# zzhang1987/Factor-Graph-Neural-Network

Hardware: AMD Instinct MI355X
Metric: VF+FV messages/sec on 96.3.963 LDPC graph (higher is better)
Workload: dtype bf16

## Files before the change

factor-graph-neural-network_amd/csrc/bnact.hip:

```cpp
#include "fgnn_common.h"
#include "fgnn_device.h"
#include "fgnn_gridfold.h"
#include <stdlib.h>

#define BN_THREADS 256
#define BN_GRID 512
#define BN_MAXPART 1024
#define BN_APPLY_GRID 4096

struct BnParams {
    const void* x;
    const void* gy;
    void* out;
    float* ws;
    const float* a;
    const float* b;
    const float* gamma;
    const float* beta;
    const float* ref;
    const void* addend;
    const void* addend2;
    const void* addend3;
    int aperiod[3];
    int64_t R;
// ... 27 lines not shown
        const uint4 t = *reinterpret_cast<const uint4*>(p);
        v[0] = __uint_as_float(t.x << 16); v[1] = __uint_as_float(t.x & 0xffff0000u);
        v[2] = __uint_as_float(t.y << 16); v[3] = __uint_as_float(t.y & 0xffff0000u);
        v[4] = __uint_as_float(t.z << 16); v[5] = __uint_as_float(t.z & 0xffff0000u);
        v[6] = __uint_as_float(t.w << 16); v[7] = __uint_as_float(t.w & 0xffff0000u);
    }
    __device__ static void store(bf16_t* p, const float (&v)[8]) {
        *reinterpret_cast<uint4*>(p) = make_uint4(fgnn_pack2(v[0], v[1]), fgnn_pack2(v[2], v[3]), fgnn_pack2(v[4], v[5]), fgnn_pack2(v[6], v[7]));
    }
};

template <typename T, int MODE>
__global__ __launch_bounds__(BN_THREADS) void bn_reduce_kernel(const BnParams p) {
    constexpr int EPC = Chunk<T>::EPC;
    __shared__ __attribute__((aligned(16))) float red[BN_THREADS * 2 * EPC];
    const int tid = threadIdx.x;
    const int cpr = 1 << p.cshift;
    const int cg = tid & (cpr - 1), rg = tid >> p.cshift;
    const int rstep = BN_THREADS >> p.cshift;
    const int c0 = cg * EPC;
    const T* xg = static_cast<const T*>(p.x);
    const T* gg = static_cast<const T*>(p.gy);
    float s0[EPC], s1[EPC], ka[EPC], kb[EPC], kc[EPC], kd[EPC];
#pragma unroll
    for (int e = 0; e < EPC; ++e) {
        s0[e] = 0.f; s1[e] = 0.f;
        if (MODE == 0) { ka[e] = p.ref ? p.ref[c0 + e] : 0.f; kb[e] = 0.f; kc[e] = 0.f; kd[e] = 0.f; }
        else {
            ka[e] = p.a[c0 + e];
            kb[e] = p.b[c0 + e];
            kc[e] = p.gamma[c0 + e] * kb[e];
            kd[e] = p.beta[c0 + e] - ka[e] * kc[e];
        }
    }
    const int64_t r_begin = (int64_t)blockIdx.x * p.rows_per_wg;
    const int64_t r_end = r_begin + p.rows_per_wg < p.R ? r_begin + p.rows_per_wg : p.R;
#pragma unroll 4
    for (int64_t r = r_begin + rg; r < r_end; r += rstep) {
        float v[EPC];
        Chunk<T>::load(xg + r * p.C + c0, v);
        if (MODE == 0) {
#pragma unroll
            for (int e = 0; e < EPC; ++e) { const float dlt = v[e] - ka[e]; s0[e] += dlt; s1[e] = fmaf(dlt, dlt, s1[e]); }
        } else {
            float g[EPC];
            Chunk<T>::load(gg + r * p.C + c0, g);
#pragma unroll
            for (int e = 0; e < EPC; ++e) {
                const float pre = fmaf(v[e], kc[e], kd[e]);
                const float ge = pre > 0.f ? g[e] : g[e] * p.slope;
                s0[e] += ge;
                s1[e] = fmaf(ge, (v[e] - ka[e]) * kb[e], s1[e]);
            }
        }
    }
#pragma unroll
    for (int e = 0; e < EPC; ++e) { red[(tid * 2) * EPC + e] = s0[e]; red[(tid * 2 + 1) * EPC + e] = s1[e]; }
    __syncthreads();
    if (rg == 0) {
        for (int q = 1; q < rstep; ++q) {
            const int t2 = q * cpr + cg;
#pragma unroll
            for (int e = 0; e < EPC; ++e) { s0[e] += red[(t2 * 2) * EPC + e]; s1[e] += red[(t2 * 2 + 1) * EPC + e]; }
        }
        float* w = p.ws + (int64_t)blockIdx.x * 2 * p.C;
#pragma unroll
        for (int e = 0; e < EPC; ++e) { fgnn_fold_store(w + c0 + e, s0[e]); fgnn_fold_store(w + p.C + c0 + e, s1[e]); }
    }
    if (p.fold.tickets) {
        double* sums = reinterpret_cast<double*>(red);
        if (fgnn_grid_fold(p.fold, sums, blockIdx.x)) {
            if (MODE == 0) fgnn_bn_final_apply(p.fin, p.C, sums);
            else fgnn_bn_bwd_final_apply(p.C, sums, nullptr, nullptr, p.dsum, p.gweight, p.gbias);
        }
    }
}

#define BN_FC 4
__device__ __forceinline__ void bn_fold(const float* ws, int nwg, int C, int c, int pg, bool ok, double& s0, double& s1) {
    __shared__ double red0[256], red1[256];
    double a = 0.0, b = 0.0;
    if (ok) {
#pragma unroll 16
        for (int w = pg; w < nwg; w += 256 / BN_FC) { a += (double)ws[(int64_t)w * 2 * C + c]; b += (double)ws[(int64_t)w * 2 * C + C + c]; }
    }
    red0[threadIdx.x] = a;
    red1[threadIdx.x] = b;
    __syncthreads();
    const int cc = threadIdx.x & (BN_FC - 1);
    a = 0.0; b = 0.0;
    if (pg < 8)
        for (int q = pg * 8; q < pg * 8 + 8; ++q) { a += red0[q * BN_FC + cc]; b += red1[q * BN_FC + cc]; }
    __syncthreads();
    if (pg < 8) { red0[threadIdx.x] = a; red1[threadIdx.x] = b; }
    __syncthreads();
    s0 = 0.0; s1 = 0.0;
    if (pg == 0)
        for (int q = 0; q < 8; ++q) { s0 += red0[q * BN_FC + cc]; s1 += red1[q * BN_FC + cc]; }
}

__global__ __launch_bounds__(256) void bn_stats_final_kernel(const float* ws, int nwg, int C, const fgnn_bn_final fin) {
    if (fin.num_batches_tracked && blockIdx.x == 0 && threadIdx.x == 0) *fin.num_batches_tracked += 1;
    const int c = blockIdx.x * BN_FC + (threadIdx.x & (BN_FC - 1)), pg = threadIdx.x / BN_FC;
    double s0, s1;
    bn_fold(ws, nwg, C, c, pg, c < C, s0, s1);
    if (pg != 0 || c >= C) return;
    const double n = (double)fin.count;
    const double m0 = s0 / n;
    double var = s1 / n - m0 * m0;
    if (var < 0.0) var = 0.0;
    const float mu = (float)(m0 + (fin.shift_k ? (double)fin.shift_k[c] : 0.0));
    const float is = (float)(1.0 / sqrt(var + (double)fin.eps));
    fin.mean[c] = mu;
    fin.invstd[c] = is;
    const float g = fin.gamma ? fin.gamma[c] : 1.f, b = fin.beta ? fin.beta[c] : 0.f;
    fin.scale[c] = g * is;
    fin.shift[c] = b - mu * g * is;
    if (fin.running_mean) {
        const double np = (double)(fin.population > 0 ? fin.population : fin.count);
        const double unbiased = np > 1.0 ? var * np / (np - 1.0) : var;
        fin.running_mean[c] = (1.f - fin.momentum) * fin.running_mean[c] + fin.momentum * mu;
        fin.running_var[c] = (1.f - fin.momentum) * fin.running_var[c] + fin.momentum * (float)unbiased;
    }
}

__global__ __launch_bounds__(256) void bn_bwd_final_kernel(const float* ws, int nwg, int C, float* dsum,
                                                           float* gweight, float* gbias) {
    const int c = blockIdx.x * BN_FC + (threadIdx.x & (BN_FC - 1)), pg = threadIdx.x / BN_FC;
    double s0, s1;
    bn_fold(ws, nwg, C, c, pg, c < C, s0, s1);
    if (pg != 0 || c >= C) return;
    dsum[c] = (float)s0;
    dsum[C + c] = (float)s1;
    if (gbias) gbias[c] += (float)s0;
    if (gweight) gweight[c] += (float)s1;
}

template <typename T, int MODE>
__global__ __launch_bounds__(BN_THREADS) void bn_apply_kernel(const BnParams p) {
    constexpr int EPC = Chunk<T>::EPC;
    const int tid = threadIdx.x;
    const int cpr = 1 << p.cshift;
    const int cg = tid & (cpr - 1), rg = tid >> p.cshift;
    const int rstep = BN_THREADS >> p.cshift;
    const int c0 = cg * EPC;
    const T* xg = static_cast<const T*>(p.x);
    const T* gg = static_cast<const T*>(p.gy);
    T* og = static_cast<T*>(p.out);
    float ka[EPC], kb[EPC], kc[EPC], kd[EPC], ke[EPC], kf[EPC];
#pragma unroll
    for (int e = 0; e < EPC; ++e) {
        if (MODE == 0) { ka[e] = p.a[c0 + e]; kb[e] = p.b[c0 + e]; kc[e] = kd[e] = ke[e] = kf[e] = 0.f; }
        else {
            ka[e] = p.a[c0 + e];
            kb[e] = p.b[c0 + e];
            kc[e] = p.gamma[c0 + e] * kb[e];
            kd[e] = p.beta[c0 + e] - ka[e] * kc[e];
            ke[e] = p.dbeta[c0 + e] * p.dsum_scale;
            kf[e] = p.dgamma[c0 + e] * p.dsum_scale;
        }
    }
    const int64_t r_begin = (int64_t)blockIdx.x * p.rows_per_wg;
    const int64_t r_end = r_begin + p.rows_per_wg < p.R ? r_begin + p.rows_per_wg : p.R;
#pragma unroll 4
    for (int64_t r = r_begin + rg; r < r_end; r += rstep) {
        float v[EPC], o[EPC];
        Chunk<T>::load(xg + r * p.C + c0, v);
        if (MODE == 0) {
#pragma unroll
            for (int e = 0; e < EPC; ++e) { const float pre = fmaf(v[e], ka[e], kb[e]); o[e] = pre > 0.f ? pre : pre * p.slope; }
            const void* const ads[3] = {p.addend, p.addend2, p.addend3};
#pragma unroll
            for (int a = 0; a < 3; ++a) {
                if (ads[a]) {
                    float ad[EPC];
                    const int64_t ar = p.aperiod[a] > 1 ? r / p.aperiod[a] : r;
                    Chunk<T>::load(static_cast<const T*>(ads[a]) + ar * p.C + c0, ad);
#pragma unroll
                    for (int e = 0; e < EPC; ++e) o[e] += ad[e];
                }
            }
        } else {
            float g[EPC];
            Chunk<T>::load(gg + r * p.C + c0, g);
#pragma unroll
            for (int e = 0; e < EPC; ++e) {
                const float pre = fmaf(v[e], kc[e], kd[e]);
                const float ge = pre > 0.f ? g[e] : g[e] * p.slope;
                const float xh = (v[e] - ka[e]) * kb[e];
                o[e] = kc[e] * (ge - ke[e] - xh * kf[e]);
            }
        }
        Chunk<T>::store(og + r * p.C + c0, o);
    }
}

static int bn_apply_grid() {
    return BN_APPLY_GRID;
}

static int bn_reduce_grid() {
    return BN_GRID > BN_MAXPART ? BN_MAXPART : BN_GRID;
}

static int bn_plan(int64_t R, int C, int dtype, BnParams* p, int* grid, int target = 0) {
    const int epc = dtype == FGNN_F32 ? 4 : 8;
    if (C % epc != 0) return -1;
    const int cpr = C / epc;
    if (cpr > BN_THREADS || (cpr & (cpr - 1)) != 0) return -1;
    int sh = 0;
    while ((1 << sh) < cpr) ++sh;
    p->cshift = sh;
    p->C = C;
    p->R = R;
    int g = target > 0 ? target : bn_reduce_grid();
    int64_t rows = (R + g - 1) / g;
    const int rstep = BN_THREADS / cpr;
    if (rows < rstep) rows = rstep;
    p->rows_per_wg = (int)rows;
    *grid = (int)((R + rows - 1) / rows);
    return 0;
}

extern "C" int fgnn_bn_supported(int64_t R, int C, int dtype) {
    BnParams p;
    int grid;
    return (R > 0 && C > 0 && (dtype == FGNN_F32 || dtype == FGNN_BF16) && bn_plan(R, C, dtype, &p, &grid) == 0) ? 1 : 0;
}

extern "C" int64_t fgnn_bn_workspace_bytes(int64_t R, int C) { return (int64_t)BN_MAXPART * 2 * C * 4 + 2 * C * 4; }

static int g_inkernel_finalisers = -1;
int fgnn_separate_finalisers(void) {
    if (g_inkernel_finalisers < 0) g_inkernel_finalisers = 0;
    return !g_inkernel_finalisers;
}
extern "C" int fgnn_set_inkernel_finalisers(int on) {
    const int was = !fgnn_separate_finalisers();
    g_inkernel_finalisers = on ? 1 : 0;
    return was;
}

static int bn_check_final(const char* who, const fgnn_bn_final* fin) {
    if (!fin || !fin->mean || !fin->invstd || !fin->scale || !fin->shift) FGNN_FAIL(FGNN_EINVAL, "%s: null pointer in fgnn_bn_final", who);
    if (fin->count < 1 || (fin->population != 0 && fin->population < fin->count)) FGNN_FAIL(FGNN_EINVAL, "%s: bad row counts in fgnn_bn_final", who);
    if ((fin->running_mean == nullptr) != (fin->running_var == nullptr)) FGNN_FAIL(FGNN_EINVAL, "%s: running_mean and running_var go together", who);
    return FGNN_OK;
}

int fgnn_bn_finalize_launch(const float* partials, int npartials, int C, const fgnn_bn_final* fin, hipStream_t st) {
    hipLaunchKernelGGL(bn_stats_final_kernel, dim3((C + BN_FC - 1) / BN_FC), dim3(256), 0, st, partials, npartials, C, *fin);
    return hipGetLastError() == hipSuccess ? 0 : -1;
}

extern "C" int fgnn_bn_stats(const void* x, int64_t R, int C, int dtype, const fgnn_bn_final* fin, void* workspace,
                             int64_t workspace_bytes, void* fold_scratch, fgnn_stream_t stream) {
    BnParams p = {};
    int grid, rc;
    if (!x || !workspace) FGNN_FAIL(FGNN_EINVAL, "bn_stats: null pointer");
    if ((rc = bn_check_final("bn_stats", fin))) return rc;
    if (fin->count != R) FGNN_FAIL(FGNN_EINVAL, "bn_stats: fin->count must be R");
    if (bn_plan(R, C, dtype, &p, &grid)) FGNN_FAIL(FGNN_EUNSUPPORTED, "bn: C=%d not a supported channel count", C);
    if (workspace_bytes < fgnn_bn_workspace_bytes(R, C)) FGNN_FAIL(FGNN_EINVAL, "bn: workspace too small");
    float* ws = (float*)workspace;
    hipStream_t st = (hipStream_t)stream;
    const float* ref = dtype == FGNN_F32 ? (const float*)x : nullptr;
    p.x = x; p.ws = ws; p.ref = ref;
    p.fin = *fin;
    if (ref) {
        if (fin->shift_k) FGNN_FAIL(FGNN_EINVAL, "bn_stats: shift_k is for partials produced elsewhere");
        p.fin.shift_k = ref;
    }
    const bool inkernel = fold_scratch && 2 * C <= FGNN_FOLD_MAXJ && !fgnn_separate_finalisers();
    p.fold = fgnn_fold_make(ws, inkernel ? fold_scratch : nullptr, grid, C);
    if (dtype == FGNN_F32) hipLaunchKernelGGL((bn_reduce_kernel<float, 0>), dim3(grid), dim3(BN_THREADS), 0, st, p);
    else hipLaunchKernelGGL((bn_reduce_kernel<bf16_t, 0>), dim3(grid), dim3(BN_THREADS), 0, st, p);
    if (!inkernel) hipLaunchKernelGGL(bn_stats_final_kernel, dim3((C + BN_FC - 1) / BN_FC), dim3(256), 0, st, ws, grid, C, p.fin);
    hipError_t e = hipGetLastError();
    if (e != hipSuccess) FGNN_FAIL(FGNN_ELAUNCH, "bn_stats launch: %s", hipGetErrorString(e));
    return FGNN_OK;
}

extern "C" int fgnn_bn_finalize(const float* partials, int npartials, int C, const fgnn_bn_final* fin, fgnn_stream_t stream) {
    int rc;
    if (!partials) FGNN_FAIL(FGNN_EINVAL, "bn_finalize: null pointer");
    if ((rc = bn_check_final("bn_finalize", fin))) return rc;
    if (npartials < 1 || npartials > BN_MAXPART || C < 1) FGNN_FAIL(FGNN_EINVAL, "bn_finalize: bad sizes");
    if (fgnn_bn_finalize_launch(partials, npartials, C, fin, (hipStream_t)stream))
        FGNN_FAIL(FGNN_ELAUNCH, "bn_finalize launch: %s", hipGetErrorString(hipGetLastError()));
    return FGNN_OK;
}

extern "C" int fgnn_bn_apply(const void* x, void* y, int64_t R, int C, int dtype, const float* scale,
                             const float* shift, float slope, const void* addend, const void* addend2,
                             const void* addend3, const int32_t* addend_period, fgnn_stream_t stream) {
    BnParams p = {};
    int grid;
    if (!x || !y || !scale || !shift) FGNN_FAIL(FGNN_EINVAL, "bn_apply: null pointer");
    if (bn_plan(R, C, dtype, &p, &grid, bn_apply_grid())) FGNN_FAIL(FGNN_EUNSUPPORTED, "bn: C=%d not a supported channel count", C);
    p.x = x; p.out = y; p.a = scale; p.b = shift; p.slope = slope; p.addend = addend; p.addend2 = addend2; p.addend3 = addend3;
    for (int a = 0; a < 3; ++a) {
        p.aperiod[a] = addend_period ? addend_period[a] : 1;
        if (p.aperiod[a] < 1) FGNN_FAIL(FGNN_EINVAL, "bn_apply: addend period < 1");
    }
    hipStream_t st = (hipStream_t)stream;
    if (dtype == FGNN_F32) hipLaunchKernelGGL((bn_apply_kernel<float, 0>), dim3(grid), dim3(BN_THREADS), 0, st, p);
    else hipLaunchKernelGGL((bn_apply_kernel<bf16_t, 0>), dim3(grid), dim3(BN_THREADS), 0, st, p);
    hipError_t e = hipGetLastError();
    if (e != hipSuccess) FGNN_FAIL(FGNN_ELAUNCH, "bn_apply launch: %s", hipGetErrorString(e));
    return FGNN_OK;
}

int fgnn_bn_backward_sums(const void* x, const void* gy, int64_t R, int C, int dtype, const float* mean, const float* invstd,
                          const float* gamma, const float* beta, float slope, float* gweight, float* gbias,
                          void* workspace, void* fold_scratch, hipStream_t st, BnParams* out, const float** dsum_out) {
    BnParams p = {};
    int grid;
    if (bn_plan(R, C, dtype, &p, &grid)) return -1;
    float* ws = (float*)workspace;
    float* dsum = ws + (int64_t)BN_MAXPART * 2 * C;
    p.x = x; p.gy = gy; p.out = nullptr; p.ws = ws; p.a = mean; p.b = invstd; p.gamma = gamma; p.beta = beta;
    p.slope = slope; p.dsum_scale = 1.0f / (float)R; p.dbeta = dsum; p.dgamma = dsum + C;
    p.dsum = dsum; p.gweight = gweight; p.gbias = gbias;
    const bool inkernel = fold_scratch && 2 * C <= FGNN_FOLD_MAXJ && !fgnn_separate_finalisers();
    p.fold = fgnn_fold_make(ws, inkernel ? fold_scratch : nullptr, grid, C);
    if (dtype == FGNN_F32) hipLaunchKernelGGL((bn_reduce_kernel<float, 1>), dim3(grid), dim3(BN_THREADS), 0, st, p);
    else hipLaunchKernelGGL((bn_reduce_kernel<bf16_t, 1>), dim3(grid), dim3(BN_THREADS), 0, st, p);
    if (!inkernel) hipLaunchKernelGGL(bn_bwd_final_kernel, dim3((C + BN_FC - 1) / BN_FC), dim3(256), 0, st, ws, grid, C, dsum, gweight, gbias);
    if (out) *out = p;
    if (dsum_out) *dsum_out = dsum;
    return 0;
}

int fgnn_bn_backward_sums_bf16(const void* x, const void* gy, int64_t R, int C, const float* mean, const float* invstd,
                               const float* gamma, const float* beta, float slope, float* gweight, float* gbias,
                               void* workspace, void* fold_scratch, hipStream_t st, const float** dsum_out) {
    return fgnn_bn_backward_sums(x, gy, R, C, FGNN_BF16, mean, invstd, gamma, beta, slope, gweight, gbias, workspace, fold_scratch, st,
                                 nullptr, dsum_out);
}

extern "C" int fgnn_bn_backward(const void* x, const void* gy, void* gx, int64_t R, int C, int dtype,
                                const float* mean, const float* invstd, const float* gamma, const float* beta,
                                float slope, float* gweight, float* gbias, void* workspace,
                                int64_t workspace_bytes, void* fold_scratch, fgnn_stream_t stream) {
// ... 57 lines not shown
```

factor-graph-neural-network_amd/csrc/fgnn_device.h:

```cpp
#pragma once
#include "fgnn_common.h"

typedef __bf16 bf16x2 __attribute__((ext_vector_type(2)));
typedef __bf16 bf16x8 __attribute__((ext_vector_type(8)));
typedef short s16x4 __attribute__((ext_vector_type(4)));

__device__ __forceinline__ unsigned fgnn_pack2(float a, float b) {
    const bf16x2 h = {(__bf16)a, (__bf16)b};
    return __builtin_bit_cast(unsigned, h);
}
__device__ __forceinline__ float fgnn_lo(unsigned u) { return __uint_as_float(u << 16); }
__device__ __forceinline__ float fgnn_hi(unsigned u) { return __uint_as_float(u & 0xffff0000u); }
__device__ __forceinline__ bf16x8 fgnn_frag8(const float* p8) {
    const f32x4 a = *reinterpret_cast<const f32x4*>(p8), b = *reinterpret_cast<const f32x4*>(p8 + 4);
    return __builtin_bit_cast(bf16x8, make_uint4(fgnn_pack2(a[0], a[1]), fgnn_pack2(a[2], a[3]),
                                                 fgnn_pack2(b[0], b[1]), fgnn_pack2(b[2], b[3])));
}

template <typename T> __device__ __forceinline__ const T* fgnn_at(const void* base, unsigned byte_off) {
    return reinterpret_cast<const T*>(static_cast<const char*>(base) + byte_off);
}
template <typename T> __device__ __forceinline__ T* fgnn_at(void* base, unsigned byte_off) {
    return reinterpret_cast<T*>(static_cast<char*>(base) + byte_off);
}

__device__ __forceinline__ void fgnn_dma16(const void* gsrc, unsigned lds_dst) {
    unsigned keep;
    asm volatile("s_mov_b32 %0, m0\n\ts_mov_b32 m0, %2\n\ts_nop 0\n\tglobal_load_lds_dwordx4 %1, off\n\ts_mov_b32 m0, %0"
                 : "=&s"(keep) : "v"(gsrc), "s"(lds_dst) : "memory");
}
__device__ __forceinline__ void fgnn_dma16s(const void* sbase, unsigned voff, unsigned lds_dst) {
    unsigned keep;
    asm volatile("s_mov_b32 %0, m0\n\ts_mov_b32 m0, %3\n\ts_nop 0\n\tglobal_load_lds_dwordx4 %1, %2\n\ts_mov_b32 m0, %0"
                 : "=&s"(keep) : "v"(voff), "s"(sbase), "s"(lds_dst) : "memory");
}
template <int N> __device__ __forceinline__ void fgnn_wait_vm() { asm volatile("s_waitcnt vmcnt(%0)" ::"n"(N) : "memory"); }

__device__ __forceinline__ uint2 fgnn_tr16(unsigned lds_addr) {
    typedef __attribute__((address_space(3))) s16x4 lds_s16x4;
    const s16x4 v = __builtin_amdgcn_ds_read_tr16_b64_v4i16(reinterpret_cast<lds_s16x4*>(static_cast<uintptr_t>(lds_addr)));
    return __builtin_bit_cast(uint2, v);
}

template <int P>
__device__ __forceinline__ uint4 fgnn_perm_col(const uint2 (&r)[8]) {
    constexpr unsigned sel = (P & 1) ? 0x07060302u : 0x05040100u;
    unsigned w[4];
#pragma unroll
    for (int q = 0; q < 4; ++q) {
        const unsigned a = P < 2 ? r[2 * q].x : r[2 * q].y, b = P < 2 ? r[2 * q + 1].x : r[2 * q + 1].y;
        w[q] = __builtin_amdgcn_perm(b, a, sel);
    }
    return make_uint4(w[0], w[1], w[2], w[3]);
}
__device__ __forceinline__ uint4 fgnn_perm_col_dyn(const uint2 (&r)[8], int P) {
    switch (P) {
        case 0: return fgnn_perm_col<0>(r);
        case 1: return fgnn_perm_col<1>(r);
        case 2: return fgnn_perm_col<2>(r);
        default: return fgnn_perm_col<3>(r);
    }
}

__device__ __forceinline__ float fgnn_row_sum(float v) {
    v += __int_as_float(__builtin_amdgcn_update_dpp(0, __float_as_int(v), 0xB1, 0xF, 0xF, false));
    v += __int_as_float(__builtin_amdgcn_update_dpp(0, __float_as_int(v), 0x4E, 0xF, 0xF, false));
    v += __int_as_float(__builtin_amdgcn_update_dpp(0, __float_as_int(v), 0x141, 0xF, 0xF, false));
    v += __int_as_float(__builtin_amdgcn_update_dpp(0, __float_as_int(v), 0x140, 0xF, 0xF, false));
    return v;
}
__device__ __forceinline__ float fgnn_row_max(float v) {
    v = fmaxf(v, __int_as_float(__builtin_amdgcn_update_dpp(__float_as_int(v), __float_as_int(v), 0xB1, 0xF, 0xF, false)));
    v = fmaxf(v, __int_as_float(__builtin_amdgcn_update_dpp(__float_as_int(v), __float_as_int(v), 0x4E, 0xF, 0xF, false)));
    v = fmaxf(v, __int_as_float(__builtin_amdgcn_update_dpp(__float_as_int(v), __float_as_int(v), 0x141, 0xF, 0xF, false)));
    v = fmaxf(v, __int_as_float(__builtin_amdgcn_update_dpp(__float_as_int(v), __float_as_int(v), 0x140, 0xF, 0xF, false)));
    return v;
}
__device__ __forceinline__ float fgnn_bcast(float v, int lane) {
    return __int_as_float(__builtin_amdgcn_readlane(__float_as_int(v), lane));
}
__device__ __forceinline__ float fgnn_dot2(unsigned p, unsigned e, float acc) {
    return __builtin_amdgcn_fdot2_f32_bf16(__builtin_bit_cast(bf16x2, p), __builtin_bit_cast(bf16x2, e), acc, false);
}

template <int DK> __device__ __forceinline__ void fgnn_pgm_logits(const void* dec, int64_t o, int64_t cs, float& v0, float& v1) {
    if (DK == FGNN_PGM_DEC_F32) {
        const float* d = static_cast<const float*>(dec);
        v0 = d[o]; v1 = d[o + cs];
    } else {
        const bf16_t* d = static_cast<const bf16_t*>(dec);
        v0 = fgnn_ld(d + o); v1 = fgnn_ld(d + o + cs);
    }
}
__device__ __forceinline__ int64_t fgnn_pgm_label(const int64_t* label, int64_t b, int64_t sb, int i) { return label[b * sb + i]; }
__device__ __forceinline__ int fgnn_pgm_decide(float v0, float v1) {
    return v1 > v0 || (__builtin_isnan(v1) && !__builtin_isnan(v0));
}
```

factor-graph-neural-network_amd/csrc/mpconv_bwd.hip:

```cpp
#include "fgnn_common.h"
#include "mpconv_dispatch.h"
#include <stdlib.h>

#define BWD_MAXT 8

struct BwdParams {
    fgnn_mpconv_desc d;
    const void* x;
    const int64_t* idx;
    const void* et;
    const float* W;
    const void* gz;
    const void* z;
    const uint8_t* argmax;
    void* gx;
    void* get;
    float* slab;
    int has_gbias;
    const float* bias;
    int chunk;
    int OT, CT, nproj, Npad, Kpad, XS, WS, PS;
    int off_xs, off_ws, off_ps, off_dps, off_idx, off_et, off_det, off_gz, off_aux, off_gb, off_cs, off_cl;
};

// ... 306 lines not shown
                    }
                }
            }
        }

        for (int step = 0; step < (d.ext == FGNN_EXT_DIFF ? 2 : 1); ++step) {
#pragma unroll
            for (int t = 0; t < BWD_MAXT; ++t) {
                const int u = wave + FGNN_WAVES * t;
                if (u < tpt) {
                    const int ctile = u % nct, colt = u / nct;
                    const int tc = colt * 16 + li;
                    const int proj = tc / CT, q = tc - proj * CT;
                    if (q < vcols) {
                        const int g = o0 * net + q;
#pragma unroll
                        for (int r = 0; r < 4; ++r) {
                            const int c = ctile * 16 + 4 * lk + r;
                            if (c >= nin) continue;
                            const float v = gw[t][r];
                            if (d.ext == FGNN_EXT_NONE) {
                                slab[(int64_t)c * ncols + g] = v;
                            } else if (d.ext == FGNN_EXT_NEIGHBOR) {
                                slab[(int64_t)(proj == 0 ? nin + c : c) * ncols + g] = v;
                            } else if (step == 0) {
                                if (proj == 1) { slab[(int64_t)c * ncols + g] = v; slab[(int64_t)(nin + c) * ncols + g] = v; }
                            } else if (proj == 0) {
                                slab[(int64_t)(nin + c) * ncols + g] -= v;
                            }
                        }
                    }
                }
            }
            __syncthreads();
        }
        if (tid < otc) slab[R_rows * ncols + o0 + tid] = gb_s[tid];
    }
}

static int plan_backward(const fgnn_mpconv_desc* d, BwdParams* p) {
    const int nproj = d->ext == FGNN_EXT_NONE ? 1 : 2;
    p->nproj = nproj;
    p->Npad = fgnn_round_up(d->N, 16);
    p->Kpad = fgnn_round_up(d->nin, 16);
    p->XS = (p->Kpad + 29) / 32 * 32 + 2;
    const int mk = d->M * d->k;
    const int nct = p->Kpad / 16;
    int best = 0;
    for (int pass = 0; pass < 2 && !best; ++pass) {
        const int64_t budget = pass == 0 ? 78 * 1024 : 160 * 1024;
        for (int ot = d->nou < 64 ? d->nou : 64; ot >= 1; ot = (ot == 1) ? 0 : (ot + 1) / 2) {
            const int CT = fgnn_round_up(ot * d->net, 16);
            const int CTT = CT * nproj;
            if (nct * (CTT / 16) > FGNN_WAVES * BWD_MAXT) continue;
            const int WS = (CTT + 13) / 32 * 32 + 18;
            const int PS = CTT + 4;
            int64_t fl = (int64_t)p->Npad * p->XS + (int64_t)p->Kpad * WS + 2 * (int64_t)p->Npad * PS +
                         fgnn_round_up(mk, 4) + 2 * (int64_t)fgnn_round_up(mk * d->net, 4) +
                         2 * (int64_t)fgnn_round_up(ot * d->M, 4) + fgnn_round_up(ot, 4) +
                         fgnn_round_up(d->N + 1, 4) + fgnn_round_up(mk, 4);
            if (fl * 4 <= budget) { best = ot; break; }
        }
    }
    if (!best) FGNN_FAIL(FGNN_EUNSUPPORTED, "mpconv backward: shape does not fit LDS/register tiling");
    p->OT = best;
    p->CT = fgnn_round_up(best * d->net, 16);
    const int CTT = p->CT * nproj;
    p->WS = (CTT + 13) / 32 * 32 + 18;
    p->PS = CTT + 4;
    int off = 0;
    p->off_xs = off;  off += p->Npad * p->XS;  off = fgnn_round_up(off, 4);
    p->off_ws = off;  off += p->Kpad * p->WS;  off = fgnn_round_up(off, 4);
    p->off_ps = off;  off += p->Npad * p->PS;  off = fgnn_round_up(off, 4);
    p->off_dps = off; off += p->Npad * p->PS;  off = fgnn_round_up(off, 4);
    p->off_idx = off; off += fgnn_round_up(mk, 4);
    p->off_et = off;  off += fgnn_round_up(mk * d->net, 4);
    p->off_det = off; off += fgnn_round_up(mk * d->net, 4);
    p->off_gz = off;  off += fgnn_round_up(best * d->M, 4);
    p->off_aux = off; off += fgnn_round_up(best * d->M, 4);
    p->off_gb = off;  off += fgnn_round_up(best, 4);
    p->off_cs = off;  off += fgnn_round_up(d->N + 1, 4);
    p->off_cl = off;  off += fgnn_round_up(mk, 4);
    return off * 4;
}

template <typename T, int NET>
static void* pick_agg_b(int agg) {
    switch (agg) {
        case FGNN_AGG_MAX: return (void*)mpconv_bwd_kernel<T, NET, FGNN_AGG_MAX>;
        case FGNN_AGG_LSE: return (void*)mpconv_bwd_kernel<T, NET, FGNN_AGG_LSE>;
        default: return (void*)mpconv_bwd_kernel<T, NET, FGNN_AGG_MEAN>;
    }
}
template <typename T>
static void* pick_net_b(int net, int agg) {
    switch (net) {
        case 1: return pick_agg_b<T, 1>(agg);
        case 4: return pick_agg_b<T, 4>(agg);
        case 16: return pick_agg_b<T, 16>(agg);
        default: return pick_agg_b<T, 0>(agg);
    }
}

extern "C" int fgnn_mpconv_backward_reduces_getype(const fgnn_mpconv_desc* d) {
    if (!d || fgnn_check_desc(d)) return 0;
    return fgnn_bwd_ext_accepts(d, fgnn_switches());
}

static int generic_plan(const FgnnBwdCall& c, const FgnnSwitches&, FgnnPlan* pl) {
    const fgnn_mpconv_desc* d = c.d;
    if (d->reserved & FGNN_DESC_GETYPE_REDUCED)
        FGNN_FAIL(FGNN_EUNSUPPORTED, "batch-reduced edge-type gradient asked of a shape without that kernel");
    BwdParams p;
    pl->lds = plan_backward(d, &p);
    if (pl->lds < 0) return pl->lds;
    const int64_t R_rows = d->ext == FGNN_EXT_NONE ? d->nin : 2 * d->nin;
    const int64_t slab_len = R_rows * d->nou * d->net + d->nou;
    if (!c.workspace || c.workspace_bytes < 256 * slab_len * 4)
        FGNN_FAIL(FGNN_EINVAL, "mpconv backward: workspace of fgnn_mpconv_backward_workspace_bytes(d) bytes needed");
    const int chunk = (d->B + 255) / 256 < 1 ? 1 : (d->B + 255) / 256;
    pl->aux = chunk;
    pl->grid = (d->B + chunk - 1) / chunk;
    pl->block = FGNN_THREADS;
    pl->fn = d->dtype == FGNN_F32 ? pick_net_b<float>(d->net, d->agg) : pick_net_b<bf16_t>(d->net, d->agg);
    return 1;
}

static int generic_launch(const FgnnBwdCall& c, const FgnnPlan& pl) {
    const fgnn_mpconv_desc* d = c.d;
    BwdParams p;
    p.d = *d;
    p.x = c.x; p.idx = c.idx; p.et = c.et; p.W = c.W; p.gz = c.gz; p.z = c.z; p.argmax = c.argmax;
    p.gx = c.gx; p.get = c.getype; p.bias = nullptr; p.has_gbias = c.gbias != nullptr;
    plan_backward(d, &p);
    const int64_t R_rows = d->ext == FGNN_EXT_NONE ? d->nin : 2 * d->nin;
    const int64_t nw = R_rows * d->nou * d->net, slab_len = nw + d->nou;
    p.slab = (float*)c.workspace;
    p.chunk = pl.aux;
    if (pl.lds > 48 * 1024) {
        hipError_t e = hipFuncSetAttribute(pl.fn, hipFuncAttributeMaxDynamicSharedMemorySize, pl.lds);
        if (e != hipSuccess) FGNN_FAIL(FGNN_ELAUNCH, "hipFuncSetAttribute(%d B LDS): %s", pl.lds, hipGetErrorString(e));
    }
    fgnn_note_kernel("mpconv_bwd_kernel<%s, %d, %d>", d->dtype ? "bf16_t" : "float",
                     (d->net == 1 || d->net == 4 || d->net == 16) ? d->net : 0, d->agg);
    void* args[] = {(void*)&p};
    hipError_t e = hipLaunchKernel(pl.fn, dim3(pl.grid), dim3(pl.block), args, pl.lds, c.stream);
    if (e != hipSuccess) FGNN_FAIL(FGNN_ELAUNCH, "mpconv backward launch: %s", hipGetErrorString(e));
    fgnn_launch_slab_reduce(p.slab, pl.grid, slab_len, nw, c.gW, c.gbias, c.stream);
    e = hipGetLastError();
    if (e != hipSuccess) FGNN_FAIL(FGNN_ELAUNCH, "mpconv backward fold launch: %s", hipGetErrorString(e));
    return FGNN_OK;
}

static const struct { FgnnBwdPlanFn plan; FgnnBwdLaunchFn launch; } kBwdFamilies[] = {
    {fgnn_bwd_ext_plan, fgnn_bwd_ext_launch},
    {fgnn_bwd_hyper_plan, fgnn_bwd_hyper_launch},
    {fgnn_bwd_ws_plan, fgnn_bwd_ws_launch},
    {fgnn_bwd_sg_plan, fgnn_bwd_sg_launch},
    {fgnn_bwd_b16_plan, fgnn_bwd_b16_launch},
    {fgnn_bwd_res_plan, fgnn_bwd_res_launch},
    {generic_plan, generic_launch},
};
static const int kBwdGeneric = sizeof(kBwdFamilies) / sizeof(kBwdFamilies[0]) - 1;

static int bwd_run(const FgnnBwdCall& c) {
    const FgnnSwitches& sw = fgnn_switches();
    for (int f = sw.force_generic ? kBwdGeneric : 0; f <= kBwdGeneric; ++f) {
        FgnnPlan pl = {};
        pl.family = f;
        const int rc = kBwdFamilies[f].plan(c, sw, &pl);
        if (rc < 0) return rc;
        if (rc > 0) return kBwdFamilies[f].launch(c, pl);
    }
    return FGNN_EUNSUPPORTED;
}

extern "C" int fgnn_mpconv_backward_with_tables(const fgnn_mpconv_desc* d, const void* x, const int64_t* nn_idx,
                                                const void* etype, const float* filters, const void* gz,
                                                const void* z, const uint8_t* argmax, void* gx, void* getype,
                                                float* gfilters, float* gbias, void* workspace,
                                                int64_t workspace_bytes, const void* tables, fgnn_stream_t stream) {
    int rc = fgnn_check_desc(d);
    if (rc) return rc;
    if (!x || !nn_idx || !etype || !filters || !gz || !gx || !gfilters)
        FGNN_FAIL(FGNN_EINVAL, "null tensor pointer");
    if (d->agg == FGNN_AGG_MAX && !argmax) FGNN_FAIL(FGNN_EINVAL, "max aggregator needs the forward's argmax");
    if (d->B == 0) return FGNN_OK;
    const FgnnBwdCall c = {d, x, nn_idx, etype, filters, gz, z, argmax, gx, getype, gfilters, gbias, workspace, workspace_bytes,
                           tables, (hipStream_t)stream};
    return bwd_run(c);
}

extern "C" int fgnn_mpconv_backward(const fgnn_mpconv_desc* d, const void* x, const int64_t* nn_idx,
                                    const void* etype, const float* filters, const void* gz,
                                    const void* z, const uint8_t* argmax, void* gx, void* getype,
                                    float* gfilters, float* gbias, void* workspace,
                                    int64_t workspace_bytes, fgnn_stream_t stream) {
    return fgnn_mpconv_backward_with_tables(d, x, nn_idx, etype, filters, gz, z, argmax, gx, getype, gfilters, gbias, workspace,
                                            workspace_bytes, nullptr, stream);
}
```

factor-graph-neural-network_amd/csrc/mpconv_bwd_hyper.hip:

```cpp
#include "fgnn_common.h"
#include "fgnn_device.h"
#include "mpconv_dispatch.h"
#include <stdlib.h>

#define BH_THREADS 512
#define BH_WAVES 8

struct BhParams {
    fgnn_mpconv_desc d;
    const void* x;
    const int64_t* idx;
    const void* et;
    const float* W;
    const void* gz;
    const uint8_t* argmax;
    void* gx;
    float* ws;
    int has_bias;
};

extern __shared__ __attribute__((aligned(16))) float fgnn_lds_bh[];


template <int NIN, int NOU>
__device__ __forceinline__ void bh_stage_w(const float* __restrict__ W, float* Wl, int tid) {
    for (int f = tid; f < NIN * NOU; f += BH_THREADS) {
        const int c = f / NOU, o = f - c * NOU;
        Wl[o * NIN + c] = W[f];
    }
}

template <int NI, int NO>
__device__ __forceinline__ void bh_flush(const BhParams& p, float* Wl, float* bl, float (&dW)[NI][64 * NO],
                                         const float (&gbv)[4 * NO], const int (&gbc)[4 * NO], int ngb, int tid,
                                         int lane, int wave) {
    constexpr int NIN = 64 * NI, NOU = 64 * NO;
    __syncthreads();
    for (int w = 0; w < BH_WAVES; ++w) {
        if (wave == w) {
#pragma unroll
            for (int i = 0; i < NI; ++i)
#pragma unroll
                for (int o = 0; o < NOU; ++o) {
                    float* q = Wl + o * NIN + lane + 64 * i;
                    *q = (w == 0) ? dW[i][o] : *q + dW[i][o];
                }
#pragma unroll
            for (int t = 0; t < 4 * NO; ++t)
                if (t < ngb && gbc[t] >= 0) bl[gbc[t]] = (w == 0) ? gbv[t] : bl[gbc[t]] + gbv[t];
        }
        __syncthreads();
    }
    float* slab = p.ws + (int64_t)blockIdx.x * (NIN * NOU + NOU);
    for (int f = tid; f < NIN * NOU; f += BH_THREADS) {
        const int c = f / NOU, o = f - c * NOU;
        slab[f] = Wl[o * NIN + c];
    }
    for (int f = tid; f < NOU; f += BH_THREADS) slab[NIN * NOU + f] = bl[f];
}

template <typename T, int NI, int NO>
__global__ __launch_bounds__(BH_THREADS) void mpconv_bwd_fanin_kernel(const BhParams p) {
    constexpr int NIN = 64 * NI, NOU = 64 * NO;
    const fgnn_mpconv_desc& d = p.d;
    const int tid = threadIdx.x, lane = tid & 63;
    const int wave = __builtin_amdgcn_readfirstlane(tid >> 6);
    float* Wl = fgnn_lds_bh;
    float* bl = Wl + NIN * NOU;
    bh_stage_w<NIN, NOU>(p.W, Wl, tid);
    __syncthreads();

    const T* X = reinterpret_cast<const T*>(p.x);
    const T* ET = reinterpret_cast<const T*>(p.et);
    const T* GZ = reinterpret_cast<const T*>(p.gz);
    T* GX = reinterpret_cast<T*>(p.gx);
    const int N = d.N, k = d.k;

    float dW[NI][NOU];
#pragma unroll
    for (int i = 0; i < NI; ++i)
#pragma unroll
        for (int o = 0; o < NOU; ++o) dW[i][o] = 0.f;
    float gbv[4 * NO];
    int gbc[4 * NO];
#pragma unroll
    for (int t = 0; t < 4 * NO; ++t) { gbv[t] = 0.f; gbc[t] = -1; }
#pragma unroll
    for (int q = 0; q < NO; ++q) gbc[q] = lane + 64 * q;

    const int nwaves = gridDim.x * BH_WAVES;
    for (int b = blockIdx.x * BH_WAVES + wave; b < d.B; b += nwaves) {
        int ns[NO];
        float cf[NO];
#pragma unroll
        for (int q = 0; q < NO; ++q) {
            const int64_t yo = (int64_t)b * d.y_sb + (int64_t)(lane + 64 * q) * d.y_sc;
            const float g = fgnn_ld(GZ + yo);
            int js = p.argmax[yo];
            js = js < k ? js : k - 1;
            int n = (int)p.idx[(int64_t)b * d.idx_sb + (int64_t)js * d.idx_sk];
            n = n < 0 ? 0 : (n >= N ? N - 1 : n);
            ns[q] = n;
            cf[q] = g * fgnn_ld(ET + (int64_t)b * d.et_sb + (int64_t)js * d.et_sk);
            gbv[q] += g;
        }
        const T* xb = X + (int64_t)b * d.x_sb;
#pragma unroll
        for (int q = 0; q < NO; ++q)
#pragma unroll
            for (int ol = 0; ol < 64; ++ol) {
                const int n = __builtin_amdgcn_readlane(ns[q], ol);
                const float s = fgnn_bcast(cf[q], ol);
#pragma unroll
                for (int i = 0; i < NI; ++i)
                    dW[i][ol + 64 * q] =
                        fmaf(s, fgnn_ld(xb + (int64_t)n * d.x_sn + (int64_t)(lane + 64 * i) * d.x_sc), dW[i][ol + 64 * q]);
            }
        T* gxb = GX + (int64_t)b * d.x_sb;
        for (int n = 0; n < N; ++n) {
            float acc[NI];
#pragma unroll
            for (int i = 0; i < NI; ++i) acc[i] = 0.f;
#pragma unroll
            for (int q = 0; q < NO; ++q) {
                unsigned long long mask = __ballot(ns[q] == n);
                while (mask) {
                    const int ol = __builtin_ctzll(mask);
                    mask &= mask - 1;
                    const float s = fgnn_bcast(cf[q], ol);
                    const float* wr = Wl + (ol + 64 * q) * NIN + lane;
#pragma unroll
                    for (int i = 0; i < NI; ++i) acc[i] = fmaf(s, wr[64 * i], acc[i]);
                }
            }
#pragma unroll
            for (int i = 0; i < NI; ++i)
                fgnn_st(gxb + (int64_t)n * d.x_sn + (int64_t)(lane + 64 * i) * d.x_sc, acc[i]);
        }
    }
    bh_flush<NI, NO>(p, Wl, bl, dW, gbv, gbc, NO, tid, lane, wave);
}

template <typename T, int NI, int NO>
__global__ __launch_bounds__(BH_THREADS) void mpconv_bwd_fanout_kernel(const BhParams p) {
    constexpr int NIN = 64 * NI, NOU = 64 * NO, CH = 4 * NO;
    const fgnn_mpconv_desc& d = p.d;
    const int tid = threadIdx.x, lane = tid & 63;
    const int wave = __builtin_amdgcn_readfirstlane(tid >> 6);
    float* Wl = fgnn_lds_bh;
    float* bl = Wl + NIN * NOU;
    bh_stage_w<NIN, NOU>(p.W, Wl, tid);
    __syncthreads();

    const T* X = reinterpret_cast<const T*>(p.x);
    const T* ET = reinterpret_cast<const T*>(p.et);
    const T* GZ = reinterpret_cast<const T*>(p.gz);
    T* GX = reinterpret_cast<T*>(p.gx);
    const int M = d.M;
    const int ch0 = (lane & 15) * CH, rc = lane >> 4;

    float dW[NI][NOU];
#pragma unroll
    for (int i = 0; i < NI; ++i)
#pragma unroll
        for (int o = 0; o < NOU; ++o) dW[i][o] = 0.f;
    float gbv[CH];
    int gbc[CH];
#pragma unroll
    for (int t = 0; t < CH; ++t) { gbv[t] = 0.f; gbc[t] = rc == 0 ? ch0 + t : -1; }

    const int nwaves = gridDim.x * BH_WAVES;
    for (int b = blockIdx.x * BH_WAVES + wave; b < d.B; b += nwaves) {
        float xv[NI];
#pragma unroll
        for (int i = 0; i < NI; ++i) xv[i] = fgnn_ld(X + (int64_t)b * d.x_sb + (int64_t)(lane + 64 * i) * d.x_sc);
        float dp[CH], bs[CH];
#pragma unroll
        for (int t = 0; t < CH; ++t) { dp[t] = 0.f; bs[t] = 0.f; }
        const T* gzb = GZ + (int64_t)b * d.y_sb + ch0;
        const T* etb = ET + (int64_t)b * d.et_sb;
        for (int r = rc; r < M; r += 4) {
            const float e = fgnn_ld(etb + (int64_t)r * d.et_sm);
#pragma unroll
            for (int h = 0; h < NO; ++h) {
                const f32x4 v = fgnn_ld4(gzb + (int64_t)r * d.y_sm + 4 * h);
#pragma unroll
                for (int u = 0; u < 4; ++u) {
                    dp[4 * h + u] = fmaf(e, v[u], dp[4 * h + u]);
                    bs[4 * h + u] += v[u];
                }
            }
        }
#pragma unroll
        for (int t = 0; t < CH; ++t) {
            dp[t] += __shfl_xor(dp[t], 16);
            dp[t] += __shfl_xor(dp[t], 32);
            bs[t] += __shfl_xor(bs[t], 16);
            bs[t] += __shfl_xor(bs[t], 32);
            gbv[t] += bs[t];
        }
        float acc[NI];
#pragma unroll
        for (int i = 0; i < NI; ++i) acc[i] = 0.f;
#pragma unroll
        for (int o = 0; o < NOU; ++o) {
            const float s = fgnn_bcast(dp[o % CH], o / CH);
#pragma unroll
            for (int i = 0; i < NI; ++i) {
                acc[i] = fmaf(s, Wl[o * NIN + lane + 64 * i], acc[i]);
                dW[i][o] = fmaf(s, xv[i], dW[i][o]);
            }
        }
#pragma unroll
        for (int i = 0; i < NI; ++i) fgnn_st(GX + (int64_t)b * d.x_sb + (int64_t)(lane + 64 * i) * d.x_sc, acc[i]);
    }
    bh_flush<NI, NO>(p, Wl, bl, dW, gbv, gbc, CH, tid, lane, wave);
}

template <typename T>
static void* bh_pick(bool fanin, int NI, int NO) {
#define BH_CASE(ni, no) if (NI == ni && NO == no) return fanin ? (void*)mpconv_bwd_fanin_kernel<T, ni, no> : (void*)mpconv_bwd_fanout_kernel<T, ni, no>;
    BH_CASE(1, 1) BH_CASE(1, 2) BH_CASE(2, 1)
#undef BH_CASE
    return nullptr;
}

int fgnn_bwd_hyper_plan(const FgnnBwdCall& c, const FgnnSwitches&, FgnnPlan* pl) {
    const fgnn_mpconv_desc* d = c.d;
    if (c.getype) FGNN_REJECT("hyper-edge backward", 1);
    if (d->ext != FGNN_EXT_NONE || d->agg != FGNN_AGG_MAX || d->net != 1) FGNN_REJECT("hyper-edge backward", 2);
    if (d->nin % 64 || d->nou % 64 || d->nin > 128 || d->nou > 128 || d->nin * d->nou > 64 * 128) FGNN_REJECT("hyper-edge backward", 3);
    const bool fanin = d->M == 1 && d->k >= 1 && d->k <= 256 && d->N >= 1;
    const bool fanout = !fanin && d->N == 1 && d->k == 1;
    if (!fanin && !fanout) FGNN_REJECT("hyper-edge backward", 4);
    if (fanout && !(d->y_sc == 1 && d->y_sm % 4 == 0 && d->y_sb % 4 == 0 && d->y_sm >= d->nou)) FGNN_REJECT("hyper-edge backward", 5);
    const int64_t slab_len = (int64_t)d->nin * d->nou + d->nou;
    if (!c.workspace || c.workspace_bytes < 256 * slab_len * 4) FGNN_REJECT("hyper-edge backward", 6);
    const int NI = d->nin / 64, NO = d->nou / 64;
    pl->fn = d->dtype == FGNN_F32 ? bh_pick<float>(fanin, NI, NO) : bh_pick<bf16_t>(fanin, NI, NO);
    if (!pl->fn) FGNN_REJECT("hyper-edge backward", 7);
    pl->mode = fanin;
    pl->lds = (int)(slab_len * 4);
    pl->grid = (d->B + BH_WAVES - 1) / BH_WAVES < 256 ? (d->B + BH_WAVES - 1) / BH_WAVES : 256;
    pl->block = BH_THREADS;
    return 1;
}

int fgnn_bwd_hyper_launch(const FgnnBwdCall& c, const FgnnPlan& pl) {
    const fgnn_mpconv_desc* d = c.d;
    const int64_t nw = (int64_t)d->nin * d->nou, slab_len = nw + d->nou;
    if (pl.lds > 48 * 1024) {
        hipError_t e = hipFuncSetAttribute(pl.fn, hipFuncAttributeMaxDynamicSharedMemorySize, pl.lds);
        if (e != hipSuccess) FGNN_FAIL(FGNN_ELAUNCH, "hipFuncSetAttribute(%d B LDS): %s", pl.lds, hipGetErrorString(e));
    }
    BhParams p;
    p.d = *d;
    p.x = c.x; p.idx = c.idx; p.et = c.et; p.W = c.W; p.gz = c.gz; p.argmax = c.argmax; p.gx = c.gx;
    p.ws = (float*)c.workspace; p.has_bias = c.gbias != nullptr;
    fgnn_note_kernel("mpconv_bwd_%s_kernel<%s, %d, %d>", pl.mode ? "fanin" : "fanout", d->dtype ? "bf16_t" : "float", d->nin / 64, d->nou / 64);
    void* args[] = {(void*)&p};
    hipError_t e = hipLaunchKernel(pl.fn, dim3(pl.grid), dim3(pl.block), args, pl.lds, c.stream);
    if (e != hipSuccess) FGNN_FAIL(FGNN_ELAUNCH, "mpconv hyper-edge backward launch: %s", hipGetErrorString(e));
    fgnn_launch_slab_reduce(p.ws, pl.grid, slab_len, nw, c.gW, c.gbias, c.stream);
    e = hipGetLastError();
    if (e != hipSuccess) FGNN_FAIL(FGNN_ELAUNCH, "mpconv backward helper launch: %s", hipGetErrorString(e));
    return FGNN_OK;
}
```

factor-graph-neural-network_amd/csrc/mpconv_bwd_ws.hip:

```cpp
#include "fgnn_common.h"
#include "fgnn_device.h"
#include "mpconv_dispatch.h"
#include <stdlib.h>

#define BW_THREADS 512
#define BW_WAVES 8
#define BW_MAXN 96
#define BW_XROW 128
#define BW_GROW 128
#define BW_PROW 512
#define BW_DROW 528

typedef float bw_f32x16 __attribute__((ext_vector_type(16)));

struct BwParams {
    const uint16_t* x;
    const int64_t* idx;
    const uint16_t* et;
    const float* W;
    const uint16_t* gz;
    const uint8_t* argmax;
    uint16_t* gx;
    uint16_t* get;
    float* ws;
    int B, N, M;
    int y_ld, w_ld, x_ld;
    int accum;
    long long x_sb, et_sb, y_sb;
    const int* tables;
    long long* prof;
};

#ifdef FGNN_ENABLE_PROF
#define BW_STAMP(slot) do { if (p.prof && blockIdx.x == 0 && lane == 0 && b == b_begin + 3) p.prof[wave * 16 + (slot)] = __builtin_readcyclecounter(); } while (0)
#define BW_STAMP_G(slot) do { if (p.prof && blockIdx.x == 0 && tid == 0 && (slot) < 128) p.prof[128 + (slot)] = __builtin_readcyclecounter(); } while (0)
#else
#define BW_STAMP(slot) do { } while (0)
#define BW_STAMP_G(slot) do { } while (0)
#endif

extern __shared__ __attribute__((aligned(16))) unsigned char bw_lds[];

__device__ __forceinline__ unsigned bw_add2(unsigned a, unsigned b) {
    return fgnn_pack2(__uint_as_float(a << 16) + __uint_as_float(b << 16), __uint_as_float(a & 0xffff0000u) + __uint_as_float(b & 0xffff0000u));
}
__device__ __forceinline__ void bw_barrier() { asm volatile("s_waitcnt lgkmcnt(0)\n\ts_barrier" ::: "memory"); }
__device__ __forceinline__ int bw_swz_r(int r) { return (((r >> 1) & 1) << 2) | ((((r >> 2) ^ (r >> 3)) & 1) << 1) | ((r >> 3) & 1); }
__device__ __forceinline__ int bw_swz_p(int n, int e) { return ((2 * (n & 3) + (e >> 1)) ^ ((n >> 2) & 1)) & 7; }

template <int KC> struct BwLayout {
    static constexpr int DEG = KC == 6 ? 3 : 6, QS = DEG <= 4 ? 4 : 8;
    static constexpr int NMAX = KC == 6 ? 96 : 64, MMAX = KC == 6 ? 48 : 96;
    static constexpr int OFF_X = 0;
    static constexpr int OFF_G = OFF_X + 3 * BW_MAXN * BW_XROW;
    static constexpr int OFF_PD = OFF_G + NMAX * QS * BW_GROW;
    static constexpr int OFF_ET = OFF_PD + NMAX * BW_DROW;
    static constexpr int OFF_GST = OFF_ET + NMAX * 4 * QS * 2;
    static constexpr int OFF_TAB = OFF_GST + 8 * MMAX * KC + 16;
    static constexpr int OFF_SLOT = OFF_TAB + NMAX * QS * 4 + 16;
    static constexpr int OFF_GT = OFF_SLOT + MMAX * KC * 4;
    static constexpr int OFF_DUMP = OFF_GT + 8 * MMAX * KC * 4;
    static constexpr int BYTES = OFF_DUMP + 16;
};

template <int KC, int DEG>
__device__ __forceinline__ void bw_build_tables(long long idx_v, int N, int M, int tid, int* tab, int* slot_of, unsigned* gtab, int* cnt) {
    typedef BwLayout<KC> LY;
    constexpr int QS = LY::QS, NMAX = LY::NMAX;
    const int mk = M * KC;
    int* tmp = cnt + NMAX;
    for (int f = tid; f < NMAX * QS + 4; f += BW_THREADS) tab[f] = -1;
    if (tid < mk) {
        const int r = tid;
        const long long v = idx_v;
        const int n = (int)(v < 0 ? 0 : (v >= N ? N - 1 : v));
        slot_of[r] = -1;
        const int pos = atomicAdd(&cnt[n], 1);
        if (pos < 8) tmp[n * 8 + pos] = r;
    }
    bw_barrier();
    if (tid < N) {
        const int n = tid, c = min(cnt[n], 8);
        int e[8];
#pragma unroll
        for (int q = 0; q < 8; ++q) e[q] = q < c ? tmp[n * 8 + q] : 0x7fffffff;
#pragma unroll
        for (int a = 0; a < 8; ++a)
#pragma unroll
            for (int q = a & 1; q + 1 < 8; q += 2) {
                const int lo = min(e[q], e[q + 1]), hi = max(e[q], e[q + 1]);
                e[q] = lo; e[q + 1] = hi;
            }
#pragma unroll
        for (int q = 0; q < DEG; ++q)
            if (q < c) { tab[n * QS + q] = e[q]; slot_of[e[q]] = n * QS + q; }
    }
    bw_barrier();
    for (int f = tid; f < 8 * mk; f += BW_THREADS) {
        const int item = f / KC, j = f - item * KC, m = item >> 3, c8 = item & 7;
        const int R = slot_of[m * KC + j];
        gtab[f] = R >= 0 ? (unsigned)(LY::OFF_G + R * BW_GROW + ((c8 ^ bw_swz_r(R)) << 4)) : (unsigned)LY::OFF_DUMP;
    }
    bw_barrier();
}

template <int KC, int DEG>
__global__ __launch_bounds__(BW_THREADS) void mpconv_bwd_ws_tables_kernel(const int64_t* idx, int N, int M, int* out) {
    typedef BwLayout<KC> LY;
    constexpr int QS = LY::QS, NMAX = LY::NMAX, MMAX = LY::MMAX;
    __shared__ int tab[NMAX * QS + 4], slot_of[MMAX * KC], cnt[NMAX * 9];
    __shared__ unsigned gtab[8 * MMAX * KC];
    const int tid = threadIdx.x, mk = M * KC;
    for (int f = tid; f < NMAX * 9; f += BW_THREADS) cnt[f] = 0;
    const long long idx_v = tid < mk ? idx[tid] : 0;
    bw_barrier();
    bw_build_tables<KC, DEG>(idx_v, N, M, tid, tab, slot_of, gtab, cnt);
    for (int f = tid; f < NMAX * QS + 4; f += BW_THREADS) out[f] = tab[f];
    for (int f = tid; f < 8 * mk; f += BW_THREADS) out[NMAX * QS + 4 + f] = (int)gtab[f];
}

template <int KC, int DEG, int XLD = 64, int NL = BwLayout<KC>::NMAX>
__global__ __launch_bounds__(BW_THREADS) void mpconv_bwd_ws_kernel(const BwParams p) {
    typedef BwLayout<KC> LY;
    constexpr int QS = LY::QS;
    constexpr int NMAX = LY::NMAX;
    constexpr int OFF_X = LY::OFF_X, OFF_G = LY::OFF_G, OFF_PD = LY::OFF_PD, OFF_ET = LY::OFF_ET, OFF_GST = LY::OFF_GST,
                  OFF_TAB = LY::OFF_TAB, OFF_SLOT = LY::OFF_SLOT, OFF_GT = LY::OFF_GT;
    constexpr int NPG = 16 / QS;
    static_assert(NL % 16 == 0 && NL <= LY::NMAX && (NL / 8) % NPG == 0, "NL");
    constexpr int NG = NL / NPG / 8;
    constexpr int NSLOT = KC == 3 ? 2 : 1;
    constexpr int ESLOT = 1;
    constexpr int MAXNPW = NL / 8;
    const int tid = threadIdx.x;
    BW_STAMP_G(0);
    const int wave = __builtin_amdgcn_readfirstlane(tid >> 6), lane = tid & 63;
    const int l31 = lane & 31, lh = lane >> 5, i16 = lane & 15, g4 = lane >> 4;
    const int N = p.N, M = p.M, mk = M * KC;
    constexpr int Npad = NMAX;
    const unsigned lds0 = (unsigned)(uintptr_t)bw_lds;
    int* tab = reinterpret_cast<int*>(bw_lds + OFF_TAB);
    int* slot_of = reinterpret_cast<int*>(bw_lds + OFF_SLOT);
    unsigned* gtab = reinterpret_cast<unsigned*>(bw_lds + OFF_GT);

    BW_STAMP_G(1);
    const bool dx_wave = wave < 2;
    const bool dw_wave = wave == 2 || wave == 3 || wave == 6 || wave == 7;
    const bool build_wave = wave >= 2;
    const bool dma_wave = dw_wave;
    const int bl = (wave - 2) * 64 + lane;
    const int dwq = wave < 4 ? wave - 2 : wave - 4;

    unsigned dsrc[3];
#pragma unroll
    for (int u = 0; u < 3; ++u) {
        const int slot = 64 * (dwq + 4 * u) + lane, row = slot >> 3, pos = slot & 7;
        dsrc[u] = (unsigned)(min(row, N - 1) * (XLD * 2) + ((pos ^ bw_swz_r(row)) << 4));
    }
    constexpr int npieces = 12;

    const int chunk_b = (p.B + gridDim.x - 1) / gridDim.x;
    const int b_begin = blockIdx.x * chunk_b, b_end = min(p.B, b_begin + chunk_b);
    const unsigned char* xg = reinterpret_cast<const unsigned char*>(p.x);

    auto dma_x = [&](int b, int buf) {
        const unsigned char* xb = xg + (int64_t)b * p.x_sb * 2;
#pragma unroll
        for (int u = 0; u < 3; ++u) {
            const int piece = dwq + 4 * u;
            if (piece < npieces) fgnn_dma16s(xb, dsrc[u], lds0 + (unsigned)(OFF_X + buf * (BW_MAXN * BW_XROW) + piece * 1024));
        }
    };
    if (b_begin < b_end && dma_wave) { dma_x(b_begin, 0); if (b_begin + 1 < b_end) dma_x(b_begin + 1, 1); }

    constexpr int WROW = 528;
    {
        unsigned char* wst = bw_lds + OFF_G;
        static_assert(64 * WROW <= LY::OFF_ET - LY::OFF_G, "W staging fits the G + P region");
#pragma unroll
        for (int it = 0; it < 4; ++it) {
            const int i = tid + BW_THREADS * it, row = i >> 5, c8 = i & 31;
            const bf16x8 f = fgnn_frag8(p.W + (int64_t)row * p.w_ld + 8 * c8);
            *reinterpret_cast<bf16x8*>(wst + row * WROW + c8 * 16) = f;
        }
    }
    long long idx_v = tid < mk ? p.idx[tid] : 0;
    bw_barrier();
    BW_STAMP_G(40);
    bf16x8 aP[4];
    unsigned xoff[4], pwo[2];
    {
        const int ob = (wave & 7) >> 1, ep = wave & 1;
        const int g = l31 >> 3, h = (l31 >> 2) & 1, r = l31 & 3;
        const int col = 4 * (16 * ob + 8 * h + 4 * (g & 1) + r) + 2 * ep + (g >> 1);
#pragma unroll
        for (int kk = 0; kk < 4; ++kk) {
            unsigned w8[8];
#pragma unroll
            for (int u = 0; u < 8; ++u) w8[u] = *reinterpret_cast<const uint16_t*>(bw_lds + OFF_G + (16 * kk + 8 * lh + u) * WROW + col * 2);
            aP[kk] = __builtin_bit_cast(bf16x8, make_uint4(w8[0] | (w8[1] << 16), w8[2] | (w8[3] << 16), w8[4] | (w8[5] << 16), w8[6] | (w8[7] << 16)));
            xoff[kk] = (unsigned)(l31 * BW_XROW + (((2 * kk + lh) ^ bw_swz_r(l31)) << 4));
        }
#pragma unroll
        for (int el = 0; el < 2; ++el)
            pwo[el] = (unsigned)(OFF_PD + l31 * BW_PROW + (2 * ep + el) * 128 + (((2 * ob + lh) ^ bw_swz_p(l31, 2 * ep + el)) << 4));
    }
    bw_f32x16 RA[4];
    const int dwi = wave < 4 ? wave - 2 : wave - 4;
    if (dx_wave) {
#pragma unroll
        for (int t = 0; t < 4; ++t)
#pragma unroll
            for (int sub = 0; sub < 4; ++sub) {
                const f32x4 f = *reinterpret_cast<const f32x4*>(bw_lds + OFF_G + (32 * wave + l31) * WROW + 32 * (4 * t + sub) + 16 * lh);
#pragma unroll
                for (int u = 0; u < 4; ++u) RA[t][4 * sub + u] = f[u];
            }
    } else {
#pragma unroll
        for (int t = 0; t < 4; ++t)
#pragma unroll
            for (int u = 0; u < 16; ++u) RA[t][u] = 0.f;
    }
    auto prefetch_g = [&](int b, uint4 (&pg)[NSLOT], uint2 (&pa)[NSLOT]) {
        const unsigned char* gzb = reinterpret_cast<const unsigned char*>(p.gz + (int64_t)b * p.y_sb);
        const unsigned char* amb = p.argmax + (int64_t)b * p.y_sb;
        int blo = bl;
        asm volatile("" : "+v"(blo));
#pragma unroll
        for (int sl = 0; sl < NSLOT; ++sl) {
            const int item = blo + 384 * sl;
            pg[sl] = make_uint4(0, 0, 0, 0);
            pa[sl] = make_uint2(0, 0);
            if (build_wave && item < 8 * M) {
                const unsigned el = (unsigned)((item >> 3) * p.y_ld + 8 * (item & 7));
                pg[sl] = *fgnn_at<uint4>(gzb, el * 2u);
                pa[sl] = *fgnn_at<uint2>(amb, el);
            }
        }
    };
    BW_STAMP_G(41);
    uint4 pg0[NSLOT];
    uint2 pa0[NSLOT];
    if (b_begin < b_end) prefetch_g(b_begin, pg0, pa0);

    bw_barrier();
    BW_STAMP_G(42);
    for (int f = OFF_G / 16 + tid; f < LY::BYTES / 16; f += BW_THREADS) reinterpret_cast<uint4*>(bw_lds)[f] = make_uint4(0, 0, 0, 0);
    BW_STAMP_G(43);
    bw_barrier();
    BW_STAMP_G(44);
    if (p.tables) {
        for (int f = tid; f < Npad * QS + 4; f += BW_THREADS) tab[f] = p.tables[f];
        for (int f = tid; f < 8 * mk; f += BW_THREADS) gtab[f] = (unsigned)p.tables[Npad * QS + 4 + f];
        bw_barrier();
        BW_STAMP_G(2);
        BW_STAMP_G(6);
    } else {
        int* cnt = reinterpret_cast<int*>(bw_lds + OFF_PD);
        bw_build_tables<KC, DEG>(idx_v, N, M, tid, tab, slot_of, gtab, cnt);
        BW_STAMP_G(6);
        for (int f = tid; f < (NMAX * 9 + 3) / 4; f += BW_THREADS) reinterpret_cast<uint4*>(cnt)[f] = make_uint4(0, 0, 0, 0);
        bw_barrier();
    }

    BW_STAMP_G(7);
    int et_src[ESLOT];
    unsigned et_dst[ESLOT];
#pragma unroll
    for (int sl = 0; sl < ESLOT; ++sl) {
        et_src[sl] = -1;
        et_dst[sl] = 0;
        const int is = bl + 384 * sl;
        if (build_wave && is < N * QS) {
            const int n = is / QS, q = is - n * QS;
            if (q < DEG) et_src[sl] = tab[n * QS + q];
            et_dst[sl] = (unsigned)(OFF_ET + ((n * 4) * QS + q) * 2);
        }
    }
    unsigned da[NG], db_[NG], dt[NG];
#pragma unroll
    for (int sl = 0; sl < NG; ++sl) {
        const int gi = wave + 8 * sl;
        const int R = gi * 16 + i16;
        da[sl] = (unsigned)(OFF_G + R * BW_GROW + ((g4 ^ bw_swz_r(R)) << 4));
        const int jn = QS == 4 ? (i16 >> 2) : ((i16 & 7) >> 2), e = i16 & 3;
        const int nb = gi * NPG + jn;
        db_[sl] = (unsigned)(OFF_PD + nb * BW_PROW + e * 128 + ((g4 ^ bw_swz_p(nb, e)) << 4));
        bool ok;
        int n, q0;
        if (QS == 4) { ok = g4 == (i16 >> 2); n = gi * 4 + g4; q0 = 0; }
        else { ok = i16 < 8 && (g4 >> 1) == (i16 >> 2); n = gi * 2 + (g4 >> 1); q0 = 4 * (g4 & 1); }
        dt[sl] = (ok && n < N) ? (unsigned)(OFF_TAB + (n * QS + q0) * 4) : (unsigned)(OFF_TAB + NMAX * QS * 4);
    }
    constexpr int npw = MAXNPW;
    unsigned gpat[4][QS / 4];
#pragma unroll
    for (int v = 0; v < 4; ++v)
#pragma unroll
        for (int h4 = 0; h4 < QS / 4; ++h4) {
            const int R = v * QS + 4 * h4 + (i16 >> 2);
            const int chunk = 2 * g4 + ((i16 & 3) >> 1);
            gpat[v][h4] = lds0 + (unsigned)(OFF_G + (4 * h4 + (i16 >> 2)) * BW_GROW + ((chunk ^ bw_swz_r(R)) << 4) + 8 * (i16 & 1));
        }
    unsigned xa[2][2], db[2];
#pragma unroll
    for (int r = 0; r < 2; ++r) {
        const int nd = 8 * (g4 >> 1) + (i16 >> 2) + 4 * r;
        const int fx = bw_swz_r(nd);
#pragma unroll
        for (int c2 = 0; c2 < 2; ++c2) {
            const int chunk = 4 * c2 + 2 * (g4 & 1) + ((i16 & 3) >> 1);
            xa[c2][r] = (unsigned)(nd * BW_XROW + ((chunk ^ fx) << 4) + 8 * (i16 & 1));
        }
        db[r] = lds0 + (unsigned)(OFF_PD + nd * BW_DROW + (64 * dwi + 16 * (g4 & 1) + 4 * (i16 & 3)) * 2);
    }
    s16x4 ones_row0;
    {
        const short o = (lane & 3) == 0 ? (short)0x3f80 : (short)0;
        ones_row0 = (s16x4){o, o, o, o};
    }
    f32x4 dbacc = {0.f, 0.f, 0.f, 0.f};

    auto prefetch_e = [&](int b, uint2 (&pe)[ESLOT]) {
#pragma unroll
        for (int sl = 0; sl < ESLOT; ++sl) {
            pe[sl] = make_uint2(0, 0);
            if (et_src[sl] >= 0) pe[sl] = *fgnn_at<uint2>(p.et + (int64_t)b * p.et_sb, (unsigned)et_src[sl] * 8u);
        }
    };
    auto build = [&](const uint4 (&pg)[NSLOT], const uint2 (&pa)[NSLOT], const uint2 (&pe)[ESLOT]) {
#pragma unroll
        for (int sl = 0; sl < ESLOT; ++sl) {
            if (et_src[sl] >= 0) {
                uint16_t* ew = reinterpret_cast<uint16_t*>(bw_lds + et_dst[sl]);
                ew[0] = (uint16_t)pe[sl].x; ew[QS] = (uint16_t)(pe[sl].x >> 16);
                ew[2 * QS] = (uint16_t)pe[sl].y; ew[3 * QS] = (uint16_t)(pe[sl].y >> 16);
            }
        }
#pragma unroll
        for (int sl = 0; sl < NSLOT; ++sl) {
            const int item = bl + 384 * sl;
            if (item < 8 * M) {
                typedef unsigned short u16x2 __attribute__((ext_vector_type(2)));
                typedef short s16x2 __attribute__((ext_vector_type(2)));
                const unsigned gq[4] = {pg[sl].x, pg[sl].y, pg[sl].z, pg[sl].w};
                unsigned gofs[KC];
#pragma unroll
                for (int j = 0; j < KC; ++j) gofs[j] = gtab[item * KC + j];
                u16x2 oh[4];
#pragma unroll
                for (int d = 0; d < 4; ++d) {
                    const unsigned src = d < 2 ? pa[sl].x : pa[sl].y;
                    const unsigned a2 = __builtin_amdgcn_perm(0u, src, (d & 1) ? 0x0c030c02u : 0x0c010c00u) & 0x00070007u;
                    oh[d] = (u16x2){1, 1} << __builtin_bit_cast(u16x2, a2);
                }
#pragma unroll
                for (int j = 0; j < KC; ++j) {
                    unsigned w[4];
#pragma unroll
                    for (int d = 0; d < 4; ++d) {
                        const s16x2 msk = __builtin_bit_cast(s16x2, (u16x2)(oh[d] << (u16x2){(unsigned short)(15 - j), (unsigned short)(15 - j)})) >> (s16x2){15, 15};
                        w[d] = gq[d] & __builtin_bit_cast(unsigned, msk);
                    }
                    *reinterpret_cast<uint4*>(bw_lds + gofs[j]) = make_uint4(w[0], w[1], w[2], w[3]);
                }
            }
        }
    };

    BW_STAMP_G(3);
    if (b_begin < b_end) {
        if (build_wave) {
            uint2 pe[ESLOT];
            prefetch_e(b_begin, pe); build(pg0, pa0, pe);
        }
        if (dma_wave) fgnn_wait_vm<0>();
    }
    bw_barrier();
    constexpr int ntile = NMAX / 32;
    int cur = 0;

    for (int b = b_begin; b < b_end; ++b) {
        const unsigned char* xs = bw_lds + OFF_X + cur * (BW_MAXN * BW_XROW);
        const bool has_next = b + 1 < b_end;
        BW_STAMP(0);
        BW_STAMP_G(8 + (b - b_begin));
        {
            uint4 xb[3][4];
#pragma unroll
            for (int t = 0; t < 3; ++t)
#pragma unroll
                for (int kk = 0; kk < 4; ++kk)
                    xb[t][kk] = t < ntile ? *reinterpret_cast<const uint4*>(xs + t * 32 * BW_XROW + xoff[kk]) : make_uint4(0, 0, 0, 0);
            __builtin_amdgcn_sched_barrier(0);
            bw_f32x16 acc[3];
#pragma unroll
            for (int t = 0; t < 3; ++t)
#pragma unroll
                for (int u = 0; u < 16; ++u) acc[t][u] = 0.f;
#pragma unroll
            for (int kk = 0; kk < 4; ++kk)
#pragma unroll
                for (int t = 0; t < 3; ++t)
                    if (t < ntile) acc[t] = __builtin_amdgcn_mfma_f32_32x32x16_bf16(aP[kk], __builtin_bit_cast(bf16x8, xb[t][kk]), acc[t], 0, 0, 0);
#pragma unroll
            for (int t = 0; t < 3; ++t) {
                if (t < ntile) {
                    unsigned char* pp0 = bw_lds + t * 32 * BW_PROW + pwo[0];
                    unsigned char* pp1 = bw_lds + t * 32 * BW_PROW + pwo[1];
                    *reinterpret_cast<uint4*>(pp0) = make_uint4(fgnn_pack2(acc[t][0], acc[t][1]), fgnn_pack2(acc[t][2], acc[t][3]),
                                                                fgnn_pack2(acc[t][4], acc[t][5]), fgnn_pack2(acc[t][6], acc[t][7]));
                    *reinterpret_cast<uint4*>(pp1) = make_uint4(fgnn_pack2(acc[t][8], acc[t][9]), fgnn_pack2(acc[t][10], acc[t][11]),
                                                                fgnn_pack2(acc[t][12], acc[t][13]), fgnn_pack2(acc[t][14], acc[t][15]));
                }
            }
        }
        BW_STAMP(1);
        bw_barrier();
        BW_STAMP(2);
        auto phase2a = [&]() {
            {
                uint16_t* gst = reinterpret_cast<uint16_t*>(bw_lds + OFF_GST);
                uint4 fa[NG][2], fb[NG][2];
                int4 te[NG];
    #pragma unroll
                for (int sl = 0; sl < NG; ++sl) {
                    fa[sl][0] = *reinterpret_cast<const uint4*>(bw_lds + da[sl]);
                    fb[sl][0] = *reinterpret_cast<const uint4*>(bw_lds + db_[sl]);
                    fa[sl][1] = *reinterpret_cast<const uint4*>(bw_lds + (da[sl] ^ 64u));
                    fb[sl][1] = *reinterpret_cast<const uint4*>(bw_lds + (db_[sl] ^ 64u));
                    te[sl] = *reinterpret_cast<const int4*>(bw_lds + dt[sl]);
                }
                __builtin_amdgcn_sched_barrier(0);
                f32x4 acc[NG];
    #pragma unroll
                for (int sl = 0; sl < NG; ++sl)
                    acc[sl] = __builtin_amdgcn_mfma_f32_16x16x32_bf16(__builtin_bit_cast(bf16x8, fa[sl][0]), __builtin_bit_cast(bf16x8, fb[sl][0]),
                                                                      (f32x4){0.f, 0.f, 0.f, 0.f}, 0, 0, 0);
    #pragma unroll
                for (int sl = 0; sl < NG; ++sl)
                    acc[sl] = __builtin_amdgcn_mfma_f32_16x16x32_bf16(__builtin_bit_cast(bf16x8, fa[sl][1]), __builtin_bit_cast(bf16x8, fb[sl][1]),
                                                                      acc[sl], 0, 0, 0);
                const int e = i16 & 3;
    #pragma unroll
                for (int sl = 0; sl < NG; ++sl) {
                    const int ed[4] = {te[sl].x, te[sl].y, te[sl].z, te[sl].w};
    #pragma unroll
                    for (int r = 0; r < 4; ++r)
                        if (ed[r] >= 0) gst[e * mk + ed[r]] = (uint16_t)(fgnn_pack2(acc[sl][r], 0.f) & 0xffffu);
                }
            }
        };
        auto phase2b = [&]() {
            {
                uint2 bv[MAXNPW][QS / 4], av[MAXNPW][QS / 4];
    #pragma unroll
                for (int i = 0; i < MAXNPW; ++i) {
                    const int n = wave * npw + i;
    #pragma unroll
                    for (int h4 = 0; h4 < QS / 4; ++h4) {
                        bv[i][h4] = fgnn_tr16(gpat[i & 3][h4] + (unsigned)(n * QS * BW_GROW));
                        av[i][h4] = *reinterpret_cast<const uint2*>(bw_lds + OFF_ET + ((n * 4 + (lane & 3)) * QS + 4 * h4) * 2);
                    }
                }
                __builtin_amdgcn_sched_barrier(0);
                BW_STAMP(9);
    #pragma unroll
                for (int i = 0; i < MAXNPW; ++i) {
                    {
                        const int n = wave * npw + i;
                        f32x4 acc = {0.f, 0.f, 0.f, 0.f};
    #pragma unroll
                        for (int h4 = 0; h4 < QS / 4; ++h4) {
                            const s16x4 b4 = __builtin_bit_cast(s16x4, bv[i][h4]);
                            acc = __builtin_amdgcn_mfma_f32_4x4x4bf16_1k(__builtin_bit_cast(s16x4, av[i][h4]), b4, acc, 0, 0, 0);
                            dbacc = __builtin_amdgcn_mfma_f32_4x4x4bf16_1k(ones_row0, b4, dbacc, 0, 0, 0);
                        }
                        *reinterpret_cast<uint2*>(bw_lds + OFF_PD + n * BW_DROW + lane * 8) = make_uint2(fgnn_pack2(acc[0], acc[1]), fgnn_pack2(acc[2], acc[3]));
                    }
                }
                BW_STAMP(10);
                const int nvec = (8 * mk) >> 4;
                if (tid < nvec) {
                    uint4 v = *reinterpret_cast<const uint4*>(bw_lds + OFF_GST + tid * 16);
                    if (p.accum & 2) {
                        const uint4 o = *fgnn_at<uint4>(p.get + (int64_t)b * 4 * mk, (unsigned)tid * 16u);
                        v = make_uint4(bw_add2(v.x, o.x), bw_add2(v.y, o.y), bw_add2(v.z, o.z), bw_add2(v.w, o.w));
                    }
                    *fgnn_at<uint4>(p.get + (int64_t)b * 4 * mk, (unsigned)tid * 16u) = v;
                }
            }
        };
        auto phase3_dw = [&](const uint4 (&pg)[NSLOT], const uint2 (&pa)[NSLOT], const uint2 (&pe)[ESLOT]) {
                const unsigned xbase = lds0 + (unsigned)(OFF_X + cur * (BW_MAXN * BW_XROW));
                constexpr int nks = NL / 16;
                uint2 f0[8], f1[8];
                auto load = [&](uint2 (&f)[8], int ks) {
    #pragma unroll
                    for (int c2 = 0; c2 < 2; ++c2) {
                        f[2 * c2] = fgnn_tr16(xbase + xa[c2][0] + ks * (16 * BW_XROW));
                        f[2 * c2 + 1] = fgnn_tr16(xbase + xa[c2][1] + ks * (16 * BW_XROW));
                    }
    #pragma unroll
                    for (int cj = 0; cj < 2; ++cj) {
                        f[4 + 2 * cj] = fgnn_tr16(db[0] + ks * (16 * BW_DROW) + cj * 64);
                        f[5 + 2 * cj] = fgnn_tr16(db[1] + ks * (16 * BW_DROW) + cj * 64);
                    }
                };
                auto mma = [&](const uint2 (&f)[8]) {
    #pragma unroll
                    for (int c2 = 0; c2 < 2; ++c2)
    #pragma unroll
                        for (int cj = 0; cj < 2; ++cj)
                            RA[2 * c2 + cj] = __builtin_amdgcn_mfma_f32_32x32x16_bf16(
                                __builtin_bit_cast(bf16x8, make_uint4(f[2 * c2].x, f[2 * c2].y, f[2 * c2 + 1].x, f[2 * c2 + 1].y)),
                                __builtin_bit_cast(bf16x8, make_uint4(f[4 + 2 * cj].x, f[4 + 2 * cj].y, f[5 + 2 * cj].x, f[5 + 2 * cj].y)),
                                RA[2 * c2 + cj], 0, 0, 0);
                };
                load(f0, 0);
                if (has_next) build(pg, pa, pe);
    #pragma unroll 1
                for (int ks = 0; ks + 1 < nks; ks += 2) {
                    load(f1, ks + 1);
                    mma(f0);
                    if (ks + 2 < nks) load(f0, ks + 2);
                    mma(f1);
                }
                if (nks & 1) mma(f0);
        };
        if (build_wave) {
            uint4 pg[NSLOT];
            uint2 pa[NSLOT], pe[ESLOT];
            prefetch_g(has_next ? b + 1 : b, pg, pa);
            prefetch_e(has_next ? b + 1 : b, pe);
            phase2a();
            BW_STAMP(3);
            bw_barrier();
            BW_STAMP(4);
            phase2b();
            BW_STAMP(5);
            bw_barrier();
            BW_STAMP(6);
            if (dw_wave) phase3_dw(pg, pa, pe);
            else if (has_next) build(pg, pa, pe);
        } else {
            phase2a();
            BW_STAMP(3);
            bw_barrier();
            BW_STAMP(4);
            phase2b();
            BW_STAMP(5);
            bw_barrier();
            BW_STAMP(6);
            {
                uint16_t* gxb = p.gx + (int64_t)b * p.x_sb;
                uint4 bf[16];
                const unsigned char* bp0 = bw_lds + OFF_PD + l31 * BW_DROW + lh * 16;
#pragma unroll
                for (int ks = 0; ks < 8; ++ks) bf[ks] = *reinterpret_cast<const uint4*>(bp0 + 32 * ks);
#pragma unroll
                for (int nt = 0; nt < ntile; ++nt) {
                    const unsigned char* bp = bp0 + nt * 32 * BW_DROW;
#pragma unroll
                    for (int ks = 8; ks < 16; ++ks) bf[ks] = *reinterpret_cast<const uint4*>(bp + 32 * ks);
                    __builtin_amdgcn_sched_barrier(0);
                    bw_f32x16 ae, ao;
#pragma unroll
                    for (int u = 0; u < 16; ++u) { ae[u] = 0.f; ao[u] = 0.f; }
#pragma unroll
                    for (int ks = 0; ks < 16; ks += 2) {
                        if (ks == 8) {
                            __builtin_amdgcn_sched_barrier(0);
                            if (nt + 1 < ntile) {
#pragma unroll
                                for (int k2 = 0; k2 < 8; ++k2) bf[k2] = *reinterpret_cast<const uint4*>(bp + 32 * BW_DROW + 32 * k2);
                            }
                            __builtin_amdgcn_sched_barrier(0);
                        }
                        f32x4 f0, f1;
#pragma unroll
                        for (int u = 0; u < 4; ++u) { f0[u] = RA[ks >> 2][4 * (ks & 3) + u]; f1[u] = RA[(ks + 1) >> 2][4 * ((ks + 1) & 3) + u]; }
                        ae = __builtin_amdgcn_mfma_f32_32x32x16_bf16(__builtin_bit_cast(bf16x8, f0), __builtin_bit_cast(bf16x8, bf[ks]), ae, 0, 0, 0);
                        ao = __builtin_amdgcn_mfma_f32_32x32x16_bf16(__builtin_bit_cast(bf16x8, f1), __builtin_bit_cast(bf16x8, bf[ks + 1]), ao, 0, 0, 0);
                    }
                    const int n = nt * 32 + l31;
                    if (n < N) {
#pragma unroll
                        for (int g = 0; g < 4; ++g) {
                            float v0 = ae[4 * g] + ao[4 * g], v1 = ae[4 * g + 1] + ao[4 * g + 1], v2 = ae[4 * g + 2] + ao[4 * g + 2],
                                  v3 = ae[4 * g + 3] + ao[4 * g + 3];
                            uint2* dst = fgnn_at<uint2>(gxb, (unsigned)(n * XLD + 32 * wave + 8 * g + 4 * lh) * 2u);
                            if (p.accum & 1) {
                                const uint2 o = *dst;
                                v0 += __uint_as_float(o.x << 16); v1 += __uint_as_float(o.x & 0xffff0000u);
                                v2 += __uint_as_float(o.y << 16); v3 += __uint_as_float(o.y & 0xffff0000u);
                            }
                            *dst = make_uint2(fgnn_pack2(v0, v1), fgnn_pack2(v2, v3));
                        }
                    }
                }
            }
        }
        if (dma_wave) {
            fgnn_wait_vm<0>();
            if (b + 2 < b_end) dma_x(b + 2, cur >= 1 ? cur - 1 : 2);
        }
        BW_STAMP(7);
        bw_barrier();
        BW_STAMP(8);
        cur = cur == 2 ? 0 : cur + 1;
    }

    BW_STAMP_G(4);
    if (b_begin < b_end) {
        float* slab = p.ws + (int64_t)blockIdx.x * (64 * 256 + 64);
        if (dw_wave) {
#pragma unroll
            for (int c2 = 0; c2 < 2; ++c2)
#pragma unroll
                for (int cj = 0; cj < 2; ++cj) {
                    const int col = 32 * (2 * dwi + cj) + l31;
#pragma unroll
                    for (int u = 0; u < 16; ++u) {
                        const int c = 32 * c2 + (u & 3) + 8 * (u >> 2) + 4 * lh;
                        slab[c * 256 + col] = RA[2 * c2 + cj][u];
                    }
                }
        }
        __syncthreads();
        float* red = reinterpret_cast<float*>(bw_lds + OFF_X);
        red[wave * 64 + lane] = dbacc[0];
        __syncthreads();
        if (tid < 64) {
            float s = 0.f;
            for (int w = 0; w < BW_WAVES; ++w) s += red[w * 64 + tid];
            slab[64 * 256 + tid] = s;
        }
    }
    BW_STAMP_G(5);
}

static int bw_tables_count(const fgnn_mpconv_desc* d) {
    if (fgnn_switches().no_ws || d->dtype != FGNN_BF16 || d->ext != FGNN_EXT_NONE || d->net != 4 || d->agg != FGNN_AGG_MAX) return 0;
    if (d->nin != 64 || (d->nou != 64 && d->nou != 128) || (d->k != 3 && d->k != 6)) return 0;
    if (d->idx_sb != 0 && d->B > 1) return 0;
    if (!(d->idx_sk == 1 && d->idx_sm == d->k)) return 0;
    const int KC = d->k;
    if (KC == 6 ? (d->N > 96 || d->M > 48) : (d->N > 64 || d->M > 96)) return 0;
    if ((d->M * KC) & 1) return 0;
    return (KC == 6 ? BwLayout<6>::NMAX * BwLayout<6>::QS : BwLayout<3>::NMAX * BwLayout<3>::QS) + 4 + 8 * d->M * KC;
}

extern "C" int64_t fgnn_mpconv_backward_tables_bytes(const fgnn_mpconv_desc* d) {
    if (fgnn_check_desc(d)) return 0;
    return (int64_t)bw_tables_count(d) * 4;
}

extern "C" int fgnn_mpconv_backward_tables(const fgnn_mpconv_desc* d, const int64_t* nn_idx, void* tables, fgnn_stream_t stream) {
    int rc = fgnn_check_desc(d);
    if (rc) return rc;
    if (!nn_idx || !tables) FGNN_FAIL(FGNN_EINVAL, "mpconv_backward_tables: null pointer");
    const int KC = d->k, DEG = KC == 6 ? 3 : 6, indeg = d->reserved & 0xffff;
    if (bw_tables_count(d) == 0 || indeg < 1 || indeg > DEG)
        FGNN_FAIL(FGNN_EUNSUPPORTED, "mpconv_backward_tables: not a shape / in-degree of the table-driven backward");
    if (KC == 6) hipLaunchKernelGGL((mpconv_bwd_ws_tables_kernel<6, 3>), dim3(1), dim3(BW_THREADS), 0, (hipStream_t)stream, nn_idx, d->N, d->M, (int*)tables);
    else hipLaunchKernelGGL((mpconv_bwd_ws_tables_kernel<3, 6>), dim3(1), dim3(BW_THREADS), 0, (hipStream_t)stream, nn_idx, d->N, d->M, (int*)tables);
    hipError_t e = hipGetLastError();
    if (e != hipSuccess) FGNN_FAIL(FGNN_ELAUNCH, "mpconv_backward_tables launch: %s", hipGetErrorString(e));
    return FGNN_OK;
}

int fgnn_bwd_ws_plan(const FgnnBwdCall& c, const FgnnSwitches& sw, FgnnPlan* pl) {
    const fgnn_mpconv_desc* d = c.d;
    const bool ksplit = d->nin == 128 && d->nou == 64;
    const int r = fgnn_bwd_sg_rules(c, sw, ksplit, pl);
    if (r <= 0) return r;
    if (sw.no_ws) FGNN_REJECT("ws backward", 0);
    const bool split = !ksplit && pl->split;
    const int KC = d->k, DEG = KC == 6 ? 3 : 6;
    const int indeg = d->reserved & 0xffff;
    if (indeg < 1 || indeg > DEG) FGNN_REJECT("ws backward", 2);
    if (KC == 6 ? (d->N > 96 || d->M > 48) : (d->N > 64 || d->M > 96)) FGNN_REJECT("ws backward", 3);
    if ((d->M * KC) & 1) FGNN_REJECT("ws backward", 4);
    if (((uintptr_t)c.getype & 15) || ((uintptr_t)c.x & 15) || ((uintptr_t)c.gz & 15) || ((uintptr_t)c.argmax & 7) || ((uintptr_t)c.gx & 7) ||
        ((uintptr_t)c.et & 7)) FGNN_REJECT("ws backward", 5);
    if ((d->x_sb % 8) != 0 || (d->y_sb % 8) != 0 || (d->et_sb % 4) != 0) FGNN_REJECT("ws backward", 6);
    const int64_t slab_len = 64 * 256 + 64;
    if (!c.workspace || c.workspace_bytes < ((split || ksplit) ? 2 : 1) * 256 * slab_len * 4) FGNN_REJECT("ws backward", 7);
    const bool nl48 = KC == 3 && d->N <= 48;
    pl->fn = ksplit ? (KC == 6 ? (void*)mpconv_bwd_ws_kernel<6, 3, 128> : nl48 ? (void*)mpconv_bwd_ws_kernel<3, 6, 128, 48> : (void*)mpconv_bwd_ws_kernel<3, 6, 128>)
                    : (KC == 6 ? (void*)mpconv_bwd_ws_kernel<6, 3> : nl48 ? (void*)mpconv_bwd_ws_kernel<3, 6, 64, 48> : (void*)mpconv_bwd_ws_kernel<3, 6>);
    static_assert(BwLayout<6>::BYTES <= 160 * 1024 && BwLayout<3>::BYTES <= 160 * 1024, "LDS");
    pl->lds = KC == 6 ? BwLayout<6>::BYTES : BwLayout<3>::BYTES;
    int grid = d->B < 256 ? d->B : 256;
    const int chunk = (d->B + grid - 1) / grid;
    pl->grid = (d->B + chunk - 1) / chunk;
    pl->block = BW_THREADS;
    pl->split = split ? 1 : 0;
    pl->mode = ksplit ? 1 : 0;
    pl->aux = c.tables && bw_tables_count(d) > 0;
    return 1;
}

int fgnn_bwd_ws_launch(const FgnnBwdCall& c, const FgnnPlan& pl) {
    const fgnn_mpconv_desc* d = c.d;
    const bool split = pl.split, ksplit = pl.mode;
    const int KC = d->k, DEG = KC == 6 ? 3 : 6;
    const int64_t nw = 64 * 256, slab_len = nw + 64;
    BwParams p;
    p.x = (const uint16_t*)c.x; p.idx = c.idx; p.et = (const uint16_t*)c.et; p.W = c.W;
    p.gz = (const uint16_t*)c.gz; p.argmax = c.argmax; p.gx = (uint16_t*)c.gx; p.get = (uint16_t*)c.getype;
    p.ws = (float*)c.workspace;
    p.B = d->B; p.N = d->N; p.M = d->M;
    p.y_ld = d->nou; p.w_ld = d->nou * 4; p.x_ld = d->nin; p.accum = 0;
    p.x_sb = d->x_sb; p.et_sb = d->et_sb; p.y_sb = d->y_sb;
    p.tables = pl.aux ? (const int*)c.tables : nullptr;
    hipError_t e = hipFuncSetAttribute(pl.fn, hipFuncAttributeMaxDynamicSharedMemorySize, pl.lds);
    if (e != hipSuccess) FGNN_FAIL(FGNN_ELAUNCH, "hipFuncSetAttribute(%d B LDS): %s", pl.lds, hipGetErrorString(e));
    const int grid = pl.grid;
    hipStream_t st = c.stream;
    fgnn_note_kernel(split ? "mpconv_bwd_ws_kernel<%d, %d> x2" : (ksplit ? "mpconv_bwd_ws_kernel<%d, %d> k2" : "mpconv_bwd_ws_kernel<%d, %d>"), KC, DEG);
    p.prof = fgnn_prof_begin();
    void* args[] = {(void*)&p};
    e = hipLaunchKernel(pl.fn, dim3(grid), dim3(pl.block), args, pl.lds, st);
    if (e != hipSuccess) FGNN_FAIL(FGNN_ELAUNCH, "mpconv ws backward launch: %s", hipGetErrorString(e));
    fgnn_prof_print(p.prof, "ws bwd", 0, 8, 11, 16);
    fgnn_prof_print(p.prof, "ws bwd kernel", 128, 1, 45, 0);
    if (ksplit) {
        fgnn_launch_slab_reduce(p.ws, grid, slab_len, nw, c.gW, c.gbias, st);
        p.ws += (int64_t)grid * slab_len;
        p.x += 64; p.W += 64 * (int64_t)p.w_ld; p.gx += 64; p.accum = 2;
        e = hipLaunchKernel(pl.fn, dim3(grid), dim3(pl.block), args, pl.lds, st);
        if (e != hipSuccess) FGNN_FAIL(FGNN_ELAUNCH, "mpconv ws backward launch (upper input channels): %s", hipGetErrorString(e));
        fgnn_launch_slab_reduce(p.ws, grid, slab_len, nw, c.gW + nw, nullptr, st);
    } else if (!split) fgnn_launch_slab_reduce(p.ws, grid, slab_len, nw, c.gW, c.gbias, st);
    else {
        fgnn_launch_slab_reduce_ld(p.ws, grid, slab_len, nw, 256, 512, c.gW, c.gbias, st);
        p.ws += (int64_t)grid * slab_len;
        p.W += 256; p.gz += 64; p.argmax += 64; p.accum = 3;
        e = hipLaunchKernel(pl.fn, dim3(grid), dim3(pl.block), args, pl.lds, st);
        if (e != hipSuccess) FGNN_FAIL(FGNN_ELAUNCH, "mpconv ws backward launch (upper half): %s", hipGetErrorString(e));
        fgnn_launch_slab_reduce_ld(p.ws, grid, slab_len, nw, 256, 512, c.gW + 256, c.gbias + 64, st);
    }
    e = hipGetLastError();
    if (e != hipSuccess) FGNN_FAIL(FGNN_ELAUNCH, "mpconv backward helper launch: %s", hipGetErrorString(e));
    return FGNN_OK;
}
```

factor-graph-neural-network_amd/csrc/mpconv_dispatch.h:

```cpp
#pragma once
#include "fgnn_common.h"

struct FgnnFold;

struct FgnnSwitches {
    bool force_generic;
    bool no_ws;
    bool no_sg;
    bool sg_nosplit;
    bool no_bwd_b16;
    bool no_fwd_hyper;
    bool no_fanin_id;
    bool no_ext;
    bool ext_bf16_split;
};
const FgnnSwitches& fgnn_switches();

struct FgnnFwdCall {
    const fgnn_mpconv_desc* d;
    const void* x; const int64_t* idx; const void* et; const float* W; const float* bias;
    const float* pscale; const float* pshift; void* y; uint8_t* argmax;
    bool stats_epilogue; float* stats; const fgnn_bn_final* fin; void* fold_scratch;
    const void* add[3];
    hipStream_t stream;
};

struct FgnnBwdCall {
    const fgnn_mpconv_desc* d;
    const void* x; const int64_t* idx; const void* et; const float* W; const void* gz; const void* z; const uint8_t* argmax;
    void* gx; void* getype; float* gW; float* gbias; void* workspace; int64_t workspace_bytes;
    const void* tables;
    hipStream_t stream;
};

struct FgnnPlan {
    int family;
    void* fn;
    int grid, block, lds;
    int mode, split, et_mode, aux;
};

typedef int (*FgnnFwdPlanFn)(const FgnnFwdCall&, const FgnnSwitches&, FgnnPlan*);
typedef int (*FgnnFwdLaunchFn)(const FgnnFwdCall&, const FgnnPlan&);
typedef int (*FgnnBwdPlanFn)(const FgnnBwdCall&, const FgnnSwitches&, FgnnPlan*);
typedef int (*FgnnBwdLaunchFn)(const FgnnBwdCall&, const FgnnPlan&);

int fgnn_fwd_hyper_plan(const FgnnFwdCall& c, const FgnnSwitches& sw, FgnnPlan* pl);
int fgnn_fwd_hyper_launch(const FgnnFwdCall& c, const FgnnPlan& pl);
int fgnn_fwd_ws_plan(const FgnnFwdCall& c, const FgnnSwitches& sw, FgnnPlan* pl);
int fgnn_fwd_ws_launch(const FgnnFwdCall& c, const FgnnPlan& pl);
int fgnn_fwd_sg_plan(const FgnnFwdCall& c, const FgnnSwitches& sw, FgnnPlan* pl);
int fgnn_fwd_sg_launch(const FgnnFwdCall& c, const FgnnPlan& pl);
int fgnn_fwd_b16_plan(const FgnnFwdCall& c, const FgnnSwitches& sw, FgnnPlan* pl);
int fgnn_fwd_b16_launch(const FgnnFwdCall& c, const FgnnPlan& pl);
int fgnn_fwd_ext_plan(const FgnnFwdCall& c, const FgnnSwitches& sw, FgnnPlan* pl);
int fgnn_fwd_ext_launch(const FgnnFwdCall& c, const FgnnPlan& pl);
int fgnn_fwd_res_plan(const FgnnFwdCall& c, const FgnnSwitches& sw, FgnnPlan* pl);
int fgnn_fwd_res_launch(const FgnnFwdCall& c, const FgnnPlan& pl);
int fgnn_fwd_sg_layout(const FgnnFwdCall& c, const FgnnSwitches& sw, FgnnPlan* pl);

int fgnn_bwd_ext_plan(const FgnnBwdCall& c, const FgnnSwitches& sw, FgnnPlan* pl);
int fgnn_bwd_ext_launch(const FgnnBwdCall& c, const FgnnPlan& pl);
int fgnn_bwd_ext_accepts(const fgnn_mpconv_desc* d, const FgnnSwitches& sw);
int fgnn_bwd_hyper_plan(const FgnnBwdCall& c, const FgnnSwitches& sw, FgnnPlan* pl);
int fgnn_bwd_hyper_launch(const FgnnBwdCall& c, const FgnnPlan& pl);
int fgnn_bwd_ws_plan(const FgnnBwdCall& c, const FgnnSwitches& sw, FgnnPlan* pl);
int fgnn_bwd_ws_launch(const FgnnBwdCall& c, const FgnnPlan& pl);
int fgnn_bwd_sg_plan(const FgnnBwdCall& c, const FgnnSwitches& sw, FgnnPlan* pl);
int fgnn_bwd_sg_launch(const FgnnBwdCall& c, const FgnnPlan& pl);
int fgnn_bwd_b16_plan(const FgnnBwdCall& c, const FgnnSwitches& sw, FgnnPlan* pl);
int fgnn_bwd_b16_launch(const FgnnBwdCall& c, const FgnnPlan& pl);
int fgnn_bwd_res_plan(const FgnnBwdCall& c, const FgnnSwitches& sw, FgnnPlan* pl);
int fgnn_bwd_res_launch(const FgnnBwdCall& c, const FgnnPlan& pl);
int fgnn_bwd_sg_rules(const FgnnBwdCall& c, const FgnnSwitches& sw, bool layout_only, FgnnPlan* pl);

int fgnn_check_desc(const fgnn_mpconv_desc* d);
void fgnn_stats_upper_half(FgnnFold* fold, fgnn_bn_final* fin);
void fgnn_launch_slab_store(const float* ws, int nslab, int64_t slab_len, float* out, hipStream_t st);
int64_t fgnn_mpconv_backward_ext_extra_bytes(const fgnn_mpconv_desc* d);
```

factor-graph-neural-network_amd/fgnn_amd/_hip.py:

```python
import ctypes
import os
import re

import torch

_HERE = os.path.dirname(os.path.abspath(__file__))
LIB_PATH = os.environ.get('FGNN_HIP_LIB') or os.path.join(_HERE, 'libfgnn_hip.so')
HEADER_PATH = os.path.normpath(os.path.join(_HERE, '..', '..', 'include', 'fgnn_hip.h'))


class FgnnHipError(RuntimeError):
    pass


class MPConvDesc(ctypes.Structure):
    _fields_ = [(n, ctypes.c_int32) for n in
                ('B', 'nin', 'nou', 'net', 'N', 'M', 'k', 'ext', 'agg', 'dtype', 'relu', 'reserved')] + \
               [(n, ctypes.c_int64) for n in
                ('x_sb', 'x_sc', 'x_sn', 'idx_sb', 'idx_sm', 'idx_sk',
                 'et_sb', 'et_se', 'et_sm', 'et_sk', 'y_sb', 'y_sc', 'y_sm')]


class BnFinal(ctypes.Structure):
    _fields_ = [(n, ctypes.c_void_p) for n in ('gamma', 'beta', 'running_mean', 'running_var', 'num_batches_tracked',
                                               'mean', 'invstd', 'scale', 'shift', 'shift_k')] + \
               [('count', ctypes.c_int64), ('population', ctypes.c_int64), ('momentum', ctypes.c_float), ('eps', ctypes.c_float)]


class DevicePointer:

    @classmethod
    def from_param(cls, obj):
        if isinstance(obj, torch.Tensor):
            if not obj.is_cuda:
                raise FgnnHipError('a %s tensor of shape %s was passed where libfgnn_hip expects device memory'
                                   % (obj.device, tuple(obj.shape)))
            return ctypes.c_void_p(obj.data_ptr())
        if obj is None or isinstance(obj, (ctypes.c_void_p, ctypes.Array, ctypes._Pointer)):
            return obj
        if isinstance(obj, int):
            return ctypes.c_void_p(obj)
        raise TypeError('expected a tensor, None, an address or a ctypes array / pointer, got %s' % type(obj).__name__)


_SCALARS = {'int': ctypes.c_int32, 'int32_t': ctypes.c_int32, 'int64_t': ctypes.c_int64, 'uint64_t': ctypes.c_uint64,
            'float': ctypes.c_float, 'double': ctypes.c_double, 'fgnn_stream_t': DevicePointer}
_STRUCTS = {'fgnn_mpconv_desc': MPConvDesc, 'fgnn_bn_final': BnFinal}


def _uncommented(header_text):
    return re.sub(r'//[^\n]*', '', re.sub(r'/\*.*?\*/', '', header_text, flags=re.S))


def _ctype(decl, proto, returned=False):
    words = [w for w in decl.replace('*', ' * ').split() if w != 'const']
    if words and re.fullmatch(r'\w+', words[0]) and all(w == '*' for w in words[1:]):
        base, depth = words[0], len(words) - 1
        if depth == 0 and base in _SCALARS:
            return _SCALARS[base]
        if returned:
            if words == ['void']:
                return None
            if words == ['char', '*']:
                return ctypes.c_char_p
        elif depth == 1 and base in _STRUCTS:
            return ctypes.POINTER(_STRUCTS[base])
        elif depth >= 1:
            return DevicePointer
    raise FgnnHipError('include/fgnn_hip.h: no ctypes type for `%s` in `%s`' % (decl.strip(), proto))


def signatures(header_text):
    text = re.sub(r'^[ \t]*#.*$', '', _uncommented(header_text), flags=re.M).replace('extern "C" {', '')
    text = re.sub(r'\{[^{}]*\}', '', text)
    out = {}
    for stmt in text.split(';'):
        stmt = ' '.join(stmt.split())
        if not stmt or stmt == '}' or stmt.startswith(('typedef ', 'enum')):
            continue
        m = re.fullmatch(r'(.*?)\b(fgnn_\w+) ?\((.*)\)', stmt)
        if not m:
            raise FgnnHipError('include/fgnn_hip.h: cannot parse the declaration `%s`' % stmt)
        ret, name, plist = m.groups()
        params = []
        for p in [] if plist.strip() == 'void' else plist.split(','):
            pm = re.fullmatch(r'(.*\W)(\w+)', p.strip())
            if not pm:
                raise FgnnHipError('include/fgnn_hip.h: cannot parse the parameter `%s` of `%s`' % (p.strip(), stmt))
            params.append((pm.group(2), _ctype(pm.group(1), stmt)))
        out[name] = (_ctype(ret, stmt, returned=True), params)
    return out


def constants(header_text):
    text = _uncommented(header_text)
    pairs = re.findall(r'^[ \t]*#define[ \t]+FGNN_(\w+)[ \t]+(\S.*)$', text, flags=re.M)
    for body in re.findall(r'\benum\s*\{([^}]*)\}', text):
        pairs += re.findall(r'FGNN_(\w+)\s*=\s*([^,]+)', body)
    out = {}
    for name, value in pairs:
        if not re.fullmatch(r'[\s\dxXa-fA-F()+*-]+', value):
            raise FgnnHipError('include/fgnn_hip.h: FGNN_%s = `%s` is not an integer expression' % (name, value.strip()))
        out[name] = int(eval(value, {'__builtins__': {}}))
    return out


def _header():
    if not os.path.exists(HEADER_PATH):
        raise FgnnHipError('the C-ABI header was not found at %s — the binding is derived from it and has no built-in '
                           'copy of the interface' % HEADER_PATH)
    with open(HEADER_PATH) as f:
        return f.read()


SIGNATURES, _K = (parse(_header()) for parse in (signatures, constants))
EXPORTS = tuple(SIGNATURES)
EXT_NONE, EXT_NEIGHBOR, EXT_DIFF = _K['EXT_NONE'], _K['EXT_NEIGHBOR'], _K['EXT_DIFF']
DESC_GETYPE_REDUCED = _K['DESC_GETYPE_REDUCED']
DESC_IDENTITY_LIST = _K['DESC_IDENTITY_LIST']
AGG_MAX, AGG_LSE, AGG_MEAN = _K['AGG_MAX'], _K['AGG_LSE'], _K['AGG_MEAN']
F32, BF16 = _K['F32'], _K['BF16']
DEC_F32, DEC_BF16, DEC_U8 = _K['DEC_F32'], _K['DEC_BF16'], _K['DEC_U8']
LABEL_I64, LABEL_U8 = _K['LABEL_I64'], _K['LABEL_U8']
PGM_DEC_F32, PGM_DEC_BF16, PGM_DEC_I64 = _K['PGM_DEC_F32'], _K['PGM_DEC_BF16'], _K['PGM_DEC_I64']
ABI_VERSION = _K['ABI_VERSION']
EUNSUPPORTED = _K['EUNSUPPORTED']
FOLD_SCRATCH_BYTES = _K['FOLD_SCRATCH_BYTES']

AGG_CODES = {'max': AGG_MAX, 'softmax': AGG_LSE, 'mean': AGG_MEAN}


def bn_final(stats, gamma, beta, running_mean, running_var, num_batches_tracked, momentum, eps, count, population=0):
    f = BnFinal()
    dp = lambda t: None if t is None else t.data_ptr()
    f.gamma, f.beta = dp(gamma), dp(beta)
    f.running_mean, f.running_var, f.num_batches_tracked = dp(running_mean), dp(running_var), dp(num_batches_tracked)
    f.mean, f.invstd, f.scale, f.shift = (stats[i].data_ptr() for i in range(4))
    f.shift_k = None
    f.count, f.population = int(count), int(population)
    f.momentum, f.eps = float(momentum), float(eps)
    return f


_lib = None
COMPANIONS = {}
_MISSING = {}


def _bind_companions(L, sigs, header):
    for name, (restype, params) in sigs.items():
        try:
            fn = getattr(L, name)
        except AttributeError:
            _MISSING[name] = header
            continue
        fn.restype, fn.argtypes = restype, [t for _, t in params]
        _MISSING.pop(name, None)


def bind_header(path):
    if not os.path.isabs(path):
        path = os.path.join(os.path.dirname(HEADER_PATH), path)
    if not os.path.exists(path):
        raise FgnnHipError('the companion header %s was not found' % path)
    with open(path) as f:
        sigs = signatures(f.read())
    clash = sorted(set(sigs) & set(SIGNATURES))
    if clash:
        raise FgnnHipError('%s declares %s again (include/fgnn_hip.h has it)' % (os.path.basename(path), ', '.join(clash)))
    for name in sigs:
        COMPANIONS[name] = sigs[name] + (os.path.basename(path),)
    if _lib is not None:
        _bind_companions(_lib, sigs, os.path.basename(path))
    return tuple(sigs)


def _prototype(name):
    if name in SIGNATURES:
        return SIGNATURES[name]
    return COMPANIONS[name][:2]


def _entry(name):
    L = lib()
    if name in _MISSING:
        raise FgnnHipError('%s does not export %s (include/%s): it was built before that header — rebuild it with '
                           '`python __graft_entry__.py`' % (LIB_PATH, name, _MISSING[name]))
    return getattr(L, name)


def lib():
    global _lib
    if _lib is not None:
        return _lib
    if not os.path.exists(LIB_PATH):
        raise FgnnHipError(
            'libfgnn_hip.so not found at %s — the FGNN message operator has no CPU/eager '
            'fallback; build it with `python __graft_entry__.py` (hipcc --offload-arch=gfx950).'
            % LIB_PATH)
    L = ctypes.CDLL(LIB_PATH)
    try:
        L.fgnn_abi_version.restype = ctypes.c_int
        have = int(L.fgnn_abi_version())
    except AttributeError:
        have = None
    if have != ABI_VERSION:
        raise FgnnHipError('%s speaks C-ABI version %s, this package binds version %d (include/fgnn_hip.h): rebuild it '
                           'with `python __graft_entry__.py`' % (LIB_PATH, have, ABI_VERSION))
    for name, (restype, params) in SIGNATURES.items():
        fn = getattr(L, name)
        fn.restype, fn.argtypes = restype, [t for _, t in params]
    for header in sorted({c[2] for c in COMPANIONS.values()}):
        _bind_companions(L, {n: c[:2] for n, c in COMPANIONS.items() if c[2] == header}, header)
    _lib = L
    return L


def invoke(name, *args):
    params = _prototype(name)[1]
    if len(args) == len(params) - 1 and params[-1][0] == 'stream':
        args += (stream_ptr(),)
    if len(args) != len(params):
        raise TypeError('%s takes %d arguments (%s), got %d' % (name, len(params), ', '.join(n for n, _ in params), len(args)))
    try:
        return _entry(name)(*args)
    except ctypes.ArgumentError as e:
        raise FgnnHipError('%s: %s' % (name, e)) from None


def call(name, *args):
    check(invoke(name, *args))


def check(rc):
    if rc != 0:
        raise FgnnHipError('libfgnn_hip: %s (code %d)' % (lib().fgnn_last_error().decode(), rc))


def _ptr(t):
    return None if t is None else ctypes.c_void_p(t.data_ptr())


def stream_ptr():
    return ctypes.c_void_p(torch.cuda.current_stream().cuda_stream)


def dtype_code(t):
    if t.dtype == torch.float32:
        return F32
    if t.dtype == torch.bfloat16:
        return BF16
    raise FgnnHipError('fgnn_amd supports float32 and bfloat16 tensors, got %s' % t.dtype)


def make_desc(x, nn_idx, etype, nou, net, ext, agg, relu, y=None):
    B, nin, N = x.shape[0], x.shape[1], x.shape[2]
    M, k = nn_idx.shape[1], nn_idx.shape[2]
    d = MPConvDesc()
    d.B, d.nin, d.nou, d.net, d.N, d.M, d.k = B, nin, nou, net, N, M, k
    d.ext, d.agg, d.dtype, d.relu = ext, agg, dtype_code(x), int(bool(relu))
    d.x_sb, d.x_sc, d.x_sn = x.stride(0), x.stride(1), x.stride(2)
    d.idx_sb, d.idx_sm, d.idx_sk = nn_idx.stride(0), nn_idx.stride(1), nn_idx.stride(2)
    d.et_sb, d.et_se, d.et_sm, d.et_sk = (etype.stride(0), etype.stride(1),
                                          etype.stride(2), etype.stride(3))
    if y is not None:
        d.y_sb, d.y_sc, d.y_sm = y.stride(0), y.stride(1), y.stride(2)
    return d


LDPC_TRAIN = bind_header('fgnn_hip_ldpc_train.h')
PGM_BP = bind_header('fgnn_hip_pgm_bp.h')
LDPC_CODE = bind_header('fgnn_hip_ldpc_code.h')
```

factor-graph-neural-network_amd/fgnn_amd/mpnn/blocks.py:

```python
import ctypes

import torch

from .. import _hip, ops
from . import pointwise
from .message_op import _EXT_CODE, base_mp_nn, mp_conv_type, mp_conv_v2
from .pointwise import (BatchNormAct2d, BnHandoff, NodeInstanceNorm, PointwiseConv2d, _InstNormAct, _RowLinear, as_addends, node_sum,
                        refresh_in_place)
from .pointwise import state_epoch as pointwise_state_epoch


def _conv_norm_act(cin, cout, norm, act, bias=True):
    layers = [PointwiseConv2d(cin, cout, 1, bias=bias)]
    if norm is not None:
        layers.append(norm)
    layers.append(act)
    return torch.nn.Sequential(*layers)


FUSE_EVAL_BLOCKS = True


class iid_mapping(torch.nn.Module):
    def __init__(self, nin, nout, bias=True):
        super().__init__()
        self.main = _conv_norm_act(nin, nout, None, torch.nn.LeakyReLU(), bias)

    def forward(self, x):
        return self.main(x)


class iid_mapping_bn(torch.nn.Module):
    def __init__(self, nin, nout, bias=True, bn=True):
        super().__init__()
        self.main = _conv_norm_act(nin, nout, BatchNormAct2d(nout, slope=0.0), torch.nn.Identity(), bias)

    def forward(self, x):
        handoff = BnHandoff.of(self.main[1])
        return self.main[1](self.main[0](x, bn=handoff), handoff=handoff)


class iid_mapping_in(torch.nn.Module):
    def __init__(self, nin, nout, bias=True):
        super().__init__()
        self.main = _conv_norm_act(nin, nout, NodeInstanceNorm(relu=True), torch.nn.Identity(), bias)

    def forward(self, x):
        if x.dim() == 4 and x.shape[2] * x.shape[3] == 1:
            return x.new_zeros((x.shape[0], self.main[0].out_channels, 1, 1))
        y = self._fused(x)
        return self.main(x) if y is None else y

    def _fused(self, x):
        if not FUSE_IID_IN or not x.is_cuda or x.dim() != 4 or x.shape[3] != 1 or x.shape[2] not in (48, 96):
            return None
        conv, norm = self.main[0], self.main[1]
        B, C, N, _ = x.shape
        cout = conv.out_channels
        dt = torch.get_autocast_dtype('cuda') if torch.is_autocast_enabled() else x.dtype
        if dt != torch.bfloat16 or C % 64 or cout % 64 or C > 256 or cout > 256 or conv.weight.dtype != torch.float32:
            return None
        grad = torch.is_grad_enabled() and (conv.weight.requires_grad or x.requires_grad)
        if C > (_IID_FUSE_MAX_CIN if grad else 256):
            return None
        rows = x.permute(0, 2, 3, 1)
        if not rows.is_contiguous():
            rows = rows.contiguous()
        rows = rows.view(B * N, C)
        if rows.dtype != torch.bfloat16:
            rows = rows.to(torch.bfloat16)
        weight = conv.weight.view(cout, C)
        w = weight.detach()
        b = None if conv.bias is None else conv.bias.detach().float().contiguous()
        z = torch.empty((B * N, cout), device=x.device, dtype=torch.bfloat16) if grad else None
        y = torch.empty((B, N, 1, cout), device=x.device, dtype=torch.bfloat16)
        rc = []
        ops.timed('linear_instnorm_fwd_kernel', 2 * B * N * (C + cout * (2 if grad else 1)),
                  lambda: rc.append(_hip.invoke('fgnn_linear_instnorm_forward', rows, w, b, z, y, B, N, C, cout, int(norm.relu),
                                                float(norm.eps))),
                  nflops=2 * B * N * C * cout)
        if rc[0] == _hip.EUNSUPPORTED:
            return None
        _hip.check(rc[0])
        if not grad:
            return y.permute(0, 3, 1, 2)
        zz = _RowLinear.apply(rows, weight, conv.bias, False, z, ops.fan_box(x))
        return _InstNormAct.apply(zz.view(B, N, 1, cout).permute(0, 3, 1, 2), norm.relu, y)


_IID_FUSE_MAX_CIN = 128
FUSE_IID_IN = True


class max_pool_layer(torch.nn.Module):
    def __init__(self, dim=2):
        super().__init__()
        self.dim = dim

    def forward(self, input):
        return input.max(dim=self.dim, keepdim=True)[0]


class flatten(torch.nn.Module):
    def forward(self, input):
        return input.view(input.size(0), -1)


TAIL_WGRAD_MOMENTS = True
FUSE_TRAIN_TAIL = True


FUSE_TRAIN_HEAD = True


_HEAD_WIDTHS = (64, 128)


class _BlockHead(torch.autograd.Function):

    @staticmethod
    def forward(ctx, rows, weight, bias, bn_w, bn_b, handoff, slope, box=None):
        ctx.box = box
        z1 = pointwise.hip_linear(rows, weight, bias, bn=handoff)
        if z1 is None:
            raise _hip.FgnnHipError('fused block head: the 1x1 map is outside csrc/linear_fwd_b16.hip (checked by the caller)')
        R = rows.shape[0]
        stats = handoff.batch_stats(z1)
        a1 = torch.empty_like(z1)
        ops.timed('bn_apply (forward)', 2 * z1.numel() * 2, lambda: _hip.call(
            'fgnn_bn_apply', z1, a1, R, 64, _hip.BF16, stats[2], stats[3], slope, None, None, None, None))
        ctx.save_for_backward(rows, z1, stats, weight, bn_w, bn_b)
        ctx.slope = slope
        ctx.params = (weight, bias, bn_w, bn_b)
        return a1

    @staticmethod
    def backward(ctx, ga1):
        ops.backward_node_begins()
        L = _hip.lib()
        rows, z1, stats, weight, bn_w, bn_b = ctx.saved_tensors
        pW, pbias, pw, pb = ctx.params
        R, cin = rows.shape
        dev = rows.device
        ga1 = ga1.contiguous()
        if ga1.dtype != z1.dtype:
            ga1 = ga1.to(z1.dtype)
        grads = ops.param_grads(dev)
        gw1, gb1 = grads.acc('gamma', pw, (64,)), grads.acc('beta', pb, (64,))
        gW, gbias = grads.acc('W', pW, (64, cin)), grads.acc('bias', pbias, (64,))
        sinks = grads.all_sunk('W', 'bias')
        gz1 = torch.empty_like(z1)
        lazy = ctx.needs_input_grad[0] and ctx.box is not None and weight.is_contiguous() and weight.dtype == torch.float32
        gx = None if lazy else torch.empty((R, cin), device=dev, dtype=z1.dtype)
        ws = ops._workspace(dev, int(L.fgnn_bn_workspace_bytes(R, 64)))
        ops.timed('block_head_backward (reduce + finalise + grad)', 2 * R * (5 * 64 + cin), lambda: _hip.call(
            'fgnn_block_head_backward', z1, ga1, stats[0], stats[1], bn_w.detach(), bn_b.detach(), ctx.slope, weight.detach(), gz1, gx, gw1,
            gb1, R, cin, ws, ws.numel() * 4, ops._fold_scratch(dev)), nflops=2 * R * 64 * cin)

        taken = 0
        if lazy:
            taken = ctx.box.deposit(gz1, weight.detach(), wgrad=(rows, gW, gbias) if sinks else None)
        if taken != 2:
            def launch(record, rows=rows, gz1=gz1, gW=gW, gbias=gbias):
                ops.linear_wgrad(rows, [(gz1, gW.view(64, cin), gbias)], record)
            grads.run_wgrad(launch, (rows, gz1), 'W', 'bias')
        if lazy:
            if taken:
                gx = ctx.box.placeholder(rows.shape)
            else:
                gx = pointwise.hip_linear(gz1, weight.detach(), None, transposed=True)
                if gx is None:
                    gx = gz1 @ pointwise.cast_cached(pW._base if pW._base is not None else pW, gz1.dtype).view(weight.shape)
        return (gx if ctx.needs_input_grad[0] else None, grads.result('W', pW.dtype), grads.result('bias'),
                grads.result('gamma'), grads.result('beta'), None, None, None)


LATE_JOIN = True
ROUTE_ADDEND_GRADS = True


class _AddendRoute(torch.autograd.Function):

    @staticmethod
    def forward(ctx, out, periods, streams, *adds):
        ctx.periods = tuple(periods)[:len(adds)]
        ctx.streams = tuple(streams)[:len(adds)]
        return out.view_as(out)

    @staticmethod
    def backward(ctx, g):
        outs = []
        for i, q in enumerate(ctx.periods):
            if not ctx.needs_input_grad[3 + i]:
                outs.append(None)
            elif q == 1:
                outs.append(g)
            else:
                ops.backward_node_begins()
                home = ctx.streams[i] if NODE_SUM_HOME and g.is_cuda else None
                cur = torch.cuda.current_stream(g.device) if g.is_cuda else None
                if home is not None and home != cur:
                    ready = torch.cuda.Event()
                    ready.record(cur)
                    with torch.cuda.stream(home):
                        home.wait_event(ready)
                        outs.append(node_sum(g.contiguous(), q))
                    g.record_stream(home)
                else:
                    outs.append(node_sum(g.contiguous(), q))
        return (g, None, None) + tuple(outs)


NODE_SUM_HOME = True


class _BlockTail(torch.autograd.Function):

    @staticmethod
    def forward(ctx, e, w2, b2, slope2, slope3, bn2, bn3, W2, bias2, w3, b3, population, add0=None, add1=None, add2=None,
                periods=(1, 1, 1)):
        L = _hip.lib()
        R, Cout = e.shape[0], W2.shape[0]
        dev = e.device
        st2 = bn2.batch_stats(e, population)
        ws = ops._workspace(dev, int(L.fgnn_bn_workspace_bytes(R, Cout)))
        fold = ops._fold_scratch(dev)
        a2 = None if TAIL_WGRAD_MOMENTS else torch.empty_like(e)
        W2c = W2.detach()
        bias2c = None if bias2 is None else bias2.detach()
        flops = 2 * R * 64 * Cout
        st3, fin3 = bn3.final(Cout, dev, R, population)
        ops.timed('block_tail_stats_kernel', 2 * R * 64, lambda: _hip.call(
            'fgnn_block_tail_stats', e, st2[2], st2[3], slope2, W2c, bias2c, R, Cout, ws, fin3, fold), nflops=flops)
        out = torch.empty((R, Cout), device=dev, dtype=e.dtype)
        if callable(add0):
            (add0, add1, add2), periods = add0()
        adds = (add0, add1, add2)
        nadd = sum(a is not None for a in adds)
        ops.timed('block_tail_apply_kernel', 2 * R * (2 * 64 + (1 + nadd) * Cout), lambda: _hip.call(
            'fgnn_block_tail_apply', e, st2[2], st2[3], slope2, W2c, bias2c, st3[2], st3[3], slope3, add0, add1, add2,
            pointwise.period_array(periods), out, a2, R, Cout), nflops=flops)
        pointwise.note_state_change()
        ctx.save_for_backward(e, a2, st2, st3, w2, b2, W2, w3)
        ctx.slopes = (slope2, slope3)
        ctx.has_add = tuple(a is not None and a.requires_grad for a in adds)
        ctx.periods = tuple(periods)
        ctx.params = (w2, b2, W2, bias2, w3, b3)
        return out

    @staticmethod
    def backward(ctx, gout):
        ops.backward_node_begins()
        L = _hip.lib()
        e, a2, st2, st3, w2, b2, W2, w3 = ctx.saved_tensors
        slope2, slope3 = ctx.slopes
        pw2, pb2, pW2, pbias2, pw3, pb3 = ctx.params
        R, Cout = e.shape[0], W2.shape[0]
        dev = e.device
        gout = gout.contiguous()
        if gout.dtype != e.dtype:
            gout = gout.to(e.dtype)
        grads = ops.param_grads(dev)
        gw3, gb3 = grads.acc('gamma3', pw3, (Cout,)), grads.acc('beta3', pb3, (Cout,))
        gw2, gb2 = grads.acc('gamma2', pw2, (64,)), grads.acc('beta2', pb2, (64,))
        gW2, gbias2 = grads.acc('W2', pW2, (Cout, 64)), grads.acc('bias2', pbias2, (Cout,))
        moments = a2 is None
        gz3 = None if moments else torch.empty((R, Cout), device=dev, dtype=e.dtype)
        ga2 = torch.empty_like(e)
        nws = (2048 * Cout + 2 * Cout + 1024 * 128) * 4
        ws = ops._workspace(dev, max(nws, int(L.fgnn_linear_wgrad_workspace_bytes(R, 64, Cout))))
        dsum2 = torch.empty((2, 64), device=dev, dtype=torch.float32)
        bias2c = None if pbias2 is None else pbias2.detach()
        if moments:
            mom = torch.empty(int(L.fgnn_block_tail_moments_bytes(R, Cout)) // 4, device=dev, dtype=torch.float32)
            ops.timed('block_tail_backward (reduce + moments + grad)', 2 * R * (2 * 64 + 2 * Cout + 64),
                      lambda: _hip.call('fgnn_block_tail_backward_moments', e, st2[2], st2[3], slope2, W2.detach(), bias2c, st3[0], st3[1],
                                        w3.detach(), st3[2], st3[3], slope3, gout, None, ga2, gw3, gb3, st2[0], st2[1], gw2, gb2, dsum2, R,
                                        Cout, ws, ws.numel() * 4, ops._fold_scratch(dev), mom, mom.numel() * 4),
                      nflops=8 * R * 64 * Cout)
        else:
            ops.timed('block_tail_backward (reduce + grad)', 2 * R * (2 * 64 + 2 * Cout + 64 + Cout),
                      lambda: _hip.call('fgnn_block_tail_backward', e, st2[2], st2[3], slope2, W2.detach(), bias2c, st3[0], st3[1],
                                        w3.detach(), st3[2], st3[3], slope3, gout, gz3, ga2, gw3, gb3, st2[0], st2[1], gw2, gb2, dsum2, R,
                                        Cout, ws, ws.numel() * 4, ops._fold_scratch(dev)),
                      nflops=6 * R * 64 * Cout)
        ge = torch.empty_like(e)
        ops.timed('bn_backward (apply)', 3 * e.numel() * 2, lambda: _hip.call(
            'fgnn_bn_backward_apply', e, ga2, ge, R, 64, _hip.BF16, st2[0], st2[1], w2.detach(), b2.detach(), slope2, dsum2))
        if moments:
            scale3 = st3[2]

            def launch(record, mom=mom, gW2=gW2, scale3=scale3, W2d=W2.detach(), bias2c=bias2c):
                ops.timed('block_tail_wgrad_finish (fold + combine)', 4 * mom.numel(), lambda: _hip.call(
                    'fgnn_block_tail_wgrad_finish', mom, mom.numel() * 4, R, Cout, W2d, bias2c, scale3, gW2.view(Cout, 64)))
            operands = (mom, scale3)
        else:
            def launch(record, a2=a2, gz3=gz3, gW2=gW2, gbias2=gbias2):
                ops.linear_wgrad(a2, [(gz3, gW2.view(Cout, 64), gbias2)], record)
            operands = (a2, gz3)
        grads.run_wgrad(launch, operands, 'W2', 'bias2')
        ha = ctx.has_add
        gadd = [None, None, None]
        for i in range(3):
            if ha[i]:
                gadd[i] = gout if ctx.periods[i] == 1 else pointwise.node_sum(gout, ctx.periods[i])
        return (ge, grads.result('gamma2'), grads.result('beta2'), None, None, None, None, grads.result('W2', pW2.dtype),
                grads.result('bias2'), grads.result('gamma3'), grads.result('beta3'), None, *gadd, None)


class mp_conv_residual(base_mp_nn):

    def __init__(self, nin, nmed, netype, extension=mp_conv_type.ORIG_WITH_DIFF,
                 with_residual=True, with_hop=False, aggregator='max', nout=None):
        super().__init__()
        nout = nin if nout is None else nout
        self.conv1 = _conv_norm_act(nin, nmed, BatchNormAct2d(nmed, slope=0.01), torch.nn.Identity())
        self.mp_conv = mp_conv_v2(nmed, nmed, netype, extension=extension, aggregtor=aggregator)
        self.conv2 = _conv_norm_act(nmed, nout, BatchNormAct2d(nout, slope=0.01), torch.nn.Identity())
        self.with_residual = with_residual
        self.with_hop = with_hop

    def folded_for_inference(self, device):
        mp = self.mp_conv
        bn1, bn2, bn3 = self.conv1[1], mp.bn, self.conv2[1]
        nin, nout = self.conv1[0].in_channels, self.conv2[0].out_channels
        key = tuple(t._version for t in (self.conv1[0].weight, self.conv1[0].bias, bn1.weight, bn1.bias, bn1.running_mean,
                                         bn1.running_var, mp.filters, mp.bias, bn2.weight, bn2.bias, bn2.running_mean,
                                         bn2.running_var, self.conv2[0].weight, self.conv2[0].bias, bn3.weight, bn3.bias,
                                         bn3.running_mean, bn3.running_var)) + (device, pointwise_state_epoch())
        if getattr(self, '_fuse_key', None) != key:
            def fold(bn, bias):
                s = bn.weight.float() * torch.rsqrt(bn.running_var.float() + bn.eps)
                t = bn.bias.float() - bn.running_mean.float() * s
                return s.contiguous(), (t + (bias.float() * s if bias is not None else 0)).contiguous()
            s1, t1 = fold(bn1, self.conv1[0].bias)
            s2, t2 = fold(bn2, mp.bias)
            s3, t3 = fold(bn3, self.conv2[0].bias)
            self._fuse = refresh_in_place(getattr(self, '_fuse', None), (
                self.conv1[0].weight.detach().float().reshape(64, nin), s1, t1,
                mp.filters.detach().float(), s2, t2,
                self.conv2[0].weight.detach().float().reshape(nout, 64), s3, t3))
            self._fuse_key = key
        return self._fuse

    def fusable_for_inference(self):
        mp = self.mp_conv
        bn1, bn2, bn3 = self.conv1[1], mp.bn, self.conv2[1]
        return (not self.with_residual and mp.nin == 64 and mp.nou == 64 and mp.nedge_types in (1, 4) and mp.aggregtor == 'max'
                and mp.extension == mp_conv_type.NO_EXTENSION and bn2 is not None and mp.bias is not None
                and isinstance(mp.activation_fn, torch.nn.ReLU) and isinstance(bn1, BatchNormAct2d)
                and isinstance(bn3, BatchNormAct2d) and bn1.slope == bn3.slope)

    def _fused_eval(self, x, nn_idx, etype, addend):
        mp = self.mp_conv
        bn1, bn2, bn3 = self.conv1[1], mp.bn, self.conv2[1]
        if (not FUSE_EVAL_BLOCKS or self.with_residual or self.training or torch.is_grad_enabled() or not x.is_cuda
                or x.dtype != torch.bfloat16 or x.shape[1] not in (64, 128, 256) or mp.nin != 64 or mp.nou != 64
                or mp.nedge_types not in (1, 4) or mp.aggregtor != 'max' or mp.extension != mp_conv_type.NO_EXTENSION
                or bn2 is None or mp.bias is None or not isinstance(mp.activation_fn, torch.nn.ReLU)
                or self.conv2[0].out_channels not in (64, 128, 256)
                or not isinstance(bn1, BatchNormAct2d) or not isinstance(bn3, BatchNormAct2d)
                or bn1.slope != bn3.slope or etype.dtype != torch.bfloat16):
            return None
        B, nin, N, _ = x.shape
        nout = self.conv2[0].out_channels
        M, k = nn_idx.shape[1:]
        fanout = mp.nedge_types == 1 and N == 1 and k == 1
        fanin = mp.nedge_types == 1 and M == 1 and k == N and N > 1 and ops.is_identity_list(nn_idx)
        if not (fanout or fanin) and not (mp.nedge_types == 4 and k in (3, 6)):
            return None
        xr = x.permute(0, 2, 3, 1)
        et = etype.permute(0, 2, 3, 1)
        if not xr.is_contiguous() or not (et.is_contiguous() or (etype.stride(0) == 0 and et[0].is_contiguous())):
            return None
        adds = as_addends(addend)
        if len(adds) > 3:
            return None
        row_mask = 0
        for i, a in enumerate(adds):
            src = getattr(a, '_fgnn_bcast_src', None)
            if src is not None and a.shape[2] > 1 and not (fanout or fanin) and src.dtype == x.dtype:
                adds[i] = src
                row_mask |= 1 << i
        for a in adds:
            if a.dtype != x.dtype or not a.permute(0, 2, 3, 1).is_contiguous():
                return None
        a0, a1, a2 = (adds + [None, None, None])[:3]
        W1, s1, t1, F, s2, t2, W2, s3, t3 = self.folded_for_inference(x.device)
        y = torch.empty((B, M, 1, nout), device=x.device, dtype=x.dtype).permute(0, 3, 1, 2)
        d = _hip.make_desc(x, nn_idx, etype, 64, mp.nedge_types, _hip.EXT_NONE, _hip.AGG_MAX, True, y)
        d.nin = 64
        if fanin:
            rc = _hip.invoke('fgnn_mpconv_block_forward_fanin', ctypes.byref(d), x, etype, W1, s1, t1, F, s2, t2, W2, s3, t3,
                             float(bn1.slope), nin, nout, a0, a1, a2, y)
            if rc == _hip.EUNSUPPORTED:
                return None
            _hip.check(rc)
            return y
        if fanout and not adds and B > 1 and ops.single_source_fanout(x, nn_idx, etype):
            y1 = torch.empty((B, 1, 1, nout), device=x.device, dtype=x.dtype).permute(0, 3, 1, 2)
            et1 = etype[:, :, :1, :]
            d1 = _hip.make_desc(x, nn_idx[:, :1, :], et1, 64, 1, _hip.EXT_NONE, _hip.AGG_MAX, True, y1)
            d1.nin = 64
            rc = _hip.invoke('fgnn_mpconv_block_forward_fanout', ctypes.byref(d1), x, et1, W1, s1, t1, F, s2, t2, W2, s3, t3,
                             float(bn1.slope), nin, nout, None, None, None, y1)
            if rc != _hip.EUNSUPPORTED:
                _hip.check(rc)
                return ops.broadcast_nodes(y1, M)
        if fanout:
            rc = _hip.invoke('fgnn_mpconv_block_forward_fanout', ctypes.byref(d), x, etype, W1, s1, t1, F, s2, t2, W2, s3, t3,
                             float(bn1.slope), nin, nout, a0, a1, a2, y)
            if rc == _hip.EUNSUPPORTED:
                return None
            _hip.check(rc)
            return y
        rc = _hip.invoke('fgnn_mpconv_block_forward_rows', ctypes.byref(d), x, nn_idx, etype, W1, s1, t1, F, s2, t2, W2, s3, t3,
                         float(bn1.slope), nin, nout, a0, a1, a2, row_mask, y)
        if rc == _hip.EUNSUPPORTED:
            return None
        _hip.check(rc)
        return y

    def forward(self, node_feature, nn_idx, etype, addend=None):
        nn_idx = ops.shared_graph_view(nn_idx)
        if etype.dtype != node_feature.dtype and torch.is_autocast_enabled('cuda') and etype.is_floating_point():
            etype = etype.to(torch.get_autocast_dtype('cuda'))
        staged = self.training and torch.is_grad_enabled()
        if callable(addend) and not staged:
            addend = addend()
        if not callable(addend):
            addend = as_addends(addend)
            if not staged and len(addend) > 3:
                addend = addend[:2] + [ops.add_n(addend[2:])]
            addend = addend if addend else None
        if not staged:
            y = self._fused_eval(node_feature, nn_idx, etype, addend)
            if y is not None:
                return y
        M = ops.single_source_fanout(node_feature, nn_idx, etype) if (staged and not self.with_residual and addend is None
                                                                     and node_feature.shape[0] > 1) else 0
        if M:
            B, C = node_feature.shape[:2]
            one = node_feature.reshape(B, 1, 1, C).permute(0, 3, 1, 2)
            y1 = self._forward_staged(one, nn_idx[:, :1, :], etype[:, :, :1, :], None, M)
            return ops.broadcast_nodes(y1, M)
        return self._forward_staged(node_feature, nn_idx, etype, addend, 1)

    def _forward_staged(self, node_feature, nn_idx, etype, addend, mult):
        fuse = self.training
        h = self._fused_train_head(node_feature)
        if h is None:
            handoff = BnHandoff.of(self.conv1[1]) if fuse else None
            h = self.conv1[1](self.conv1[0](node_feature, bn=handoff), handoff=handoff)
        y = self._fused_train_tail(h, nn_idx, etype, addend, mult)
        if y is not None:
            return y + node_feature if self.with_residual else y
        h = self.mp_conv(h, nn_idx, etype, population_mult=mult)
        handoff = BnHandoff.of(self.conv2[1]) if (fuse and mult == 1) else None
        h = self.conv2[0](h, bn=handoff)
        if callable(addend):
            addend = addend()
        h = self.conv2[1](h, addend=addend, population_mult=mult, handoff=handoff)
        return h + node_feature if self.with_residual else h

    def _fused_train_head(self, x):
        conv, bn = self.conv1[0], self.conv1[1]
        handoff = BnHandoff.of(bn) if isinstance(bn, BatchNormAct2d) else None
        if not (FUSE_TRAIN_HEAD and self.training and torch.is_grad_enabled() and x.is_cuda and isinstance(conv, PointwiseConv2d)
                and handoff is not None and conv.out_channels == 64 and conv.in_channels in _HEAD_WIDTHS
                and conv.weight.dtype == torch.float32 and (x.requires_grad or conv.weight.requires_grad)):
            return None
        B, C, H, W = x.shape
        rows = x.permute(0, 2, 3, 1)
        if not rows.is_contiguous():
            rows = rows.contiguous()
        rows = rows.view(B * H * W, C)
        if torch.is_autocast_enabled():
            rows = rows.to(torch.get_autocast_dtype('cuda'))
        L = _hip.lib()
        R = B * H * W
        if rows.dtype != torch.bfloat16 or R < 2 or not L.fgnn_block_tail_partials(R, C) or not L.fgnn_linear_forward_partials(R, C, 64):
            return None
        a1 = _BlockHead.apply(rows, conv.weight.view(64, C), conv.bias, bn.weight, bn.bias, handoff, float(bn.slope), ops.fan_box(x))
        return a1.view(B, H, W, 64).permute(0, 3, 1, 2)

    def _fused_train_tail(self, h, nn_idx, etype, addend, mult=1):
        mp = self.mp_conv
        bn2, conv2, bn3 = mp.bn, self.conv2[0], self.conv2[1]
        hand2, hand3 = (BnHandoff.of(b) if isinstance(b, BatchNormAct2d) else None for b in (bn2, bn3))
        if not (FUSE_TRAIN_TAIL and self.training and torch.is_grad_enabled() and h.is_cuda and h.dtype == torch.bfloat16
                and mp.nou == 64 and mp.extension == mp_conv_type.NO_EXTENSION
                and isinstance(mp.aggregtor, str) and isinstance(mp.activation_fn, torch.nn.ReLU)
                and hand2 is not None and hand3 is not None
                and isinstance(conv2, PointwiseConv2d) and conv2.in_channels == 64 and conv2.out_channels in (64, 128, 256)
                and conv2.weight.dtype == torch.float32):
            return None
        B, M = h.shape[0], nn_idx.shape[1]
        if B * M < 2 or not _hip.lib().fgnn_block_tail_partials(B * M, conv2.out_channels):
            return None
        z = ops.mpconv(h, nn_idx, etype, mp.filters, mp.bias, mp.nou, mp.nedge_types, _EXT_CODE[mp.extension],
                       _hip.AGG_CODES[mp.aggregtor], bn=hand2 if mult == 1 else None)
        rows = z.permute(0, 2, 3, 1)
        if not rows.is_contiguous():
            rows = rows.contiguous()
        rows = rows.view(B * M, 64)
        Cout = conv2.out_channels
        got = {}

        def addend_rows():
            with torch.enable_grad():
                a = addend() if callable(addend) else addend
                addends = as_addends(a)
                if len(addends) > 3:
                    addends = addends[:2] + [ops.add_n(addends[2:])]
                addends, periods = pointwise.split_broadcast(addends)
                arows = [None, None, None]
                for i, t in enumerate(addends):
                    ar = t.permute(0, 2, 3, 1)
                    if ar.dtype != rows.dtype or not ar.is_contiguous():
                        ar = ar.to(rows.dtype).contiguous()
                    arows[i] = ar.view(-1, Cout)
            got['arows'] = arows
            got['periods'] = tuple((periods + [1, 1, 1])[:3])
            got['streams'] = tuple(([getattr(t, '_fgnn_home_stream', None) for t in addends] + [None, None, None])[:3])
            return arows, got['periods']

        late = ROUTE_ADDEND_GRADS and LATE_JOIN and callable(addend) and torch.is_grad_enabled()
        arows, periods = (None, (1, 1, 1)) if late else addend_rows()
        route = late or (ROUTE_ADDEND_GRADS and torch.is_grad_enabled() and any(a is not None and a.requires_grad for a in arows))
        if late:
            def detached():
                ar, pr = addend_rows()
                return [None if a is None else a.detach() for a in ar], pr
            tail_adds = [detached, None, None]
        else:
            tail_adds = [(a.detach() if (route and a is not None) else a) for a in arows]
        y = _BlockTail.apply(rows, bn2.weight, bn2.bias, 0.0, float(bn3.slope), hand2, hand3, conv2.weight.view(Cout, 64), conv2.bias,
                             bn3.weight, bn3.bias, 0 if mult == 1 else B * M * mult, *tail_adds, periods)
        if route:
            pairs = [(a, q, st) for a, q, st in zip(got['arows'], got['periods'], got['streams']) if a is not None]
            y = _AddendRoute.apply(y, tuple(q for _, q, _ in pairs), tuple(st for _, _, st in pairs), *[a for a, _, _ in pairs])
        return y.view(B, M, 1, Cout).permute(0, 3, 1, 2)
```

factor-graph-neural-network_amd/fgnn_amd/ops.py:

```python
import ctypes
import os

import torch

from . import _hip
from .backward_pass import PASS, ParamGrads, run_wgrad
from .verdicts import Verdicts, remembered


class KernelTimer:

    def __init__(self):
        self.records = []

    def run(self, symbol, nbytes, nflops, launch, use_note=True):
        start, end = torch.cuda.Event(enable_timing=True), torch.cuda.Event(enable_timing=True)
        start.record()
        launch()
        end.record()
        name = (_hip.lib().fgnn_last_kernel().decode() or symbol) if use_note else symbol
        self.records.append((name, nbytes, nflops, start, end))

    def summary(self):
        torch.cuda.synchronize()
# ... 155 lines not shown

def backward_tables(nn_idx, d):
    if not BACKWARD_TABLES or (d.reserved & 0xffff) == 0 or (nn_idx.shape[0] > 1 and nn_idx.stride(0) != 0):
        return None
    L = _hip.lib()
    nbytes = int(L.fgnn_mpconv_backward_tables_bytes(ctypes.byref(d)))
    if nbytes == 0:
        return None
    def build():
        t = torch.empty(nbytes // 4, device=nn_idx.device, dtype=torch.int32)
        rc = _hip.invoke('fgnn_mpconv_backward_tables', ctypes.byref(d), nn_idx, t)
        if rc == _hip.EUNSUPPORTED:
            return None
        _hip.check(rc)
        torch.cuda.current_stream(nn_idx.device).synchronize()
        return t
    return remembered(nn_idx, '_fgnn_bwd_tables', (nn_idx.data_ptr(), d.N, d.M, d.k, d.reserved & 0xffff), build, during_capture=None)


def mpconv_forward_raw(x, nn_idx, etype, filters, bias, nou, net, ext, agg, *,
                       post_scale=None, post_shift=None, relu=False, want_argmax=False, bn=None, addends=None):
    _require_device(x, nn_idx, etype, filters, bias)
    _check_shapes(x, nn_idx, etype, filters, nou, net, ext)
    nn_idx = shared_graph_view(nn_idx)
    L = _hip.lib()
    M = nn_idx.shape[1]
    y = _alloc_out(x, nou, M)
    amax = None
    if want_argmax and agg == _hip.AGG_MAX:
        amax = torch.empty_like(y, dtype=torch.uint8)
    filters = filters.detach()
    if filters.dtype != torch.float32 or not filters.is_contiguous():
        filters = filters.float().contiguous()
    f32 = lambda t: None if t is None else t.detach().float().contiguous()
    bias, post_scale, post_shift = f32(bias), f32(post_scale), f32(post_shift)
    d = _hip.make_desc(x, nn_idx, etype, nou, net, ext, agg, relu, y)
    if M == 1 and net == 1 and agg == _hip.AGG_MAX and nn_idx.shape[2] == x.shape[2] and x.shape[2] > 1 and is_identity_list(nn_idx):
        d.reserved |= _hip.DESC_IDENTITY_LIST
    nbytes = int(L.fgnn_mpconv_algorithmic_bytes(ctypes.byref(d))) if TIMER is not None else 0
    npart = 0
    if bn is not None and STATS_EPILOGUE and post_scale is None and not relu:
        npart = int(L.fgnn_mpconv_forward_stats_partials(ctypes.byref(d)))
    if npart > 0:
        R = x.shape[0] * M
        ws = _workspace(x.device, int(L.fgnn_bn_workspace_bytes(R, nou)))
        stats, fin = bn.final(nou, x.device, R)
        fold = _fold_scratch(x.device)
        _launch('fwd', d, nbytes, lambda: _hip.call('fgnn_mpconv_forward_stats', ctypes.byref(d), x, nn_idx, etype, filters, bias, y, amax,
                                                    ws, fin, fold))
        bn.record(y.permute(0, 2, 3, 1).reshape(R, nou), stats)
        return y, amax
    if addends:
        fits = (amax is None and post_scale is not None and relu and len(addends) <= 3 and
                all(a.dtype == y.dtype and a.shape == y.shape and a.stride() == y.stride() for a in addends))
        took = []
        if fits:
            ap = list(addends) + [None] * (3 - len(addends))
            _launch('fwd', d, nbytes + sum(a.numel() * a.element_size() for a in addends), lambda: took.append(_hip.invoke(
                'fgnn_mpconv_forward_addends', ctypes.byref(d), x, nn_idx, etype, filters, bias, post_scale, post_shift, *ap, y)))
            if took[0] < 0:
                _hip.check(took[0])
            if took[0] == 1:
                return y, amax
            return add_n([y] + list(addends)), amax
    _launch('fwd', d, nbytes, lambda: _hip.call('fgnn_mpconv_forward', ctypes.byref(d), x, nn_idx, etype, filters, bias, post_scale,
                                                post_shift, y, amax))
    if addends:
        return add_n([y] + list(addends)), amax
    return y, amax


def grad_sink(param):
    if not ACCUMULATE_INTO_GRAD or param is None or not getattr(param, '_fgnn_grad_sink', False):
        return None
    if not param.is_leaf or not param.requires_grad:
        return None
    g = param.grad
    if (g is None or g.dtype != torch.float32 or not g.is_contiguous() or g.device != param.device
            or g.shape != param.shape or g.requires_grad):
        return None
    return g


def param_grads(device):
    return ParamGrads(device, grad_sink)


def enable_grad_sink(params, on=True):
    for q in params:
        q._fgnn_grad_sink = bool(on)


STAMPS = None


def stamp(tag):
    st = STAMPS
    if st is None:
        return
    i = len(st['tags'])
    if i >= st['buf'].numel():
        return
    st['tags'].append(tag)
    _hip.call('fgnn_stamp', st['buf'].data_ptr() + 8 * i)


ACCUMULATE_INTO_GRAD = True
STATS_EPILOGUE = True
_WS = {}


def _workspace(device, nbytes):
    key = (device, torch.cuda.current_stream(device).cuda_stream)
    ent = _WS.get(key)
    capturing = torch.cuda.is_current_stream_capturing()
    if ent is None or ent[0].numel() * 4 < nbytes:
        if ent is not None and ent[1]:
            _WS_CAPTURED.append(ent[0])
        ent = _WS[key] = [torch.empty((nbytes + 3) // 4, device=device, dtype=torch.float32), capturing]
    elif capturing:
        ent[1] = True
    return ent[0]


_WS_CAPTURED = []
_FOLD = {}


def _fold_scratch(device):
    key = (device, torch.cuda.current_stream(device).cuda_stream)
    buf = _FOLD.get(key)
    if buf is None:
        if torch.cuda.is_current_stream_capturing():
            raise _hip.FgnnHipError('fgnn_amd: first use of a stream inside hipGraph capture — run the step once eagerly on the capture '
                                    'stream first (graph.StepGraph does)')
        buf = _FOLD[key] = torch.zeros(_hip.FOLD_SCRATCH_BYTES // 4, device=device, dtype=torch.int32)
    return buf


_SIDE = {}
SIDE_STREAM = os.environ.get('FGNN_NO_SIDE_STREAM') is None


def side_stream(device):
    st = _SIDE.get(device)
    if st is None:
        st = _SIDE[device] = torch.cuda.Stream(device)
    return st


ROUTE_TAP = None


class _MPConv(torch.autograd.Function):

    @staticmethod
    def forward(ctx, x, nn_idx, etype, filters, bias, nou, net, ext, agg, bn=None):
        nn_idx = shared_graph_view(nn_idx)
        ctx.shared_et = etype.shape[0] == 1 and x.shape[0] > 1
        if ctx.shared_et:
            etype = etype.expand(x.shape[0], -1, -1, -1)
        z, amax = mpconv_forward_raw(x, nn_idx, etype, filters, bias, nou, net, ext, agg, bn=bn, want_argmax=True)
        if ROUTE_TAP is not None:
            ROUTE_TAP(filters, amax)
        ctx.cfg = (nou, net, ext, agg)
        ctx.params = (filters, bias)
        ctx.save_for_backward(x, nn_idx, etype, filters, amax)
        return z

    @staticmethod
    def backward(ctx, gz):
        backward_node_begins()
        x, nn_idx, etype, filters, amax = ctx.saved_tensors
        nou, net, ext, agg = ctx.cfg
        L = _hip.lib()
        B, M, k = nn_idx.shape
        zl = _alloc_out(x, nou, M)
        if gz.dtype != zl.dtype or gz.stride() != zl.stride():
            zl.copy_(gz)
            gz = zl
        dense = x.is_contiguous() or x.permute(0, 2, 3, 1).is_contiguous()
        xx = x if dense else x.contiguous()
        gx = torch.empty_like(xx)
        want_get = ctx.needs_input_grad[2]
        get = torch.empty((B, net, M, k), device=x.device, dtype=etype.dtype) if want_get else None
        grads = param_grads(x.device)
        gw = grads.acc('filters', ctx.params[0], filters.shape)
        gb = grads.acc('bias', ctx.params[1], (nou,))
        w = filters.detach().float().contiguous()
        d = _hip.make_desc(xx, nn_idx, etype, nou, net, ext, agg, False, gz)
        d.reserved = max_in_degree(nn_idx, x.shape[2])
        reduced = bool(want_get and ctx.shared_et and L.fgnn_mpconv_backward_reduces_getype(ctypes.byref(d)))
        if reduced:
            d.reserved |= _hip.DESC_GETYPE_REDUCED
            get = torch.empty((1, net, M, k), device=x.device, dtype=torch.float32)
        scope = PASS.fold_scope(grads.all_sunk('filters', 'bias') and PASS.folds_deferrable(), _workspace)
        ws = scope.slabs(x.device, int(L.fgnn_mpconv_backward_workspace_bytes(ctypes.byref(d))))
        nbytes = 0
        if TIMER is not None:
            shared_et = etype.stride(0) == 0 and B > 1
            shared_idx = nn_idx.stride(0) == 0 and B > 1
            nbytes = (xx.element_size() * (2 * xx.numel() + gz.numel())
                      + etype.element_size() * net * M * k * (1 if shared_et else B)
                      + 8 * M * k * (1 if shared_idx else B)
                      + (B * nou * M if amax is not None else 0)
                      + (get.element_size() * get.numel() if want_get else 0) + 8 * w.numel())
        tables = backward_tables(nn_idx, d)
        with scope:
            _launch('bwd', d, nbytes, lambda: _hip.call('fgnn_mpconv_backward_with_tables', ctypes.byref(d), xx, nn_idx, etype, w, gz, None,
                                                        amax, gx, get, gw, gb, ws, ws.numel() * 4, tables))
        if want_get and ctx.shared_et and not reduced:
            get = get.sum(dim=0, keepdim=True)
        if want_get and get.dtype != etype.dtype:
            get = get.to(etype.dtype)
        return (gx, None, get, grads.result('filters', filters.dtype), grads.result('bias'), None, None, None, None, None)


def _unexpanded(etype):
    if etype.dim() != 4 or etype.shape[0] < 2:
        return None
    if etype.stride(0) != 0:
        if etype.requires_grad:
            fn = etype.grad_fn
            reps = getattr(fn, '_saved_repeats', None) if fn is not None and fn.name() == 'RepeatBackward0' else None
            src = getattr(fn, '_saved_self_sym_sizes', None) if reps is not None else None
            if (not DEDUPE_GRAPHS or reps is None or src is None or tuple(reps) != (etype.shape[0], 1, 1, 1)
                    or tuple(src) != (1,) + tuple(etype.shape[1:])):
                return None
            return etype[:1]
        if not DEDUPE_GRAPHS or not etype.is_cuda:
            return None
        if torch.cuda.is_current_stream_capturing():
            same = Verdicts.recall('equal_rows', etype)
        else:
            same = Verdicts.note('equal_rows', etype, bool((etype == etype[:1]).all().item()))
        return etype[:1] if same else None
    base = etype._base
    if (base is not None and base.dim() == 4 and base.shape[0] == 1 and base.shape[1:] == etype.shape[1:]
            and base.data_ptr() == etype.data_ptr() and base.stride()[1:] == etype.stride()[1:]
            and base.requires_grad == etype.requires_grad):
        return base
    return etype[:1]


def autocast_operands(x, etype):
    if (x.dtype != etype.dtype and x.is_cuda and x.is_floating_point() and etype.is_floating_point()
            and torch.is_autocast_enabled('cuda')):
        dt = torch.get_autocast_dtype('cuda')
        x = x if x.dtype == dt else x.to(dt)
        etype = etype if etype.dtype == dt else etype.to(dt)
    return x, etype


def mpconv(x, nn_idx, etype, filters, bias, nou, net, ext, agg, bn=None):
    if ext != _hip.EXT_NONE:
        base = _unexpanded(etype)
        if base is not None:
            etype = base
    elif etype.shape[0] == 1 and x.shape[0] > 1:
        etype = etype.expand(x.shape[0], -1, -1, -1)
    return _MPConv.apply(x, nn_idx, etype, filters, bias, nou, net, ext, agg, bn)


def single_source_fanout(x, nn_idx, etype):
    if not FANOUT_BROADCAST or x.dim() != 4 or x.shape[2] != 1 or x.shape[3] != 1 or nn_idx.dim() != 3:
        return 0
    B, M, k = nn_idx.shape
    if k != 1 or M <= 1 or not x.is_cuda or etype.shape[2] != M:
        return 0
    if etype.stride(2) == 0:
        return M
    if etype.requires_grad:
        return 0
    same = remembered(etype, '_fgnn_node_invariant', (etype.data_ptr(),), lambda: bool((etype == etype[:, :, :1, :]).all().item()),
                      site='node_invariant', during_capture=False)
    return M if same else 0


FANOUT_BROADCAST = True


class _BroadcastNodes(torch.autograd.Function):

    @staticmethod
    def forward(ctx, y1, M):
        ctx.M = M
        return y1.expand(-1, -1, M, -1)

    @staticmethod
    def backward(ctx, g):
        backward_node_begins()
        from .mpnn import pointwise
        B, C, M, _ = g.shape
        rows = g.permute(0, 2, 3, 1)
        if not rows.is_contiguous():
            rows = rows.contiguous()
        return pointwise.node_sum(rows.reshape(B * M, C), M).view(B, 1, 1, C).permute(0, 3, 1, 2), None


def broadcast_nodes(y1, M):
    if torch.is_grad_enabled() and y1.requires_grad:
        out = _BroadcastNodes.apply(y1, M)
    else:
        out = y1.expand(-1, -1, M, -1)
    out._fgnn_bcast_src = y1
    if y1.is_cuda:
        y1._fgnn_home_stream = torch.cuda.current_stream(y1.device)
    return out


def _dense_same_layout(ts):
    t0 = ts[0]
    if not (t0.is_cuda and t0.dtype in (torch.float32, torch.bfloat16) and 2 <= len(ts) <= 8):
        return False
    if (t0.numel() * t0.element_size()) % 16 or t0.numel() == 0:
        return False
    dense = t0.is_contiguous() or (t0.dim() == 4 and t0.permute(0, 2, 3, 1).is_contiguous())
    order = lambda t: tuple(st for st, n in zip(t.stride(), t.shape) if n > 1)
    o0 = order(t0)
    return dense and all(t.dtype == t0.dtype and t.shape == t0.shape and order(t) == o0 and
                         t.data_ptr() % 16 == 0 for t in ts)


def sum_tensors(ts):
    ts = [t for t in ts if t is not None]
    if len(ts) == 1:
        return ts[0]
    if not _dense_same_layout(ts):
        out = ts[0]
        for t in ts[1:]:
            out = out + t
        return out
    out = torch.empty_like(ts[0])
    arr = (ctypes.c_void_p * len(ts))(*[t.data_ptr() for t in ts])
    timed('sum_n_kernel', (len(ts) + 1) * ts[0].numel() * ts[0].element_size(),
          lambda: _hip.call('fgnn_sum_n', arr, len(ts), ts[0].numel(), _hip.dtype_code(ts[0]), out))
    return out


MERGE_FAN_GRADS = True
MERGE_FAN_WGRADS = True
_PLACEHOLDERS = {}


class FanBox:

    def __init__(self, x):
        self.shape, self.dtype, self.device = tuple(x.shape), x.dtype, x.device
        B, C, H, W = x.shape
        self.R, self.C = B * H * W, C
        self.ok = (MERGE_FAN_GRADS and x.is_cuda and x.dtype == torch.bfloat16 and C in (64, 128, 256) and self.R >= 1024
                   and (x.permute(0, 2, 3, 1).is_contiguous() or x.is_contiguous() and H * W == 1))
        self.slots = [None, None, None]
        self.wg = [None, None, None]
        self.task = None
        self._ph = None

    def placeholder(self, shape):
        if self._ph is None:
            key = (self.device, self.dtype)
            ph = _PLACEHOLDERS.get(key)
            if ph is None:
                ph = _PLACEHOLDERS[key] = torch.zeros(1, device=self.device, dtype=self.dtype)
            self._ph = ph
        return self._ph.expand(shape)

    def is_placeholder(self, g):
        return self._ph is not None and g.data_ptr() == self._ph.data_ptr()

    def deposit(self, gz, weight, wgrad=None):
        if not self.ok or gz.dim() != 2 or gz.shape[0] != self.R or gz.dtype != torch.bfloat16 or not gz.is_contiguous():
            return 0
        self._enter_pass()
        K = gz.shape[1]
        if (tuple(weight.shape) != (K, self.C) or weight.dtype != torch.float32 or not weight.is_contiguous() or gz.data_ptr() % 16
                or weight.data_ptr() % 16):
            return 0
        order = (0, 2, 1) if K == 64 else ((1,) if K in (128, 256) else ())
        for i in order:
            if self.slots[i] is None:
                self.slots[i] = (gz, weight)
                if MERGE_FAN_WGRADS and wgrad is not None and self._wgrad_ok(K, *wgrad):
                    self.wg[i] = wgrad
                    return 2
                return 1
        return 0

    def _enter_pass(self):
        task = torch._C._current_graph_task_id()
        if self.task != task:
            if any(self.slots):
                self.slots, self.wg = [None, None, None], [None, None, None]
            self.task = task

    def _wgrad_ok(self, K, rows, gW, gb):
        if not (rows.dtype == torch.bfloat16 and tuple(rows.shape) == (self.R, self.C) and rows.is_contiguous() and rows.data_ptr() % 16 == 0):
            return False
        if not (gW.dtype == torch.float32 and gW.numel() == K * self.C and gW.is_contiguous()):
            return False
        if gb is not None and not (gb.dtype == torch.float32 and gb.numel() == K and gb.is_contiguous()):
            return False
        first = next((w for w in self.wg if w is not None), None)
        return first is None or first[0].data_ptr() == rows.data_ptr()

    def _park_wgrads(self, slots, wg):
        jobs = [(slots[i][0], wg[i]) for i in range(3) if wg[i] is not None]
        if not jobs:
            return
        if len(jobs) == 3 and self.C == 256 and jobs[1][0].shape[1] == 256:
            self._park_wgrad_group([jobs[0], jobs[2]])
            self._park_wgrad_group([jobs[1]])
            return
        self._park_wgrad_group(jobs)

    def _park_wgrad_group(self, jobs):
        rows = jobs[0][1][0]
        wjobs = [(gz, gW, gb) for gz, (_, gW, gb) in jobs]
        run_wgrad(lambda record: linear_wgrad(rows, wjobs, record), (rows,) + tuple(j[0] for j in wjobs), sunk=True)

    def merge(self, grads):
        real = [g for g in grads if g is not None and not self.is_placeholder(g)]
        self._enter_pass()
        slots, self.slots = self.slots, [None, None, None]
        wg, self.wg = self.wg, [None, None, None]
        if not any(slots):
            return sum_tensors(real) if real else None
        self._park_wgrads(slots, wg)
        if slots[0] is None and slots[2] is not None:
            slots[0], slots[2] = slots[2], None
        B, C, H, W = self.shape
        adds = []
        for g in real:
            rows = g.permute(0, 2, 3, 1)
            if rows.dtype != self.dtype or not rows.is_contiguous():
                rows = rows.to(self.dtype).contiguous()
            adds.append(rows.view(self.R, C))
        if len(adds) > 3:
            adds = adds[:2] + [sum_tensors(adds[2:])]
        cur = torch.cuda.current_stream(self.device)
        for sl in slots:
            if sl is not None:
                sl[0].record_stream(cur)
        out = torch.empty((self.R, C), device=self.device, dtype=self.dtype)
        xs = (ctypes.c_void_p * 3)(*[sl[0].data_ptr() if sl else None for sl in slots])
        ws = (ctypes.c_void_p * 3)(*[sl[1].data_ptr() if sl else None for sl in slots])
        ks = (ctypes.c_int32 * 3)(*[sl[0].shape[1] if sl else 0 for sl in slots])
        ad = (ctypes.c_void_p * 3)(*([a.data_ptr() for a in adds] + [None] * (3 - len(adds))))
        ktot = sum(ks)
        timed('linear_multi_b16_kernel', 2 * self.R * (ktot + C * (1 + len(adds))),
              lambda: _hip.call('fgnn_linear_multi_forward', xs, ks, ws, ad, out, self.R, C),
              nflops=2 * self.R * ktot * C)
        return out.view(B, H, W, C).permute(0, 3, 1, 2)


def fan_box(x):
    box = getattr(x, '_fgnn_box', None)
    return box if (box is not None and box.ok) else None


class _FanOut(torch.autograd.Function):

    @staticmethod
    def forward(ctx, x, n, box):
        ctx.set_materialize_grads(False)
        ctx.box = box
        return tuple(x.view_as(x) for _ in range(n))

    @staticmethod
    def backward(ctx, *grads):
        backward_node_begins()
        return ctx.box.merge(grads), None, None


class _SumN(torch.autograd.Function):
    @staticmethod
    def forward(ctx, *ts):
        return sum_tensors([t.detach() for t in ts])

    @staticmethod
    def backward(ctx, g):
        return tuple(g for _ in ctx.needs_input_grad)


def fan_out(x, n):
    if n <= 1 or not (torch.is_grad_enabled() and x.requires_grad and x.is_cuda):
        return [x] * n
    box = FanBox(x) if x.dim() == 4 else None
    if box is None:
        class _Plain:
            ok = False
            merge = staticmethod(lambda grads: (lambda gs: sum_tensors(gs) if gs else None)([g for g in grads if g is not None]))
        box = _Plain()
    outs = list(_FanOut.apply(x, n, box))
    for o in outs:
        o._fgnn_box = box
    return outs


def add_n(ts):
    ts = [t for t in ts if t is not None]
    if len(ts) == 1:
        return ts[0]
    if not (ts[0].is_cuda and _dense_same_layout([t.detach() for t in ts])):
        out = ts[0]
        for t in ts[1:]:
            out = out + t
        return out
    return _SumN.apply(*ts)


def _concat2_plan(a, b, dim):
    if not (a.is_cuda and b.is_cuda and a.dim() == 4 and b.dim() == 4 and a.dtype == b.dtype and a.shape[3] == 1 and b.shape[3] == 1
            and a.shape[0] == b.shape[0] and dim in (1, 2) and a.shape[3 - dim] == b.shape[3 - dim] and a.numel() and b.numel()):
        return None
    es = a.element_size()
    for t in (a, b):
        C, N = t.shape[1], t.shape[2]
        if (C > 1 and t.stride(1) != 1) or (N > 1 and t.stride(2) < C) or (t.shape[0] > 1 and t.stride(0) < C * N):
# ... 63 lines not shown
```

Measured before the change: 2.039 billion.

## Fuse batch-norm/activation backward apply into mpconv backward gradient load

Adds a path where the mpconv backward kernels (hyper-edge fan-in and ws families) compute the incoming gradient on load from the BN pre-activation and its upstream gradient, so there is no separate bn_backward apply pass. The Python side links the block tail to the mpconv through a GzLink record and probes in forward whether the chosen kernel family supports this. It is meant to remove one full read/write of the [rows][64] gradient tensor and a kernel launch. In exchange the kernels carry extra per-element BN arithmetic and read a second input, and an unsupported call falls back to the separate apply.

```diff
diff --git a/factor-graph-neural-network_amd/csrc/bnact.hip b/factor-graph-neural-network_amd/csrc/bnact.hip
--- a/factor-graph-neural-network_amd/csrc/bnact.hip
+++ b/factor-graph-neural-network_amd/csrc/bnact.hip
@@ -203,12 +203,9 @@
     for (int e = 0; e < EPC; ++e) {
         if (MODE == 0) { ka[e] = p.a[c0 + e]; kb[e] = p.b[c0 + e]; kc[e] = kd[e] = ke[e] = kf[e] = 0.f; }
         else {
-            ka[e] = p.a[c0 + e];
-            kb[e] = p.b[c0 + e];
-            kc[e] = p.gamma[c0 + e] * kb[e];
-            kd[e] = p.beta[c0 + e] - ka[e] * kc[e];
-            ke[e] = p.dbeta[c0 + e] * p.dsum_scale;
-            kf[e] = p.dgamma[c0 + e] * p.dsum_scale;
+            const FgnnBnBwdK k = fgnn_bn_bwd_consts(p.a[c0 + e], p.b[c0 + e], p.gamma[c0 + e], p.beta[c0 + e], p.dbeta[c0 + e],
+                                                    p.dgamma[c0 + e], p.dsum_scale);
+            ka[e] = k.mean; kb[e] = k.invstd; kc[e] = k.scale; kd[e] = k.shift; ke[e] = k.dbeta_r; kf[e] = k.dgamma_r;
         }
     }
     const int64_t r_begin = (int64_t)blockIdx.x * p.rows_per_wg;
@@ -235,12 +232,7 @@
             float g[EPC];
             Chunk<T>::load(gg + r * p.C + c0, g);
 #pragma unroll
-            for (int e = 0; e < EPC; ++e) {
-                const float pre = fmaf(v[e], kc[e], kd[e]);
-                const float ge = pre > 0.f ? g[e] : g[e] * p.slope;
-                const float xh = (v[e] - ka[e]) * kb[e];
-                o[e] = kc[e] * (ge - ke[e] - xh * kf[e]);
-            }
+            for (int e = 0; e < EPC; ++e) o[e] = fgnn_bn_bwd_elem(v[e], g[e], ka[e], kb[e], kc[e], kd[e], ke[e], kf[e], p.slope);
         }
         Chunk<T>::store(og + r * p.C + c0, o);
     }
diff --git a/factor-graph-neural-network_amd/csrc/fgnn_device.h b/factor-graph-neural-network_amd/csrc/fgnn_device.h
--- a/factor-graph-neural-network_amd/csrc/fgnn_device.h
+++ b/factor-graph-neural-network_amd/csrc/fgnn_device.h
@@ -83,6 +83,25 @@
     return __builtin_amdgcn_fdot2_f32_bf16(__builtin_bit_cast(bf16x2, p), __builtin_bit_cast(bf16x2, e), acc, false);
 }
 
+struct FgnnBnBwdK { float mean, invstd, scale, shift, dbeta_r, dgamma_r; };
+__device__ __forceinline__ FgnnBnBwdK fgnn_bn_bwd_consts(float mean, float invstd, float gamma, float beta, float dbeta, float dgamma, float rinv) {
+    FgnnBnBwdK k;
+    k.mean = mean;
+    k.invstd = invstd;
+    k.scale = gamma * invstd;
+    k.shift = __builtin_fmaf(-mean, k.scale, beta);
+    k.dbeta_r = dbeta * rinv;
+    k.dgamma_r = dgamma * rinv;
+    return k;
+}
+__device__ __forceinline__ float fgnn_bn_bwd_elem(float x, float g, float mean, float invstd, float scale, float shift, float dbeta_r,
+                                                  float dgamma_r, float slope) {
+    const float pre = __builtin_fmaf(x, scale, shift);
+    const float ge = pre > 0.f ? g : g * slope;
+    const float xh = (x - mean) * invstd;
+    return scale * __builtin_fmaf(-xh, dgamma_r, ge - dbeta_r);
+}
+
 template <int DK> __device__ __forceinline__ void fgnn_pgm_logits(const void* dec, int64_t o, int64_t cs, float& v0, float& v1) {
     if (DK == FGNN_PGM_DEC_F32) {
         const float* d = static_cast<const float*>(dec);
diff --git a/factor-graph-neural-network_amd/csrc/mpconv_bwd.hip b/factor-graph-neural-network_amd/csrc/mpconv_bwd.hip
--- a/factor-graph-neural-network_amd/csrc/mpconv_bwd.hip
+++ b/factor-graph-neural-network_amd/csrc/mpconv_bwd.hip
@@ -482,27 +482,73 @@
     return FGNN_OK;
 }
 
-static const struct { FgnnBwdPlanFn plan; FgnnBwdLaunchFn launch; } kBwdFamilies[] = {
-    {fgnn_bwd_ext_plan, fgnn_bwd_ext_launch},
-    {fgnn_bwd_hyper_plan, fgnn_bwd_hyper_launch},
-    {fgnn_bwd_ws_plan, fgnn_bwd_ws_launch},
-    {fgnn_bwd_sg_plan, fgnn_bwd_sg_launch},
-    {fgnn_bwd_b16_plan, fgnn_bwd_b16_launch},
-    {fgnn_bwd_res_plan, fgnn_bwd_res_launch},
-    {generic_plan, generic_launch},
+static const struct { FgnnBwdPlanFn plan; FgnnBwdLaunchFn launch; bool gz_bn; } kBwdFamilies[] = {
+    {fgnn_bwd_ext_plan, fgnn_bwd_ext_launch, false},
+    {fgnn_bwd_hyper_plan, fgnn_bwd_hyper_launch, true},
+    {fgnn_bwd_ws_plan, fgnn_bwd_ws_launch, true},
+    {fgnn_bwd_sg_plan, fgnn_bwd_sg_launch, false},
+    {fgnn_bwd_b16_plan, fgnn_bwd_b16_launch, false},
+    {fgnn_bwd_res_plan, fgnn_bwd_res_launch, false},
+    {generic_plan, generic_launch, false},
 };
 static const int kBwdGeneric = sizeof(kBwdFamilies) / sizeof(kBwdFamilies[0]) - 1;
 
-static int bwd_run(const FgnnBwdCall& c) {
+static int bwd_run(const FgnnBwdCall& c, bool launch = true) {
     const FgnnSwitches& sw = fgnn_switches();
     for (int f = sw.force_generic ? kBwdGeneric : 0; f <= kBwdGeneric; ++f) {
         FgnnPlan pl = {};
         pl.family = f;
         const int rc = kBwdFamilies[f].plan(c, sw, &pl);
         if (rc < 0) return rc;
-        if (rc > 0) return kBwdFamilies[f].launch(c, pl);
+        if (rc == 0) continue;
+        if (c.bn && !kBwdFamilies[f].gz_bn)
+            FGNN_FAIL(FGNN_EUNSUPPORTED, "mpconv backward: the kernel family of this call (%d) does not form gz from a fgnn_gz_bn record", f);
+        return launch ? kBwdFamilies[f].launch(c, pl) : 1;
     }
     return FGNN_EUNSUPPORTED;
+}
+
+static int bwd_check_gz_bn(const fgnn_mpconv_desc* d, const fgnn_gz_bn* bn, bool pointers) {
+    if (pointers && (!bn->e || !bn->ga || !bn->mean || !bn->invstd || !bn->gamma || !bn->beta || !bn->dsum))
+        FGNN_FAIL(FGNN_EINVAL, "mpconv_backward_gz_bn: null pointer in fgnn_gz_bn");
+    if (bn->rows != (int64_t)d->B * d->M) FGNN_FAIL(FGNN_EINVAL, "mpconv_backward_gz_bn: rows must be B * M");
+    if (d->nou != 64 || d->dtype != FGNN_BF16)
+        FGNN_FAIL(FGNN_EUNSUPPORTED, "mpconv_backward_gz_bn: a record stands for bf16 [rows][64] tensors (nou %d, dtype %d)", d->nou, d->dtype);
+    if (!(d->y_sc == 1 && (d->y_sm == 64 || d->M == 1) && (d->y_sb == (int64_t)64 * d->M || d->B == 1)))
+        FGNN_FAIL(FGNN_EUNSUPPORTED, "mpconv_backward_gz_bn: gz's layout is not the dense channel-fastest [rows][64] of e / ga");
+    if (pointers && ((((uintptr_t)bn->e) | ((uintptr_t)bn->ga)) & 15))
+        FGNN_FAIL(FGNN_EUNSUPPORTED, "mpconv_backward_gz_bn: e / ga must be 16-byte aligned");
+    return FGNN_OK;
+}
+
+extern "C" int fgnn_mpconv_backward_gz_bn(const fgnn_mpconv_desc* d, const void* x, const int64_t* nn_idx, const void* etype,
+                                          const float* filters, const void* gz, const void* z, const uint8_t* argmax, void* gx,
+                                          void* getype, float* gfilters, float* gbias, void* workspace, int64_t workspace_bytes,
+                                          const void* tables, const fgnn_gz_bn* gz_bn, fgnn_stream_t stream) {
+    int rc = fgnn_check_desc(d);
+    if (rc) return rc;
+    if (!x || !nn_idx || !etype || !filters || !gx || !gfilters || (gz_bn ? gz != nullptr : gz == nullptr))
+        FGNN_FAIL(FGNN_EINVAL, gz_bn && gz ? "mpconv_backward_gz_bn: gz must be NULL when a record is given" : "null tensor pointer");
+    if (d->agg == FGNN_AGG_MAX && !argmax) FGNN_FAIL(FGNN_EINVAL, "max aggregator needs the forward's argmax");
+    if (gz_bn && (rc = bwd_check_gz_bn(d, gz_bn, true))) return rc;
+    if (d->B == 0) return FGNN_OK;
+    const FgnnBwdCall c = {d, x, nn_idx, etype, filters, gz, z, argmax, gx, getype, gfilters, gbias, workspace, workspace_bytes,
+                           tables, (hipStream_t)stream, gz_bn};
+    return bwd_run(c);
+}
+
+extern "C" int fgnn_mpconv_backward_takes_gz_bn(const fgnn_mpconv_desc* d) {
+    if (!d || fgnn_check_desc(d) || d->B == 0) return 0;
+    alignas(256) static char probe[256];
+    fgnn_gz_bn bn = {};
+    bn.rows = (int64_t)d->B * d->M;
+    if (bwd_check_gz_bn(d, &bn, false)) return 0;
+    for (int with_getype = 1; with_getype >= 0; --with_getype) {
+        const FgnnBwdCall c = {d, probe, (const int64_t*)probe, probe, (const float*)probe, nullptr, nullptr, (const uint8_t*)probe, probe,
+                               with_getype ? probe : nullptr, (float*)probe, (float*)probe, probe, INT64_MAX, nullptr, nullptr, &bn};
+        if (bwd_run(c, false) == 1) return 1;
+    }
+    return 0;
 }
 
 extern "C" int fgnn_mpconv_backward_with_tables(const fgnn_mpconv_desc* d, const void* x, const int64_t* nn_idx,
diff --git a/factor-graph-neural-network_amd/csrc/mpconv_bwd_hyper.hip b/factor-graph-neural-network_amd/csrc/mpconv_bwd_hyper.hip
--- a/factor-graph-neural-network_amd/csrc/mpconv_bwd_hyper.hip
+++ b/factor-graph-neural-network_amd/csrc/mpconv_bwd_hyper.hip
@@ -17,6 +17,9 @@
     void* gx;
     float* ws;
     int has_bias;
+    const void* bn_e;
+    const float* bn_mean; const float* bn_invstd; const float* bn_gamma; const float* bn_beta; const float* bn_dsum;
+    float bn_rinv, bn_slope;
 };
 
 extern __shared__ __attribute__((aligned(16))) float fgnn_lds_bh[];
@@ -88,6 +91,13 @@
 #pragma unroll
     for (int q = 0; q < NO; ++q) gbc[q] = lane + 64 * q;
 
+    constexpr bool CAN_BN = NO == 1 && sizeof(T) == 2;
+    const bool gz_bn = CAN_BN && p.bn_e != nullptr;
+    const T* E = reinterpret_cast<const T*>(p.bn_e);
+    FgnnBnBwdK bk = {};
+    if (gz_bn) bk = fgnn_bn_bwd_consts(p.bn_mean[lane], p.bn_invstd[lane], p.bn_gamma[lane], p.bn_beta[lane], p.bn_dsum[lane],
+                                       p.bn_dsum[64 + lane], p.bn_rinv);
+
     const int nwaves = gridDim.x * BH_WAVES;
     for (int b = blockIdx.x * BH_WAVES + wave; b < d.B; b += nwaves) {
         int ns[NO];
@@ -95,7 +105,10 @@
 #pragma unroll
         for (int q = 0; q < NO; ++q) {
             const int64_t yo = (int64_t)b * d.y_sb + (int64_t)(lane + 64 * q) * d.y_sc;
-            const float g = fgnn_ld(GZ + yo);
+            float g = fgnn_ld(GZ + yo);
+            if (gz_bn)
+                g = fgnn_lo(fgnn_pack2(fgnn_bn_bwd_elem(fgnn_ld(E + yo), g, bk.mean, bk.invstd, bk.scale, bk.shift, bk.dbeta_r, bk.dgamma_r,
+                                                        p.bn_slope), 0.f));
             int js = p.argmax[yo];
             js = js < k ? js : k - 1;
             int n = (int)p.idx[(int64_t)b * d.idx_sb + (int64_t)js * d.idx_sk];
@@ -233,6 +246,8 @@
     const bool fanin = d->M == 1 && d->k >= 1 && d->k <= 256 && d->N >= 1;
     const bool fanout = !fanin && d->N == 1 && d->k == 1;
     if (!fanin && !fanout) FGNN_REJECT("hyper-edge backward", 4);
+    if (c.bn && !(fanin && d->nou == 64 && d->dtype == FGNN_BF16 && d->y_sc == 1))
+        FGNN_FAIL(FGNN_EUNSUPPORTED, "hyper-edge backward: gz on load is the bf16 fan-in kernel's, 64 output channels");
     if (fanout && !(d->y_sc == 1 && d->y_sm % 4 == 0 && d->y_sb % 4 == 0 && d->y_sm >= d->nou)) FGNN_REJECT("hyper-edge backward", 5);
     const int64_t slab_len = (int64_t)d->nin * d->nou + d->nou;
     if (!c.workspace || c.workspace_bytes < 256 * slab_len * 4) FGNN_REJECT("hyper-edge backward", 6);
@@ -257,7 +272,14 @@
     p.d = *d;
     p.x = c.x; p.idx = c.idx; p.et = c.et; p.W = c.W; p.gz = c.gz; p.argmax = c.argmax; p.gx = c.gx;
     p.ws = (float*)c.workspace; p.has_bias = c.gbias != nullptr;
-    fgnn_note_kernel("mpconv_bwd_%s_kernel<%s, %d, %d>", pl.mode ? "fanin" : "fanout", d->dtype ? "bf16_t" : "float", d->nin / 64, d->nou / 64);
+    p.bn_e = nullptr; p.bn_mean = p.bn_invstd = p.bn_gamma = p.bn_beta = p.bn_dsum = nullptr; p.bn_rinv = p.bn_slope = 0.f;
+    if (c.bn) {
+        p.gz = c.bn->ga; p.bn_e = c.bn->e;
+        p.bn_mean = c.bn->mean; p.bn_invstd = c.bn->invstd; p.bn_gamma = c.bn->gamma; p.bn_beta = c.bn->beta; p.bn_dsum = c.bn->dsum;
+        p.bn_rinv = 1.0f / (float)c.bn->rows; p.bn_slope = c.bn->slope;
+    }
+    fgnn_note_kernel(c.bn ? "mpconv_bwd_%s_kernel<%s, %d, %d> gz_bn" : "mpconv_bwd_%s_kernel<%s, %d, %d>", pl.mode ? "fanin" : "fanout",
+                     d->dtype ? "bf16_t" : "float", d->nin / 64, d->nou / 64);
     void* args[] = {(void*)&p};
     hipError_t e = hipLaunchKernel(pl.fn, dim3(pl.grid), dim3(pl.block), args, pl.lds, c.stream);
     if (e != hipSuccess) FGNN_FAIL(FGNN_ELAUNCH, "mpconv hyper-edge backward launch: %s", hipGetErrorString(e));
diff --git a/factor-graph-neural-network_amd/csrc/mpconv_bwd_ws.hip b/factor-graph-neural-network_amd/csrc/mpconv_bwd_ws.hip
--- a/factor-graph-neural-network_amd/csrc/mpconv_bwd_ws.hip
+++ b/factor-graph-neural-network_amd/csrc/mpconv_bwd_ws.hip
@@ -29,6 +29,9 @@
     long long x_sb, et_sb, y_sb;
     const int* tables;
     long long* prof;
+    const uint16_t* bn_e;
+    const float* bn_mean; const float* bn_invstd; const float* bn_gamma; const float* bn_beta; const float* bn_dsum;
+    float bn_rinv;
 };
 
 #ifdef FGNN_ENABLE_PROF
@@ -61,6 +64,9 @@
     static constexpr int OFF_GT = OFF_SLOT + MMAX * KC * 4;
     static constexpr int OFF_DUMP = OFF_GT + 8 * MMAX * KC * 4;
     static constexpr int BYTES = OFF_DUMP + 16;
+    static constexpr int OFF_BNK = BYTES;
+    static constexpr int BYTES_BN = OFF_BNK + 6 * 64 * 4;
+    static_assert(BYTES_BN <= 160 * 1024, "LDS");
 };
 
 template <int KC, int DEG>
@@ -119,7 +125,7 @@
     for (int f = tid; f < 8 * mk; f += BW_THREADS) out[NMAX * QS + 4 + f] = (int)gtab[f];
 }
 
-template <int KC, int DEG, int XLD = 64, int NL = BwLayout<KC>::NMAX>
+template <int KC, int DEG, int XLD = 64, int NL = BwLayout<KC>::NMAX, bool GZBN = false>
 __global__ __launch_bounds__(BW_THREADS) void mpconv_bwd_ws_kernel(const BwParams p) {
     typedef BwLayout<KC> LY;
     constexpr int QS = LY::QS;
@@ -185,6 +191,13 @@
         }
     }
     long long idx_v = tid < mk ? p.idx[tid] : 0;
+    float bnv[GZBN ? 6 : 1] = {};
+    if constexpr (GZBN) {
+        if (tid < 64) {
+            bnv[0] = p.bn_mean[tid]; bnv[1] = p.bn_invstd[tid]; bnv[2] = p.bn_gamma[tid]; bnv[3] = p.bn_beta[tid];
+            bnv[4] = p.bn_dsum[tid]; bnv[5] = p.bn_dsum[64 + tid];
+        }
+    }
     bw_barrier();
     BW_STAMP_G(40);
     bf16x8 aP[4];
@@ -222,9 +235,10 @@
 #pragma unroll
             for (int u = 0; u < 16; ++u) RA[t][u] = 0.f;
     }
-    auto prefetch_g = [&](int b, uint4 (&pg)[NSLOT], uint2 (&pa)[NSLOT]) {
+    auto prefetch_g = [&](int b, uint4 (&pg)[NSLOT], uint2 (&pa)[NSLOT], uint4 (&px)[NSLOT]) {
         const unsigned char* gzb = reinterpret_cast<const unsigned char*>(p.gz + (int64_t)b * p.y_sb);
         const unsigned char* amb = p.argmax + (int64_t)b * p.y_sb;
+        const unsigned char* exb = GZBN ? reinterpret_cast<const unsigned char*>(p.bn_e + (int64_t)b * p.y_sb) : nullptr;
         int blo = bl;
         asm volatile("" : "+v"(blo));
 #pragma unroll
@@ -232,21 +246,31 @@
             const int item = blo + 384 * sl;
             pg[sl] = make_uint4(0, 0, 0, 0);
             pa[sl] = make_uint2(0, 0);
+            if constexpr (GZBN) px[sl] = make_uint4(0, 0, 0, 0);
             if (build_wave && item < 8 * M) {
                 const unsigned el = (unsigned)((item >> 3) * p.y_ld + 8 * (item & 7));
                 pg[sl] = *fgnn_at<uint4>(gzb, el * 2u);
                 pa[sl] = *fgnn_at<uint2>(amb, el);
+                if constexpr (GZBN) px[sl] = *fgnn_at<uint4>(exb, el * 2u);
             }
         }
     };
     BW_STAMP_G(41);
-    uint4 pg0[NSLOT];
+    uint4 pg0[NSLOT], px0[NSLOT];
     uint2 pa0[NSLOT];
-    if (b_begin < b_end) prefetch_g(b_begin, pg0, pa0);
+    if (b_begin < b_end) prefetch_g(b_begin, pg0, pa0, px0);
 
     bw_barrier();
     BW_STAMP_G(42);
     for (int f = OFF_G / 16 + tid; f < LY::BYTES / 16; f += BW_THREADS) reinterpret_cast<uint4*>(bw_lds)[f] = make_uint4(0, 0, 0, 0);
+    if constexpr (GZBN) {
+        if (tid < 64) {
+            const FgnnBnBwdK k = fgnn_bn_bwd_consts(bnv[0], bnv[1], bnv[2], bnv[3], bnv[4], bnv[5], p.bn_rinv);
+            float* kt = reinterpret_cast<float*>(bw_lds + LY::OFF_BNK);
+            kt[tid] = k.mean; kt[64 + tid] = k.invstd; kt[128 + tid] = k.scale; kt[192 + tid] = k.shift;
+            kt[256 + tid] = k.dbeta_r; kt[320 + tid] = k.dgamma_r;
+        }
+    }
     BW_STAMP_G(43);
     bw_barrier();
     BW_STAMP_G(44);
@@ -329,7 +353,7 @@
             if (et_src[sl] >= 0) pe[sl] = *fgnn_at<uint2>(p.et + (int64_t)b * p.et_sb, (unsigned)et_src[sl] * 8u);
         }
     };
-    auto build = [&](const uint4 (&pg)[NSLOT], const uint2 (&pa)[NSLOT], const uint2 (&pe)[ESLOT]) {
+    auto build = [&](const uint4 (&pg)[NSLOT], const uint2 (&pa)[NSLOT], const uint2 (&pe)[ESLOT], const uint4 (&px)[NSLOT]) {
 #pragma unroll
         for (int sl = 0; sl < ESLOT; ++sl) {
             if (et_src[sl] >= 0) {
@@ -344,7 +368,26 @@
             if (item < 8 * M) {
                 typedef unsigned short u16x2 __attribute__((ext_vector_type(2)));
                 typedef short s16x2 __attribute__((ext_vector_type(2)));
-                const unsigned gq[4] = {pg[sl].x, pg[sl].y, pg[sl].z, pg[sl].w};
+                unsigned gq[4] = {pg[sl].x, pg[sl].y, pg[sl].z, pg[sl].w};
+                if constexpr (GZBN) {
+                    const unsigned ex[4] = {px[sl].x, px[sl].y, px[sl].z, px[sl].w};
+                    const unsigned char* kt = bw_lds + LY::OFF_BNK + (item & 7) * 32;
+#pragma unroll
+                    for (int h = 0; h < 2; ++h) {
+                        f32x4 k[6];
+#pragma unroll
+                        for (int t = 0; t < 6; ++t) k[t] = *reinterpret_cast<const f32x4*>(kt + t * 256 + h * 16);
+#pragma unroll
+                        for (int u = 0; u < 2; ++u) {
+                            const int d = 2 * h + u;
+                            const float lo = fgnn_bn_bwd_elem(fgnn_lo(ex[d]), fgnn_lo(gq[d]), k[0][2 * u], k[1][2 * u], k[2][2 * u], k[3][2 * u],
+                                                              k[4][2 * u], k[5][2 * u], 0.f);
+                            const float hi = fgnn_bn_bwd_elem(fgnn_hi(ex[d]), fgnn_hi(gq[d]), k[0][2 * u + 1], k[1][2 * u + 1], k[2][2 * u + 1],
+                                                              k[3][2 * u + 1], k[4][2 * u + 1], k[5][2 * u + 1], 0.f);
+                            gq[d] = fgnn_pack2(lo, hi);
+                        }
+                    }
+                }
                 unsigned gofs[KC];
 #pragma unroll
                 for (int j = 0; j < KC; ++j) gofs[j] = gtab[item * KC + j];
@@ -373,7 +416,7 @@
     if (b_begin < b_end) {
         if (build_wave) {
             uint2 pe[ESLOT];
-            prefetch_e(b_begin, pe); build(pg0, pa0, pe);
+            prefetch_e(b_begin, pe); build(pg0, pa0, pe, px0);
         }
         if (dma_wave) fgnn_wait_vm<0>();
     }
@@ -492,7 +535,7 @@
                 }
             }
         };
-        auto phase3_dw = [&](const uint4 (&pg)[NSLOT], const uint2 (&pa)[NSLOT], const uint2 (&pe)[ESLOT]) {
+        auto phase3_dw = [&](const uint4 (&pg)[NSLOT], const uint2 (&pa)[NSLOT], const uint2 (&pe)[ESLOT], const uint4 (&px)[NSLOT]) {
                 const unsigned xbase = lds0 + (unsigned)(OFF_X + cur * (BW_MAXN * BW_XROW));
                 constexpr int nks = NL / 16;
                 uint2 f0[8], f1[8];
@@ -519,7 +562,7 @@
                                 RA[2 * c2 + cj], 0, 0, 0);
                 };
                 load(f0, 0);
-                if (has_next) build(pg, pa, pe);
+                if (has_next) build(pg, pa, pe, px);
     #pragma unroll 1
                 for (int ks = 0; ks + 1 < nks; ks += 2) {
                     load(f1, ks + 1);
@@ -530,9 +573,9 @@
                 if (nks & 1) mma(f0);
         };
         if (build_wave) {
-            uint4 pg[NSLOT];
+            uint4 pg[NSLOT], px[NSLOT];
             uint2 pa[NSLOT], pe[ESLOT];
-            prefetch_g(has_next ? b + 1 : b, pg, pa);
+            prefetch_g(has_next ? b + 1 : b, pg, pa, px);
             prefetch_e(has_next ? b + 1 : b, pe);
             phase2a();
             BW_STAMP(3);
@@ -542,8 +585,8 @@
             BW_STAMP(5);
             bw_barrier();
             BW_STAMP(6);
-            if (dw_wave) phase3_dw(pg, pa, pe);
-            else if (has_next) build(pg, pa, pe);
+            if (dw_wave) phase3_dw(pg, pa, pe, px);
+            else if (has_next) build(pg, pa, pe, px);
         } else {
             phase2a();
             BW_STAMP(3);
@@ -640,6 +683,15 @@
     }
     BW_STAMP_G(5);
 }
+
+static int g_bw_gzbn_mask = 1;
+extern "C" int fgnn_set_gz_bn_instances(int32_t mask) {
+    const int was = g_bw_gzbn_mask;
+    g_bw_gzbn_mask = mask & 3;
+    return was;
+}
+#define BW_GZBN_VF (g_bw_gzbn_mask & 1)
+#define BW_GZBN_FV (g_bw_gzbn_mask & 2)
 
 static int bw_tables_count(const fgnn_mpconv_desc* d) {
     if (fgnn_switches().no_ws || d->dtype != FGNN_BF16 || d->ext != FGNN_EXT_NONE || d->net != 4 || d->agg != FGNN_AGG_MAX) return 0;
@@ -689,10 +741,22 @@
     const int64_t slab_len = 64 * 256 + 64;
     if (!c.workspace || c.workspace_bytes < ((split || ksplit) ? 2 : 1) * 256 * slab_len * 4) FGNN_REJECT("ws backward", 7);
     const bool nl48 = KC == 3 && d->N <= 48;
-    pl->fn = ksplit ? (KC == 6 ? (void*)mpconv_bwd_ws_kernel<6, 3, 128> : nl48 ? (void*)mpconv_bwd_ws_kernel<3, 6, 128, 48> : (void*)mpconv_bwd_ws_kernel<3, 6, 128>)
-                    : (KC == 6 ? (void*)mpconv_bwd_ws_kernel<6, 3> : nl48 ? (void*)mpconv_bwd_ws_kernel<3, 6, 64, 48> : (void*)mpconv_bwd_ws_kernel<3, 6>);
+    if (c.bn) {
+        if (split || ksplit || d->nou != 64 || (KC == 3 && !nl48))
+            FGNN_FAIL(FGNN_EUNSUPPORTED, "ws backward: no gz-on-load instance for %d -> %d channels, k %d, N %d", d->nin, d->nou, KC, d->N);
+        if (c.bn->slope != 0.f) FGNN_FAIL(FGNN_EUNSUPPORTED, "ws backward: gz on load takes slope 0 only (got %g)", (double)c.bn->slope);
+        if (!(KC == 6 ? BW_GZBN_VF : BW_GZBN_FV))
+            FGNN_FAIL(FGNN_EUNSUPPORTED, "ws backward: the gz-on-load instance of k %d is off (it lost to the staged pass: profiles/bn2_on_load)", KC);
+    }
     static_assert(BwLayout<6>::BYTES <= 160 * 1024 && BwLayout<3>::BYTES <= 160 * 1024, "LDS");
-    pl->lds = KC == 6 ? BwLayout<6>::BYTES : BwLayout<3>::BYTES;
+    if (c.bn) {
+        pl->fn = KC == 6 ? (void*)mpconv_bwd_ws_kernel<6, 3, 64, 96, true> : (void*)mpconv_bwd_ws_kernel<3, 6, 64, 48, true>;
+        pl->lds = KC == 6 ? BwLayout<6>::BYTES_BN : BwLayout<3>::BYTES_BN;
+    } else {
+        pl->fn = ksplit ? (KC == 6 ? (void*)mpconv_bwd_ws_kernel<6, 3, 128> : nl48 ? (void*)mpconv_bwd_ws_kernel<3, 6, 128, 48> : (void*)mpconv_bwd_ws_kernel<3, 6, 128>)
+                        : (KC == 6 ? (void*)mpconv_bwd_ws_kernel<6, 3> : nl48 ? (void*)mpconv_bwd_ws_kernel<3, 6, 64, 48> : (void*)mpconv_bwd_ws_kernel<3, 6>);
+        pl->lds = KC == 6 ? BwLayout<6>::BYTES : BwLayout<3>::BYTES;
+    }
     int grid = d->B < 256 ? d->B : 256;
     const int chunk = (d->B + grid - 1) / grid;
     pl->grid = (d->B + chunk - 1) / chunk;
@@ -716,11 +780,18 @@
     p.y_ld = d->nou; p.w_ld = d->nou * 4; p.x_ld = d->nin; p.accum = 0;
     p.x_sb = d->x_sb; p.et_sb = d->et_sb; p.y_sb = d->y_sb;
     p.tables = pl.aux ? (const int*)c.tables : nullptr;
+    p.bn_e = nullptr; p.bn_mean = p.bn_invstd = p.bn_gamma = p.bn_beta = p.bn_dsum = nullptr; p.bn_rinv = 0.f;
+    if (c.bn) {
+        p.gz = (const uint16_t*)c.bn->ga; p.bn_e = (const uint16_t*)c.bn->e;
+        p.bn_mean = c.bn->mean; p.bn_invstd = c.bn->invstd; p.bn_gamma = c.bn->gamma; p.bn_beta = c.bn->beta; p.bn_dsum = c.bn->dsum;
+        p.bn_rinv = 1.0f / (float)c.bn->rows;
+    }
     hipError_t e = hipFuncSetAttribute(pl.fn, hipFuncAttributeMaxDynamicSharedMemorySize, pl.lds);
     if (e != hipSuccess) FGNN_FAIL(FGNN_ELAUNCH, "hipFuncSetAttribute(%d B LDS): %s", pl.lds, hipGetErrorString(e));
     const int grid = pl.grid;
     hipStream_t st = c.stream;
-    fgnn_note_kernel(split ? "mpconv_bwd_ws_kernel<%d, %d> x2" : (ksplit ? "mpconv_bwd_ws_kernel<%d, %d> k2" : "mpconv_bwd_ws_kernel<%d, %d>"), KC, DEG);
+    if (c.bn) fgnn_note_kernel("mpconv_bwd_ws_kernel<%d, %d, 64, %d, true>", KC, DEG, KC == 6 ? 96 : 48);
+    else fgnn_note_kernel(split ? "mpconv_bwd_ws_kernel<%d, %d> x2" : (ksplit ? "mpconv_bwd_ws_kernel<%d, %d> k2" : "mpconv_bwd_ws_kernel<%d, %d>"), KC, DEG);
     p.prof = fgnn_prof_begin();
     void* args[] = {(void*)&p};
     e = hipLaunchKernel(pl.fn, dim3(grid), dim3(pl.block), args, pl.lds, st);
diff --git a/factor-graph-neural-network_amd/csrc/mpconv_dispatch.h b/factor-graph-neural-network_amd/csrc/mpconv_dispatch.h
--- a/factor-graph-neural-network_amd/csrc/mpconv_dispatch.h
+++ b/factor-graph-neural-network_amd/csrc/mpconv_dispatch.h
@@ -1,5 +1,6 @@
 #pragma once
 #include "fgnn_common.h"
+#include "fgnn_hip_gz_bn.h"
 
 struct FgnnFold;
 
@@ -31,6 +32,7 @@
     void* gx; void* getype; float* gW; float* gbias; void* workspace; int64_t workspace_bytes;
     const void* tables;
     hipStream_t stream;
+    const fgnn_gz_bn* bn;
 };
 
 struct FgnnPlan {
diff --git a/factor-graph-neural-network_amd/fgnn_amd/_hip.py b/factor-graph-neural-network_amd/fgnn_amd/_hip.py
--- a/factor-graph-neural-network_amd/fgnn_amd/_hip.py
+++ b/factor-graph-neural-network_amd/fgnn_amd/_hip.py
@@ -25,6 +25,11 @@
     _fields_ = [(n, ctypes.c_void_p) for n in ('gamma', 'beta', 'running_mean', 'running_var', 'num_batches_tracked',
                                                'mean', 'invstd', 'scale', 'shift', 'shift_k')] + \
                [('count', ctypes.c_int64), ('population', ctypes.c_int64), ('momentum', ctypes.c_float), ('eps', ctypes.c_float)]
+
+
+class GzBn(ctypes.Structure):
+    _fields_ = [(n, ctypes.c_void_p) for n in ('e', 'ga', 'mean', 'invstd', 'gamma', 'beta', 'dsum')] + \
+               [('slope', ctypes.c_float), ('rows', ctypes.c_int64)]
 
 
 class DevicePointer:
@@ -45,7 +50,7 @@
 
 _SCALARS = {'int': ctypes.c_int32, 'int32_t': ctypes.c_int32, 'int64_t': ctypes.c_int64, 'uint64_t': ctypes.c_uint64,
             'float': ctypes.c_float, 'double': ctypes.c_double, 'fgnn_stream_t': DevicePointer}
-_STRUCTS = {'fgnn_mpconv_desc': MPConvDesc, 'fgnn_bn_final': BnFinal}
+_STRUCTS = {'fgnn_mpconv_desc': MPConvDesc, 'fgnn_bn_final': BnFinal, 'fgnn_gz_bn': GzBn}
 
 
 def _uncommented(header_text):
@@ -271,3 +276,11 @@
 LDPC_TRAIN = bind_header('fgnn_hip_ldpc_train.h')
 PGM_BP = bind_header('fgnn_hip_pgm_bp.h')
 LDPC_CODE = bind_header('fgnn_hip_ldpc_code.h')
+GZ_BN = bind_header('fgnn_hip_gz_bn.h')
+
+
+def gz_bn(e, ga, mean, invstd, gamma, beta, dsum, slope, rows):
+    r = GzBn()
+    r.e, r.ga, r.mean, r.invstd, r.gamma, r.beta, r.dsum = (t.data_ptr() for t in (e, ga, mean, invstd, gamma, beta, dsum))
+    r.slope, r.rows = float(slope), int(rows)
+    return r
diff --git a/factor-graph-neural-network_amd/fgnn_amd/mpnn/blocks.py b/factor-graph-neural-network_amd/fgnn_amd/mpnn/blocks.py
--- a/factor-graph-neural-network_amd/fgnn_amd/mpnn/blocks.py
+++ b/factor-graph-neural-network_amd/fgnn_amd/mpnn/blocks.py
@@ -175,6 +175,7 @@
                 grads.result('gamma'), grads.result('beta'), None, None, None)
 
 
+BN2_ON_LOAD = True
 LATE_JOIN = True
 ROUTE_ADDEND_GRADS = True
 
@@ -218,7 +219,8 @@
 
     @staticmethod
     def forward(ctx, e, w2, b2, slope2, slope3, bn2, bn3, W2, bias2, w3, b3, population, add0=None, add1=None, add2=None,
-                periods=(1, 1, 1)):
+                periods=(1, 1, 1), gz_link=None):
+        ctx.gz_link = gz_link
         L = _hip.lib()
         R, Cout = e.shape[0], W2.shape[0]
         dev = e.device
@@ -284,9 +286,14 @@
                                         w3.detach(), st3[2], st3[3], slope3, gout, gz3, ga2, gw3, gb3, st2[0], st2[1], gw2, gb2, dsum2, R,
                                         Cout, ws, ws.numel() * 4, ops._fold_scratch(dev)),
                       nflops=6 * R * 64 * Cout)
-        ge = torch.empty_like(e)
-        ops.timed('bn_backward (apply)', 3 * e.numel() * 2, lambda: _hip.call(
-            'fgnn_bn_backward_apply', e, ga2, ge, R, 64, _hip.BF16, st2[0], st2[1], w2.detach(), b2.detach(), slope2, dsum2))
+        link = ctx.gz_link
+        if BN2_ON_LOAD and link is not None and link.fusable and ctx.needs_input_grad[0]:
+            link.pending = (torch._C._current_graph_task_id(), e, ga2, st2[0], st2[1], w2.detach(), b2.detach(), dsum2, slope2)
+            ge = ops.placeholder(dev, e.dtype, e.shape)
+        else:
+            ge = torch.empty_like(e)
+            ops.timed('bn_backward (apply)', 3 * e.numel() * 2, lambda: _hip.call(
+                'fgnn_bn_backward_apply', e, ga2, ge, R, 64, _hip.BF16, st2[0], st2[1], w2.detach(), b2.detach(), slope2, dsum2))
         if moments:
             scale3 = st3[2]
 
@@ -305,7 +312,7 @@
             if ha[i]:
                 gadd[i] = gout if ctx.periods[i] == 1 else pointwise.node_sum(gout, ctx.periods[i])
         return (ge, grads.result('gamma2'), grads.result('beta2'), None, None, None, None, grads.result('W2', pW2.dtype),
-                grads.result('bias2'), grads.result('gamma3'), grads.result('beta3'), None, *gadd, None)
+                grads.result('bias2'), grads.result('gamma3'), grads.result('beta3'), None, *gadd, None, None)
 
 
 class mp_conv_residual(base_mp_nn):
@@ -498,8 +505,9 @@
         B, M = h.shape[0], nn_idx.shape[1]
         if B * M < 2 or not _hip.lib().fgnn_block_tail_partials(B * M, conv2.out_channels):
             return None
+        link = ops.GzLink() if mult == 1 else None
         z = ops.mpconv(h, nn_idx, etype, mp.filters, mp.bias, mp.nou, mp.nedge_types, _EXT_CODE[mp.extension],
-                       _hip.AGG_CODES[mp.aggregtor], bn=hand2 if mult == 1 else None)
+                       _hip.AGG_CODES[mp.aggregtor], bn=hand2 if mult == 1 else None, gz_link=link)
         rows = z.permute(0, 2, 3, 1)
         if not rows.is_contiguous():
             rows = rows.contiguous()
@@ -536,7 +544,7 @@
         else:
             tail_adds = [(a.detach() if (route and a is not None) else a) for a in arows]
         y = _BlockTail.apply(rows, bn2.weight, bn2.bias, 0.0, float(bn3.slope), hand2, hand3, conv2.weight.view(Cout, 64), conv2.bias,
-                             bn3.weight, bn3.bias, 0 if mult == 1 else B * M * mult, *tail_adds, periods)
+                             bn3.weight, bn3.bias, 0 if mult == 1 else B * M * mult, *tail_adds, periods, link)
         if route:
             pairs = [(a, q, st) for a, q, st in zip(got['arows'], got['periods'], got['streams']) if a is not None]
             y = _AddendRoute.apply(y, tuple(q for _, q, _ in pairs), tuple(st for _, _, st in pairs), *[a for a, _, _ in pairs])
diff --git a/factor-graph-neural-network_amd/fgnn_amd/ops.py b/factor-graph-neural-network_amd/fgnn_amd/ops.py
--- a/factor-graph-neural-network_amd/fgnn_amd/ops.py
+++ b/factor-graph-neural-network_amd/fgnn_amd/ops.py
@@ -331,10 +331,34 @@
 ROUTE_TAP = None
 
 
+def placeholder(device, dtype, shape):
+    key = (device, dtype)
+    ph = _PLACEHOLDERS.get(key)
+    if ph is None:
+        ph = _PLACEHOLDERS[key] = torch.zeros(1, device=device, dtype=dtype)
+    return ph.expand(shape)
+
+
+_PLACEHOLDERS = {}
+
+
+class GzLink:
+    __slots__ = ('fusable', 'pending')
+
+    def __init__(self):
+        self.fusable, self.pending = False, None
+
+    def take(self):
+        rec, self.pending = self.pending, None
+        if rec is None or rec[0] != torch._C._current_graph_task_id():
+            return None
+        return rec[1:]
+
+
 class _MPConv(torch.autograd.Function):
 
     @staticmethod
-    def forward(ctx, x, nn_idx, etype, filters, bias, nou, net, ext, agg, bn=None):
+    def forward(ctx, x, nn_idx, etype, filters, bias, nou, net, ext, agg, bn=None, gz_link=None):
         nn_idx = shared_graph_view(nn_idx)
         ctx.shared_et = etype.shape[0] == 1 and x.shape[0] > 1
         if ctx.shared_et:
@@ -345,6 +369,16 @@
         ctx.cfg = (nou, net, ext, agg)
         ctx.params = (filters, bias)
         ctx.save_for_backward(x, nn_idx, etype, filters, amax)
+        ctx.gz_link = gz_link
+        if gz_link is not None:
+            M = nn_idx.shape[1]
+            rows_dense = z.stride(1) == 1 and (M == 1 or z.stride(2) == nou) and (z.shape[0] == 1 or z.stride(0) == M * nou)
+            x_dense = x.is_contiguous() or x.permute(0, 2, 3, 1).is_contiguous()
+            gz_link.fusable = False
+            if rows_dense and x_dense and z.dtype == torch.bfloat16:
+                d = _hip.make_desc(x, nn_idx, etype, nou, net, ext, agg, False, z)
+                d.reserved = max_in_degree(nn_idx, x.shape[2])
+                gz_link.fusable = bool(_hip.invoke('fgnn_mpconv_backward_takes_gz_bn', ctypes.byref(d)))
         return z
 
     @staticmethod
@@ -354,10 +388,14 @@
         nou, net, ext, agg = ctx.cfg
         L = _hip.lib()
         B, M, k = nn_idx.shape
-        zl = _alloc_out(x, nou, M)
-        if gz.dtype != zl.dtype or gz.stride() != zl.stride():
-            zl.copy_(gz)
-            gz = zl
+        rec = ctx.gz_link.take() if ctx.gz_link is not None else None
+        if rec is not None:
+            gz = rec[1].view(B, M, 1, nou).permute(0, 3, 1, 2)
+        else:
+            zl = _alloc_out(x, nou, M)
+            if gz.dtype != zl.dtype or gz.stride() != zl.stride():
+                zl.copy_(gz)
+                gz = zl
         dense = x.is_contiguous() or x.permute(0, 2, 3, 1).is_contiguous()
         xx = x if dense else x.contiguous()
         gx = torch.empty_like(xx)
@@ -379,20 +417,36 @@
         if TIMER is not None:
             shared_et = etype.stride(0) == 0 and B > 1
             shared_idx = nn_idx.stride(0) == 0 and B > 1
-            nbytes = (xx.element_size() * (2 * xx.numel() + gz.numel())
+            nbytes = (xx.element_size() * (2 * xx.numel() + gz.numel() * (2 if rec is not None else 1))
                       + etype.element_size() * net * M * k * (1 if shared_et else B)
                       + 8 * M * k * (1 if shared_idx else B)
                       + (B * nou * M if amax is not None else 0)
                       + (get.element_size() * get.numel() if want_get else 0) + 8 * w.numel())
         tables = backward_tables(nn_idx, d)
         with scope:
-            _launch('bwd', d, nbytes, lambda: _hip.call('fgnn_mpconv_backward_with_tables', ctypes.byref(d), xx, nn_idx, etype, w, gz, None,
-                                                        amax, gx, get, gw, gb, ws, ws.numel() * 4, tables))
+            if rec is not None:
+                e, ga, mean, invstd, gamma, beta, dsum, slope = rec
+                R = e.shape[0]
+                took = []
+                bn = _hip.gz_bn(e, ga, mean, invstd, gamma, beta, dsum, slope, R)
+                _launch('bwd', d, nbytes, lambda: took.append(_hip.invoke(
+                    'fgnn_mpconv_backward_gz_bn', ctypes.byref(d), xx, nn_idx, etype, w, None, None, amax, gx, get, gw, gb, ws,
+                    ws.numel() * 4, tables, ctypes.byref(bn))))
+                if took[0] == _hip.EUNSUPPORTED:
+                    ge = torch.empty_like(e)
+                    timed('bn_backward (apply)', 3 * e.numel() * 2, lambda: _hip.call(
+                        'fgnn_bn_backward_apply', e, ga, ge, R, nou, _hip.BF16, mean, invstd, gamma, beta, slope, dsum))
+                    gz, rec = ge.view(B, M, 1, nou).permute(0, 3, 1, 2), None
+                else:
+                    _hip.check(took[0])
+            if rec is None:
+                _launch('bwd', d, nbytes, lambda: _hip.call('fgnn_mpconv_backward_with_tables', ctypes.byref(d), xx, nn_idx, etype, w, gz, None,
+                                                            amax, gx, get, gw, gb, ws, ws.numel() * 4, tables))
         if want_get and ctx.shared_et and not reduced:
             get = get.sum(dim=0, keepdim=True)
         if want_get and get.dtype != etype.dtype:
             get = get.to(etype.dtype)
-        return (gx, None, get, grads.result('filters', filters.dtype), grads.result('bias'), None, None, None, None, None)
+        return (gx, None, get, grads.result('filters', filters.dtype), grads.result('bias'), None, None, None, None, None, None)
 
 
 def _unexpanded(etype):
@@ -431,14 +485,14 @@
     return x, etype
 
 
-def mpconv(x, nn_idx, etype, filters, bias, nou, net, ext, agg, bn=None):
+def mpconv(x, nn_idx, etype, filters, bias, nou, net, ext, agg, bn=None, gz_link=None):
     if ext != _hip.EXT_NONE:
         base = _unexpanded(etype)
         if base is not None:
             etype = base
     elif etype.shape[0] == 1 and x.shape[0] > 1:
         etype = etype.expand(x.shape[0], -1, -1, -1)
-    return _MPConv.apply(x, nn_idx, etype, filters, bias, nou, net, ext, agg, bn)
+    return _MPConv.apply(x, nn_idx, etype, filters, bias, nou, net, ext, agg, bn, gz_link)
 
 
 def single_source_fanout(x, nn_idx, etype):
@@ -519,7 +573,6 @@
 
 MERGE_FAN_GRADS = True
 MERGE_FAN_WGRADS = True
-_PLACEHOLDERS = {}
 
 
 class FanBox:
@@ -536,13 +589,9 @@
         self._ph = None
 
     def placeholder(self, shape):
-        if self._ph is None:
-            key = (self.device, self.dtype)
-            ph = _PLACEHOLDERS.get(key)
-            if ph is None:
-                ph = _PLACEHOLDERS[key] = torch.zeros(1, device=self.device, dtype=self.dtype)
-            self._ph = ph
-        return self._ph.expand(shape)
+        out = placeholder(self.device, self.dtype, shape)
+        self._ph = _PLACEHOLDERS[(self.device, self.dtype)]
+        return out
 
     def is_placeholder(self, g):
         return self._ph is not None and g.data_ptr() == self._ph.data_ptr()
diff --git a/include/fgnn_hip_gz_bn.h b/include/fgnn_hip_gz_bn.h
--- /dev/null
+++ b/include/fgnn_hip_gz_bn.h
@@ -0,0 +1,27 @@
+#ifndef FGNN_HIP_GZ_BN_H
+#define FGNN_HIP_GZ_BN_H
+
+#include "fgnn_hip.h"
+
+#ifdef __cplusplus
+extern "C" {
+#endif
+
+typedef struct fgnn_gz_bn {
+    const void* e; const void* ga; const float* mean; const float* invstd;
+    const float* gamma; const float* beta; const float* dsum; float slope; int64_t rows;
+} fgnn_gz_bn;
+
+int fgnn_mpconv_backward_gz_bn(const fgnn_mpconv_desc* d, const void* x, const int64_t* nn_idx, const void* etype,
+                               const float* filters, const void* gz, const void* z, const uint8_t* argmax, void* gx,
+                               void* getype, float* gfilters, float* gbias, void* workspace, int64_t workspace_bytes,
+                               const void* tables, const fgnn_gz_bn* gz_bn, fgnn_stream_t stream);
+
+int fgnn_mpconv_backward_takes_gz_bn(const fgnn_mpconv_desc* d);
+
+int fgnn_set_gz_bn_instances(int32_t mask);
+
+#ifdef __cplusplus
+}
+#endif
+#endif
```

After: 2.010 billion. -1.4%, worse.
